# isno0907/ldmae

Measured on AMD Instinct MI355X. Metric: DiT-B train-step images/sec (32×32×16 latents) at 1/2/4/8 MI355X, higher is better.
Workload: dtype bf16; 1 GPU; LightningDiT-B/1 f8d16 bf16 train step (fwd+bwd+AdamW+EMA), 1024 tokens x 768, synthetic ImageNet-256 latents 32x32x16; per_gpu_batch=256, global_batch=256, parallelism=dp1

## Files before the change

### include/ldmae_hip.h

```cpp
#ifndef LDMAE_HIP_H
#define LDMAE_HIP_H
#ifdef __cplusplus
extern "C" {
#endif

#define LDMAE_OK 0
#define LDMAE_ERR_INVALID (-1)
#define LDMAE_ERR_HIP (-2)

#define LDMAE_F32 0
#define LDMAE_BF16 1
#define LDMAE_F16 2

#define LDMAE_EPI_BIAS 0
#define LDMAE_EPI_GATE_RES 1
#define LDMAE_EPI_BIAS_POS 2
#define LDMAE_EPI_BIAS_GELU 3
#define LDMAE_EPI_SWIGLU 4
#define LDMAE_EPI_SWIGLU_BWD 5
#define LDMAE_EPI_GELU_BWD 6
#define LDMAE_EPI_QKV_ROPE 7
#define LDMAE_EPI_TILE_LAUNCH 0x100
#define LDMAE_EPI_HALF_LINES 0x200
#define LDMAE_EPI_F16_INF 0x400

const char* ldmae_last_error(void);
const char* ldmae_version(void);
const char* ldmae_arch(void);

int ldmae_gemm_nt(int dtype, int out_dtype, int epi, const void* A, int lda, const void* B, int ldb, void* C, int ldc,
                  int M, int N, int K, const float* bias, float beta, const float* xin, float* xout,
                  const float* gate, int gate_ld, int rows_per_batch, void* stream);
int ldmae_gemm_nt_qkv_rope_ok(int B, int N, int H, int hd, int K, int lda, int ldb);
int ldmae_gemm_nt_qkv_rope(const void* A, int lda, const void* W, int ldb, const float* bias, void* qkv, void* q2, void* k2, const float* wq,
                           const float* wk, const float* cos, const float* sin, int B, int N, int H, int hd, int K, float eps, int store_raw_qk,
                           int tile_launch, void* stream);
int ldmae_gemm_tn_splits(int dtype, int M, int N, int K);
long ldmae_gemm_tn_workspace_bytes(int dtype, int M, int N, int K);
int ldmae_gemm_tn(int dtype, const void* A, int lda, const void* B, int ldb, float* C, float* dbias, int M, int N, int K, float beta,
                  float* workspace, long workspace_bytes, void* stream);
long ldmae_colsum_workspace_bytes(int M, int N);
int ldmae_colsum(int dtype, const void* X, int ldx, int M, int N, float* out, float beta, float* workspace, void* stream);

int ldmae_cast_weight(int dst_dtype, const float* src, void* dst, void* dstT, int R, int C, void* stream);
int ldmae_cast(int src_dtype, int dst_dtype, const void* src, void* dst, long n, void* stream);
int ldmae_thin_nt(int out_dtype, const float* T, const float* W, const float* bias, const float* pos, void* out, int M, int N, int K,
                  int rows_per_batch, void* stream);
long ldmae_thin_tn_workspace_bytes(int M, int N, int K);
int ldmae_thin_tn(const float* G, const float* T, float* dW, float* dbias, int M, int N, int K, float beta, float* workspace,
                  long workspace_bytes, void* stream);
int ldmae_multi_add(int count, void* const* dst, const void* const* src, const long* n, void* stream);
int ldmae_cast_stack(int dst_dtype, const void* const* srcs, int count, long n_each, void* dst, void* stream);

int ldmae_rmsnorm_modulate_fwd(int out_dtype, const float* x, const float* w, const float* shift, const float* scale,
                               int mod_ld, void* out, float* rstd, int M, int D, int rows_per_batch, float eps, void* stream);
long ldmae_rmsnorm_modulate_bwd_workspace_bytes(int M, int D, int rows_per_batch);
int ldmae_rmsnorm_modulate_bwd(int dtype, const void* dout, const float* x, const float* w, const float* scale, int mod_ld,
                               const float* rstd, float* dx_accum, float beta_x, float* dshift, float* dscale, int dmod_ld, float* dw,
                               float beta_w, int M, int D, int rows_per_batch, float* workspace, void* stream);
long ldmae_rmsnorm_modulate_bwd_gate_workspace_bytes(int M, int D, int rows_per_batch);
int ldmae_rmsnorm_modulate_bwd_gate(int dtype, const void* dout, const float* x, const float* w, const float* scale, int mod_ld,
                                    const float* rstd, float* dx_accum, float beta_x, float* dshift, float* dscale, int dmod_ld, float* dw,
                                    float beta_w, const void* y, const float* gate, int gate_ld, void* dy, float* dgate, int dgate_ld,
                                    float* dbias, int M, int D, int rows_per_batch, float* workspace, void* stream);
int ldmae_layernorm_modulate_fwd(int out_dtype, const float* x, const float* shift, const float* scale, int mod_ld, void* out, float* rstd,
                                 int M, int D, int rows_per_batch, float eps, void* stream);
int ldmae_layernorm_modulate_bwd(int dtype, const void* dout, const float* x, const float* scale, int mod_ld, const float* rstd, float* dx_accum,
                                 float beta_x, float* dshift, float* dscale, int dmod_ld, int M, int D, int rows_per_batch, float* workspace,
                                 void* stream);
int ldmae_layernorm_modulate_bwd_gate(int dtype, const void* dout, const float* x, const float* scale, int mod_ld, const float* rstd,
                                      float* dx_accum, float beta_x, float* dshift, float* dscale, int dmod_ld, const void* y, const float* gate,
                                      int gate_ld, void* dy, float* dgate, int dgate_ld, float* dbias, int M, int D, int rows_per_batch,
                                      float* workspace, void* stream);

int ldmae_qknorm_rope_fwd(int dtype, const void* qkv, const float* wq, const float* wk, const float* cos, const float* sin,
                          void* q, void* k, void* v, int B, int N, int H, int hd, float eps, void* stream);
long ldmae_qknorm_rope_bwd_workspace_bytes(int B, int N, int H, int hd);
int ldmae_qknorm_rope_bwd(int dtype, const void* dq, const void* dk, const void* dv, const void* qkv, const float* wq,
                          const float* wk, const float* cos, const float* sin, void* dqkv, float* dwq, float* dwk, float beta_w,
                          float* dbias_hqd, int B, int N, int H, int hd, float eps, float* workspace, void* stream);

int ldmae_rope(int dtype, const void* t, const float* cos, const float* sin, void* out, long rows, int N, int hd, int transposed,
               void* stream);

int ldmae_attention_fwd(int dtype, const void* q, const void* k, const void* v, void* o, float* lse, int B, int H, int N, int hd,
                        float scale, void* stream);
int ldmae_attention_bwd(int dtype, const void* q, const void* k, const void* v, const void* o, const void* do_, const float* lse,
                        void* dq, void* dk, void* dv, float* delta, int B, int H, int N, int hd, float scale, void* stream);

int ldmae_attention_fwd_qkv(int dtype, const void* qkv, void* o, float* lse, int B, int H, int N, int hd, float scale, void* stream);
int ldmae_attention_fwd_qkv_bounded(int dtype, const void* qkv, void* o, float* lse, const float* qk_max2, int B, int H, int N, int hd,
                                    float scale, void* stream);
int ldmae_k_norm_max(const void* qkv, float* qk_max2, int B, int N, int H, int hd, void* stream);
int ldmae_attention_bwd_qkv(int dtype, const void* qkv, const void* o, const void* do_, const float* lse, void* dqkv, float* delta,
                            int B, int H, int N, int hd, float scale, void* stream);

int ldmae_attention_fwd_pv(int dtype, const void* q, const void* k, const void* qkv, void* o, float* lse, int B, int H, int N, int hd,
                           float scale, void* stream);
int ldmae_attention_fwd_pv_bounded(int dtype, const void* q, const void* k, const void* qkv, void* o, float* lse, const float* score_bound,
                                   int B, int H, int N, int hd, float scale, void* stream);
int ldmae_qk_score_bound(const float* wq, const float* wk, int hd, float scale, float* out, void* stream);
int ldmae_attention_bwd_pv(int dtype, const void* q, const void* k, const void* qkv, const void* o, const void* do_, const float* lse,
                           void* dq, void* dk, void* dqkv, float* delta, int B, int H, int N, int hd, float scale, void* stream);
long ldmae_attention_bwd_pv_qknorm_workspace_bytes(int B, int H, int N, int hd);
int ldmae_attention_bwd_pv_qknorm(int dtype, const void* q, const void* k, const void* qkv, const void* o, const void* do_, const float* lse,
                                  const float* wq, const float* wk, const float* cos, const float* sin, float eps, void* dqkv, float* dwq,
                                  float* dwk, float* dbias, float* workspace, int B, int H, int N, int hd, float scale, void* stream);

int ldmae_swiglu_fwd(int dtype, const void* h12, void* hid, int M, int Hs, void* stream);
int ldmae_swiglu_bwd(int dtype, const void* dhid, const void* h12, void* dh12, int M, int Hs, void* stream);

long ldmae_gate_bwd_workspace_bytes(int M, int D, int rows_per_batch);
int ldmae_gate_bwd(int dtype, const float* dxout, const void* y, const float* gate, int gate_ld, void* dy, float* dgate,
                   int dgate_ld, float* dbias, int M, int D, int rows_per_batch, float* workspace, void* stream);

int ldmae_timestep_embedding(const float* t, float* out, int B, int dim, float max_period, void* stream);
int ldmae_silu_fwd(int out_dtype, const float* x, void* out, long n, void* stream);
int ldmae_silu_bwd(const float* dy, const float* x, float* dx, long n, void* stream);
int ldmae_label_embed_fwd(const float* table, const long long* y, const unsigned char* drop, float* out, int B, int D,
                          int num_classes, void* stream);
int ldmae_label_embed_bwd(const float* dout, const long long* y, const unsigned char* drop, float* dtable, int B, int D,
                          int num_classes, int rows, void* stream);

int ldmae_adamw_ema(float* p, const float* g, float* m, float* v, float* ema, long n, int step, double lr, double beta1,
                    double beta2, double eps, double weight_decay, double ema_decay, double grad_scale, void* stream);
int ldmae_ema_only(float* ema, const float* p, long n, double ema_decay, void* stream);

int ldmae_random_masking(const float* noise, long long* ids_restore, float* mask, long long* ids_keep, int N, int L, int keep,
                         void* stream);
int ldmae_patch_gather(int tok_dtype, const float* img, const long long* ids, const float* pos, void* tok, float* posg, int N, int keep,
                       int C, int S, int p, int D, void* stream);
int ldmae_latent_prologue(const float* moments, const float* noise, const float* lat_mean, const float* lat_std, float multiplier,
                          float* out, int B, int C, int HW, int sample, void* stream);
int ldmae_crop_resize_flip_u8(const unsigned char* blob, long blob_bytes, const long* offset, const int* geom, void* out, int out_bf16, int B,
                              int S, float mean, float std, void* stream);
int ldmae_gather_rows(const float* x, const long long* ids, float* out, int N, int L, int keep, int D, void* stream);
int ldmae_scatter_rows(const float* dout, const long long* ids, float* dx, int N, int L, int keep, int D, void* stream);
int ldmae_restore_tokens(const float* x, const float* mask_token, const float* pos, const long long* ids_restore, float* out, int B, int L,
                         int keep, int D, void* stream);
long ldmae_restore_tokens_bwd_workspace_bytes(int B, int L, int D);
int ldmae_restore_tokens_bwd(const float* dout, const long long* ids_restore, float* dx, float* dmask_token, int B, int L, int keep, int D,
                             float* workspace, void* stream);
long ldmae_vmae_encoder_blob_bytes(int nblocks);
int ldmae_vmae_encoder_fwd(const float* x, float* out, const void* blob, int B, int tokens, int dim, int heads, int hidden, int nblocks,
                           float eps, void* stream);
long ldmae_vmae_encoder_fwd_tiled_workspace_bytes(int B, int tokens);
int ldmae_vmae_encoder_fwd_tiled(const float* x, float* out, const void* blob, void* workspace, int B, int tokens, int dim, int heads,
                                 int hidden, int nblocks, float eps, void* stream);
int ldmae_vmae_encoder_fwd_tiled_f16(const float* x, float* out, const void* blob, void* workspace, int B, int tokens, int dim, int heads,
                                     int hidden, int nblocks, float eps, void* stream);
int ldmae_layernorm_fwd(int out_dtype, const float* x, const float* w, const float* b, void* out, float* mean, float* rstd,
                        int M, int D, float eps, void* stream);
long ldmae_layernorm_bwd_workspace_bytes(int M, int D);
int ldmae_layernorm_bwd(int dtype, const void* dout, const float* x, const float* w, const float* mean, const float* rstd,
                        float* dx_accum, float* dw, float* db, float beta_w, int M, int D, float* workspace, void* stream);
int ldmae_layernorm_bwd_cast(int dtype, const void* dout, const float* x, const float* w, const float* mean, const float* rstd,
                             float* dx_accum, void* dx_cast, float* dw, float* db, float beta_w, int M, int D, float* workspace, void* stream);
int ldmae_gelu_fwd(int dtype, const void* x, void* out, long n, void* stream);
int ldmae_gelu_bwd(int dtype, const void* dout, const void* x, void* dx, long n, void* stream);
int ldmae_gelu_tanh_fwd(int dtype, const void* x, void* out, long n, void* stream);
int ldmae_gelu_tanh_bwd(int dtype, const void* dout, const void* x, void* dx, long n, void* stream);
int ldmae_conv3x3(const float* x, const float* w, const float* b, float* out, int B, int C, int H, int W, void* stream);
long ldmae_conv3x3_bwd_workspace_bytes(int C);
int ldmae_conv3x3_bwd(const float* dout, const float* x, const float* w, float* dx, float* dw, float* db, int B, int C, int H, int W,
                      float* workspace, void* stream);

long ldmae_mae_loss_groups(long elements);
int ldmae_mae_loss_fwd(const float* pred_img, const float* imgs, const float* mask, float* partials, int B, int C, int H, int W, int p, void* stream);
int ldmae_mae_loss_bwd(const float* pred_img, const float* imgs, const float* mask, const float* coef, float* dpred_img, int B, int C, int H, int W,
                       int p, void* stream);

int ldmae_conv2d_nhwc_f32(const float* x, int ldx, int xoff, const float* w, const float* bias, float* out, int ldo, int ooff, int B, int H, int W,
                          int Cin, int Cout, int kh, int kw, int sh, int sw, int ph, int pw, int relu, void* stream);
int ldmae_pool2d_nhwc_f32(int mode, const float* x, int ldx, int xoff, float* out, int ldo, int ooff, int B, int H, int W, int C, int k, int stride,
                          int pad, void* stream);
int ldmae_global_avgpool_nhwc_f32(const float* x, int ldx, int xoff, float* out, int B, int HW, int C, void* stream);
int ldmae_fid_preprocess(const unsigned char* img, float* out, int B, int H, int W, int Ho, int Wo, void* stream);
int ldmae_fid_stats_accumulate(const float* feats, int n, int D, const float* shift, double* sum, double* cross, void* stream);

int ldmae_adm_preprocess(const unsigned char* img, float* out, int B, int H, int W, int Ho, int Wo, void* stream);
int ldmae_adm_spatial_tap(const float* x, int ldx, int xoff, float* out, int B, int HW, int C, void* stream);
int ldmae_row_sqnorms_f32(const float* x, int M, int D, float* out, void* stream);
int ldmae_pairwise_logits(const float* u, int M, int D, const float* w, int N, float* out, void* stream);
long ldmae_knn_partials_bytes(int M, int nsplit);
int ldmae_knn_radii(const float* x, const float* norms, int N, int D, const int* nhood, int nk, int nsplit, float* partials, float* radii,
                    void* stream);
int ldmae_pr_flags(const float* u, const float* nu, const float* ru, int M, const float* v, const float* nv, const float* rv, int N, int D, int nk,
                   int nsplit, int* u_in, int* v_in, void* stream);
long ldmae_adm_is_workspace_bytes(int M, int C, int split);
int ldmae_adm_softmax_is(const float* logits, int M, int C, int split, void* workspace, double* h, double* S, void* stream);

int ldmae_lpips_prep(const float* input, const float* target, float* out, int B, int H, int W, void* stream);
long ldmae_lpips_workspace_bytes(int B, int h, int w);
int ldmae_lpips_layer(const float* f, const float* lin_w, float* out, int B, int h, int w, int C, void* workspace, void* stream);
long ldmae_ssim_workspace_bytes(int B, int C, int H, int W);
int ldmae_ssim(const float* preds, const float* target, float* out, int B, int C, int H, int W, float lo, float hi, float data_range,
               void* workspace, void* stream);
long ldmae_sse_workspace_bytes(int B, long pixels);
int ldmae_recon_quantize_psnr(const float* decoded, const float* ref, unsigned char* dec8, unsigned char* ref8, long long* sse, int B, int H,
                              int W, void* workspace, void* stream);
int ldmae_sse_u8(const unsigned char* a, const unsigned char* b, long long* sse, int B, long n, void* workspace, void* stream);

int ldmae_conv3x3_relu_dgrad_nhwc_f32(const float* dy, const float* y, const float* w_rot, float* dx, int B, int H, int W, int Cy, int Cx,
                                      void* stream);
int ldmae_maxpool2x2_bwd_nhwc_f32(const float* dy, const float* x, float* dx, int B, int H, int W, int C, void* stream);
int ldmae_lpips_layer_bwd(const float* f, const float* lin_w, const float* g, float* d_input, float* d_target, int B, int h, int w, int C,
                          int accumulate, void* stream);
int ldmae_lpips_prep_bwd(const float* g, float* out, int B, int H, int W, void* stream);

int ldmae_lpips_prep_f16(const float* input, const float* target, void* out, int B, int H, int W, void* stream);
int ldmae_conv3x3_relu_nhwc_f16(const void* x, const void* w, const float* bias, void* out, int B, int H, int W, int Cin, int Cout, void* stream);
int ldmae_maxpool2x2_nhwc_f16(const void* x, void* out, int B, int H, int W, int C, void* stream);
int ldmae_lpips_layer_f16(const void* f, const float* lin_w, float* out, int B, int h, int w, int C, void* workspace, void* stream);
int ldmae_conv3x3_relu_dgrad_nhwc_bf16(const float* dy, const void* y, const void* w_rot, float* dx, int B, int H, int W, int Cy, int Cx,
                                       void* stream);
int ldmae_maxpool2x2_bwd_nhwc_xf16(const float* dy, const void* x, float* dx, int B, int H, int W, int C, void* stream);
int ldmae_lpips_layer_bwd_f16(const void* f, const float* lin_w, const float* g, float* d_input, float* d_target, int B, int h, int w, int C,
// ... 75 lines not shown
```

### ldmae_amd/_lib.py

```python
from __future__ import annotations

import ctypes as C
import os

import torch

_HERE = os.path.dirname(os.path.abspath(__file__))
LIB_PATH = os.path.join(_HERE, "libldmae_hip.so")
LIB_PATH = os.environ.get("LDMAE_HIP_LIB", LIB_PATH)

F32, BF16, F16 = 0, 1, 2
EPI_BIAS, EPI_GATE_RES, EPI_BIAS_POS, EPI_BIAS_GELU, EPI_SWIGLU, EPI_SWIGLU_BWD, EPI_GELU_BWD = 0, 1, 2, 3, 4, 5, 6

_vp, _i, _l, _f, _d = C.c_void_p, C.c_int, C.c_long, C.c_float, C.c_double

SIGNATURES = {
    "ldmae_last_error": (C.c_char_p, []),
    "ldmae_version": (C.c_char_p, []),
    "ldmae_arch": (C.c_char_p, []),
    "ldmae_gemm_nt": (_i, [_i, _i, _i, _vp, _i, _vp, _i, _vp, _i, _i, _i, _i, _vp, _f, _vp, _vp, _vp, _i, _i, _vp]),
    "ldmae_gemm_nt_qkv_rope_ok": (_i, [_i, _i, _i, _i, _i, _i, _i]),
    "ldmae_gemm_nt_qkv_rope": (_i, [_vp, _i, _vp, _i, _vp, _vp, _vp, _vp, _vp, _vp, _vp, _vp, _i, _i, _i, _i, _i, _f, _i, _i, _vp]),
    "ldmae_gemm_tn_splits": (_i, [_i, _i, _i, _i]),
    "ldmae_gemm_tn_workspace_bytes": (_l, [_i, _i, _i, _i]),
    "ldmae_gemm_tn": (_i, [_i, _vp, _i, _vp, _i, _vp, _vp, _i, _i, _i, _f, _vp, _l, _vp]),
    "ldmae_colsum_workspace_bytes": (_l, [_i, _i]),
    "ldmae_colsum": (_i, [_i, _vp, _i, _i, _i, _vp, _f, _vp, _vp]),
    "ldmae_cast_weight": (_i, [_i, _vp, _vp, _vp, _i, _i, _vp]),
    "ldmae_cast": (_i, [_i, _i, _vp, _vp, _l, _vp]),
    "ldmae_cast_stack": (_i, [_i, _vp, _i, _l, _vp, _vp]),
    "ldmae_multi_add": (_i, [_i, _vp, _vp, _vp, _vp]),
    "ldmae_thin_nt": (_i, [_i, _vp, _vp, _vp, _vp, _vp, _i, _i, _i, _i, _vp]),
    "ldmae_thin_tn_workspace_bytes": (_l, [_i, _i, _i]),
    "ldmae_thin_tn": (_i, [_vp, _vp, _vp, _vp, _i, _i, _i, _f, _vp, _l, _vp]),
    "ldmae_rmsnorm_modulate_fwd": (_i, [_i, _vp, _vp, _vp, _vp, _i, _vp, _vp, _i, _i, _i, _f, _vp]),
    "ldmae_rmsnorm_modulate_bwd_workspace_bytes": (_l, [_i, _i, _i]),
    "ldmae_rmsnorm_modulate_bwd": (_i, [_i, _vp, _vp, _vp, _vp, _i, _vp, _vp, _f, _vp, _vp, _i, _vp, _f, _i, _i, _i, _vp, _vp]),
    "ldmae_rmsnorm_modulate_bwd_gate_workspace_bytes": (_l, [_i, _i, _i]),
    "ldmae_rmsnorm_modulate_bwd_gate": (_i, [_i, _vp, _vp, _vp, _vp, _i, _vp, _vp, _f, _vp, _vp, _i, _vp, _f, _vp, _vp, _i, _vp, _vp, _i, _vp,
                                             _i, _i, _i, _vp, _vp]),
    "ldmae_qknorm_rope_fwd": (_i, [_i, _vp, _vp, _vp, _vp, _vp, _vp, _vp, _vp, _i, _i, _i, _i, _f, _vp]),
    "ldmae_qknorm_rope_bwd_workspace_bytes": (_l, [_i, _i, _i, _i]),
    "ldmae_qknorm_rope_bwd": (_i, [_i, _vp, _vp, _vp, _vp, _vp, _vp, _vp, _vp, _vp, _vp, _vp, _f, _vp, _i, _i, _i, _i, _f, _vp, _vp]),
    "ldmae_rope": (_i, [_i, _vp, _vp, _vp, _vp, _l, _i, _i, _i, _vp]),
    "ldmae_attention_fwd": (_i, [_i, _vp, _vp, _vp, _vp, _vp, _i, _i, _i, _i, _f, _vp]),
    "ldmae_attention_bwd": (_i, [_i, _vp, _vp, _vp, _vp, _vp, _vp, _vp, _vp, _vp, _vp, _i, _i, _i, _i, _f, _vp]),
    "ldmae_attention_fwd_qkv": (_i, [_i, _vp, _vp, _vp, _i, _i, _i, _i, _f, _vp]),
    "ldmae_attention_bwd_qkv": (_i, [_i, _vp, _vp, _vp, _vp, _vp, _vp, _i, _i, _i, _i, _f, _vp]),
    "ldmae_attention_fwd_pv": (_i, [_i, _vp, _vp, _vp, _vp, _vp, _i, _i, _i, _i, _f, _vp]),
    "ldmae_k_norm_max": (_i, [_vp, _vp, _i, _i, _i, _i, _vp]),
    "ldmae_attention_fwd_qkv_bounded": (_i, [_i, _vp, _vp, _vp, _vp, _i, _i, _i, _i, _f, _vp]),
    "ldmae_attention_fwd_pv_bounded": (_i, [_i, _vp, _vp, _vp, _vp, _vp, _vp, _i, _i, _i, _i, _f, _vp]),
    "ldmae_qk_score_bound": (_i, [_vp, _vp, _i, _f, _vp, _vp]),
    "ldmae_attention_bwd_pv": (_i, [_i, _vp, _vp, _vp, _vp, _vp, _vp, _vp, _vp, _vp, _vp, _i, _i, _i, _i, _f, _vp]),
    "ldmae_attention_bwd_pv_qknorm_workspace_bytes": (_l, [_i, _i, _i, _i]),
    "ldmae_attention_bwd_pv_qknorm": (_i, [_i, _vp, _vp, _vp, _vp, _vp, _vp, _vp, _vp, _vp, _vp, _f, _vp, _vp, _vp, _vp, _vp, _i, _i, _i, _i,
                                           _f, _vp]),
    "ldmae_swiglu_fwd": (_i, [_i, _vp, _vp, _i, _i, _vp]),
    "ldmae_swiglu_bwd": (_i, [_i, _vp, _vp, _vp, _i, _i, _vp]),
    "ldmae_gate_bwd_workspace_bytes": (_l, [_i, _i, _i]),
    "ldmae_gate_bwd": (_i, [_i, _vp, _vp, _vp, _i, _vp, _vp, _i, _vp, _i, _i, _i, _vp, _vp]),
    "ldmae_timestep_embedding": (_i, [_vp, _vp, _i, _i, _f, _vp]),
    "ldmae_silu_fwd": (_i, [_i, _vp, _vp, _l, _vp]),
    "ldmae_silu_bwd": (_i, [_vp, _vp, _vp, _l, _vp]),
    "ldmae_label_embed_fwd": (_i, [_vp, _vp, _vp, _vp, _i, _i, _i, _vp]),
    "ldmae_label_embed_bwd": (_i, [_vp, _vp, _vp, _vp, _i, _i, _i, _i, _vp]),
    "ldmae_adamw_ema": (_i, [_vp, _vp, _vp, _vp, _vp, _l, _i, _d, _d, _d, _d, _d, _d, _d, _vp]),
    "ldmae_ema_only": (_i, [_vp, _vp, _l, _d, _vp]),
    "ldmae_random_masking": (_i, [_vp, _vp, _vp, _vp, _i, _i, _i, _vp]),
    "ldmae_patch_gather": (_i, [_i, _vp, _vp, _vp, _vp, _vp, _i, _i, _i, _i, _i, _i, _vp]),
    "ldmae_latent_prologue": (_i, [_vp, _vp, _vp, _vp, _f, _vp, _i, _i, _i, _i, _vp]),
    "ldmae_crop_resize_flip_u8": (_i, [_vp, _l, _vp, _vp, _vp, _i, _i, _i, _f, _f, _vp]),
    "ldmae_gather_rows": (_i, [_vp, _vp, _vp, _i, _i, _i, _i, _vp]),
    "ldmae_scatter_rows": (_i, [_vp, _vp, _vp, _i, _i, _i, _i, _vp]),
    "ldmae_restore_tokens": (_i, [_vp, _vp, _vp, _vp, _vp, _i, _i, _i, _i, _vp]),
    "ldmae_restore_tokens_bwd_workspace_bytes": (_l, [_i, _i, _i]),
    "ldmae_restore_tokens_bwd": (_i, [_vp, _vp, _vp, _vp, _i, _i, _i, _i, _vp, _vp]),
    "ldmae_vmae_encoder_blob_bytes": (_l, [_i]),
    "ldmae_vmae_encoder_fwd": (_i, [_vp, _vp, _vp, _i, _i, _i, _i, _i, _i, _f, _vp]),
    "ldmae_vmae_encoder_fwd_tiled_workspace_bytes": (_l, [_i, _i]),
    "ldmae_vmae_encoder_fwd_tiled": (_i, [_vp, _vp, _vp, _vp, _i, _i, _i, _i, _i, _i, _f, _vp]),
    "ldmae_vmae_encoder_fwd_tiled_f16": (_i, [_vp, _vp, _vp, _vp, _i, _i, _i, _i, _i, _i, _f, _vp]),
    "ldmae_layernorm_fwd": (_i, [_i, _vp, _vp, _vp, _vp, _vp, _vp, _i, _i, _f, _vp]),
    "ldmae_layernorm_bwd_workspace_bytes": (_l, [_i, _i]),
    "ldmae_layernorm_bwd": (_i, [_i, _vp, _vp, _vp, _vp, _vp, _vp, _vp, _vp, _f, _i, _i, _vp, _vp]),
    "ldmae_mae_loss_groups": (_l, [_l]),
    "ldmae_mae_loss_fwd": (_i, [_vp, _vp, _vp, _vp, _i, _i, _i, _i, _i, _vp]),
    "ldmae_mae_loss_bwd": (_i, [_vp, _vp, _vp, _vp, _vp, _i, _i, _i, _i, _i, _vp]),
    "ldmae_layernorm_bwd_cast": (_i, [_i, _vp, _vp, _vp, _vp, _vp, _vp, _vp, _vp, _vp, _f, _i, _i, _vp, _vp]),
    "ldmae_gelu_fwd": (_i, [_i, _vp, _vp, _l, _vp]),
    "ldmae_gelu_bwd": (_i, [_i, _vp, _vp, _vp, _l, _vp]),
    "ldmae_gelu_tanh_fwd": (_i, [_i, _vp, _vp, _l, _vp]),
    "ldmae_gelu_tanh_bwd": (_i, [_i, _vp, _vp, _vp, _l, _vp]),
    "ldmae_layernorm_modulate_fwd": (_i, [_i, _vp, _vp, _vp, _i, _vp, _vp, _i, _i, _i, _f, _vp]),
    "ldmae_layernorm_modulate_bwd": (_i, [_i, _vp, _vp, _vp, _i, _vp, _vp, _f, _vp, _vp, _i, _i, _i, _i, _vp, _vp]),
    "ldmae_layernorm_modulate_bwd_gate": (_i, [_i, _vp, _vp, _vp, _i, _vp, _vp, _f, _vp, _vp, _i, _vp, _vp, _i, _vp, _vp, _i, _vp, _i, _i, _i, _vp, _vp]),
    "ldmae_conv3x3": (_i, [_vp, _vp, _vp, _vp, _i, _i, _i, _i, _vp]),
    "ldmae_conv3x3_bwd_workspace_bytes": (_l, [_i]),
    "ldmae_conv3x3_bwd": (_i, [_vp, _vp, _vp, _vp, _vp, _vp, _i, _i, _i, _i, _vp, _vp]),
    "ldmae_conv2d_nhwc_f32": (_i, [_vp, _i, _i, _vp, _vp, _vp, _i, _i, _i, _i, _i, _i, _i, _i, _i, _i, _i, _i, _i, _i, _vp]),
    "ldmae_pool2d_nhwc_f32": (_i, [_i, _vp, _i, _i, _vp, _i, _i, _i, _i, _i, _i, _i, _i, _i, _vp]),
    "ldmae_global_avgpool_nhwc_f32": (_i, [_vp, _i, _i, _vp, _i, _i, _i, _vp]),
    "ldmae_fid_preprocess": (_i, [_vp, _vp, _i, _i, _i, _i, _i, _vp]),
    "ldmae_fid_stats_accumulate": (_i, [_vp, _i, _i, _vp, _vp, _vp, _vp]),
    "ldmae_adm_preprocess": (_i, [_vp, _vp, _i, _i, _i, _i, _i, _vp]),
    "ldmae_adm_spatial_tap": (_i, [_vp, _i, _i, _vp, _i, _i, _i, _vp]),
    "ldmae_row_sqnorms_f32": (_i, [_vp, _i, _i, _vp, _vp]),
    "ldmae_pairwise_logits": (_i, [_vp, _i, _i, _vp, _i, _vp, _vp]),
    "ldmae_knn_partials_bytes": (_l, [_i, _i]),
    "ldmae_knn_radii": (_i, [_vp, _vp, _i, _i, _vp, _i, _i, _vp, _vp, _vp]),
    "ldmae_pr_flags": (_i, [_vp, _vp, _vp, _i, _vp, _vp, _vp, _i, _i, _i, _i, _vp, _vp, _vp]),
    "ldmae_adm_is_workspace_bytes": (_l, [_i, _i, _i]),
    "ldmae_adm_softmax_is": (_i, [_vp, _i, _i, _i, _vp, _vp, _vp, _vp]),
    "ldmae_lpips_prep": (_i, [_vp, _vp, _vp, _i, _i, _i, _vp]),
    "ldmae_lpips_workspace_bytes": (_l, [_i, _i, _i]),
    "ldmae_lpips_layer": (_i, [_vp, _vp, _vp, _i, _i, _i, _i, _vp, _vp]),
    "ldmae_ssim_workspace_bytes": (_l, [_i, _i, _i, _i]),
    "ldmae_ssim": (_i, [_vp, _vp, _vp, _i, _i, _i, _i, _f, _f, _f, _vp, _vp]),
    "ldmae_sse_workspace_bytes": (_l, [_i, _l]),
    "ldmae_recon_quantize_psnr": (_i, [_vp, _vp, _vp, _vp, _vp, _i, _i, _i, _vp, _vp]),
    "ldmae_sse_u8": (_i, [_vp, _vp, _vp, _i, _l, _vp, _vp]),
    "ldmae_conv3x3_relu_dgrad_nhwc_f32": (_i, [_vp, _vp, _vp, _vp, _i, _i, _i, _i, _i, _vp]),
    "ldmae_maxpool2x2_bwd_nhwc_f32": (_i, [_vp, _vp, _vp, _i, _i, _i, _i, _vp]),
    "ldmae_lpips_layer_bwd": (_i, [_vp, _vp, _vp, _vp, _vp, _i, _i, _i, _i, _i, _vp]),
    "ldmae_lpips_prep_bwd": (_i, [_vp, _vp, _i, _i, _i, _vp]),
    "ldmae_lpips_prep_f16": (_i, [_vp, _vp, _vp, _i, _i, _i, _vp]),
    "ldmae_conv3x3_relu_nhwc_f16": (_i, [_vp, _vp, _vp, _vp, _i, _i, _i, _i, _i, _vp]),
    "ldmae_maxpool2x2_nhwc_f16": (_i, [_vp, _vp, _i, _i, _i, _i, _vp]),
    "ldmae_lpips_layer_f16": (_i, [_vp, _vp, _vp, _i, _i, _i, _i, _vp, _vp]),
    "ldmae_conv3x3_relu_dgrad_nhwc_bf16": (_i, [_vp, _vp, _vp, _vp, _i, _i, _i, _i, _i, _vp]),
    "ldmae_maxpool2x2_bwd_nhwc_xf16": (_i, [_vp, _vp, _vp, _i, _i, _i, _i, _vp]),
    "ldmae_lpips_layer_bwd_f16": (_i, [_vp, _vp, _vp, _vp, _vp, _i, _i, _i, _i, _i, _vp]),
    "ldmae_lpips_prep_bwd_c8": (_i, [_vp, _vp, _i, _i, _i, _vp]),
    "ldmae_groupnorm_stats_nhwc_f32": (_i, [_vp, _vp, _vp, _i, _i, _i, _i, _f, _vp]),
    "ldmae_groupnorm_apply_nhwc_f32": (_i, [_vp, _vp, _vp, _vp, _vp, _vp, _i, _i, _i, _i, _i, _vp]),
    "ldmae_conv3x3_vae_nhwc_f32": (_i, [_i, _vp, _vp, _vp, _vp, _vp, _vp, _vp, _vp, _i, _i, _vp, _i, _i, _i, _i, _i, _vp]),
    "ldmae_conv1x1_res_nhwc_f32": (_i, [_vp, _vp, _vp, _vp, _vp, _i, _i, _i, _vp]),
    "ldmae_softmax_rows_f32": (_i, [_vp, _i, _i, _i, _f, _vp]),
    "ldmae_conv3x3_vae_nhwc_f16": (_i, [_i, _i, _vp, _vp, _vp, _vp, _vp, _vp, _vp, _vp, _i, _i, _vp, _i, _i, _i, _i, _i, _vp]),
    "ldmae_conv1x1_res_nhwc_f16": (_i, [_vp, _vp, _vp, _vp, _vp, _i, _i, _i, _vp]),
    "ldmae_groupnorm_apply_nhwc_f16out": (_i, [_vp, _vp, _vp, _vp, _vp, _vp, _i, _i, _i, _i, _i, _vp]),
    "ldmae_ode_partials": (_i, [_l]),
    "ldmae_rk_stage_f32": (_i, [_vp, _vp, _l, C.POINTER(_f), _i, _vp, _vp, _l, _vp, _f, _vp, _i, _vp]),
    "ldmae_dopri5_finish_f32": (_i, [_vp, _vp, _l, _vp, _f, _f, _vp, _vp, _vp, _l, _vp]),
    "ldmae_rms_norm_scaled_f32": (_i, [_vp, _vp, _f, _f, _vp, _vp, _l, _vp]),
    "ldmae_dopri5_interp_f32": (_i, [_vp, _vp, _vp, _vp, _l, _vp, _vp, _f, _vp, _l, _vp]),
    "ldmae_dopri5_advance": (_i, [_vp, _vp, _vp, _vp, _vp]),
    "ldmae_dopri5_initial_step": (_i, [_vp, _i, _vp, _vp]),
    "ldmae_rademacher_f32": (_i, [_vp, _l, C.c_ulonglong, C.c_ulonglong, _vp]),
    "ldmae_rowdot_partials": (_l, [_i, _l]),
    "ldmae_rowdot_f32": (_i, [_vp, _vp, _vp, _i, _l, _vp, _vp]),
    "ldmae_likelihood_finish_f32": (_i, [_vp, _vp, _f, _vp, _i, _vp]),
    "ldmae_normal_f32": (_i, [_vp, _l, C.c_ulonglong, C.c_ulonglong, _vp]),
    "ldmae_sde_combine_f32": (_i, [_vp, _vp, _vp, _vp, C.POINTER(_f), _i, _vp, _f, _i, C.c_ulonglong, C.c_ulonglong, _vp, _vp, _l, _f, _vp, _i, _vp]),
    "ldmae_prof_enable": (_i, [_i]),
    "ldmae_prof_collect": (_i, [C.POINTER(_d), C.POINTER(_d), C.POINTER(_l)]),
    "ldmae_launch_counts": (_i, [C.POINTER(_l), _i, _i]),
    "ldmae_mx8_quantize": (_i, [_i, _vp, _i, _vp, _vp, _i, _i, _vp]),
    "ldmae_rmsnorm_modulate_fwd_mx8": (_i, [_vp, _vp, _vp, _vp, _i, _vp, _vp, _vp, _i, _i, _i, _f, _vp]),
    "ldmae_gemm_nt_mx8_ok": (_i, [_i, _i, _i, _i, _i]),
    "ldmae_gemm_nt_mx8": (_i, [_i, _i, _vp, _vp, _i, _vp, _vp, _i, _vp, _i, _i, _i, _i, _vp, _vp, _vp, _vp, _i, _i, _vp]),
    "ldmae_gemm_nt_qkv_rope_mx8_ok": (_i, [_i, _i, _i, _i, _i, _i, _i]),
    "ldmae_gemm_nt_qkv_rope_mx8": (_i, [_vp, _vp, _i, _vp, _vp, _i, _vp, _vp, _vp, _vp, _vp, _vp, _vp, _vp, _i, _i, _i, _i, _i, _f, _i, _i, _vp]),
    "ldmae_mx8_launch_counts": (_i, [C.POINTER(_l), _i, _i]),
}
DIAG_SIGNATURES = {
    "ldmae_tune": (_i, [_i, _i]),
    "ldmae_tune_query": (_i, [_i]),
    "ldmae_debug_nt_stamps": (None, [_vp]),
}
EPI_TILE_LAUNCH = 0x100
EPI_HALF_LINES = 0x200
EPI_F16_INF = 0x400

_lib = None


def load():
    global _lib
    if _lib is not None:
        return _lib
    if not os.path.exists(LIB_PATH):
        raise RuntimeError(
            f"{LIB_PATH} is missing: build it with `python -c 'import __graft_entry__ as g; g.build()'` "
            "(or `make -C ldmae_amd/csrc`).  ldmae_amd has no CPU / PyTorch fallback.")
    lib = C.CDLL(LIB_PATH)
    for name, (res, args) in SIGNATURES.items():
        fn = getattr(lib, name)
        fn.restype = res
        fn.argtypes = args
    if hasattr(lib, "ldmae_tune"):
        for name, (res, args) in DIAG_SIGNATURES.items():
            fn = getattr(lib, name)
# ... 61 lines not shown
```

### ldmae_amd/csrc/common.h

```cpp
#pragma once
#include <hip/hip_runtime.h>
#include <stdint.h>
#include <stdio.h>

#include "../../include/ldmae_hip.h"

typedef __bf16 bf16;
typedef __attribute__((ext_vector_type(8))) __bf16 bf16x8;
typedef __attribute__((ext_vector_type(4))) __bf16 bf16x4;
typedef __attribute__((ext_vector_type(2))) __bf16 bf16x2;
typedef _Float16 f16;
typedef __attribute__((ext_vector_type(8))) _Float16 f16x8;
typedef __attribute__((ext_vector_type(4))) _Float16 f16x4;
typedef __attribute__((ext_vector_type(4))) float f32x4;
typedef __attribute__((ext_vector_type(16))) float f32x16;
typedef __attribute__((ext_vector_type(4))) short s16x4;

#define LDS_PTR(T, p) ((__attribute__((address_space(3))) T*)(p))
#define GLB_PTR(p) ((const __attribute__((address_space(1))) void*)(p))

__device__ __forceinline__ void glds16(const void* g, const void* lds) {
  const unsigned a = __builtin_amdgcn_readfirstlane((unsigned)(uintptr_t)LDS_PTR(void, lds));
  asm volatile("s_mov_b32 m0, %1\n\ts_nop 0\n\tglobal_load_lds_dwordx4 %0, off" ::"v"(g), "s"(a) : "memory", "m0");
}
__device__ __forceinline__ void glds4(const void* g, const void* lds) {
  const unsigned a = __builtin_amdgcn_readfirstlane((unsigned)(uintptr_t)LDS_PTR(void, lds));
  asm volatile("s_mov_b32 m0, %1\n\ts_nop 0\n\tglobal_load_lds_dword %0, off" ::"v"(g), "s"(a) : "memory", "m0");
}

__device__ __forceinline__ void glds16_s(const void* sbase, unsigned voff, unsigned lds_addr) {
  asm volatile("s_mov_b32 m0, %2\n\ts_nop 0\n\tglobal_load_lds_dwordx4 %0, %1" ::"v"(voff), "s"(sbase), "s"(lds_addr) : "memory", "m0");
}
__device__ __forceinline__ void glds4_s(const void* sbase, unsigned voff, unsigned lds_addr) {
  asm volatile("s_mov_b32 m0, %2\n\ts_nop 0\n\tglobal_load_lds_dword %0, %1" ::"v"(voff), "s"(sbase), "s"(lds_addr) : "memory", "m0");
}

void ldmae_set_error(const char* fmt, ...);
#define LDMAE_FAIL(code, ...) do { ldmae_set_error(__VA_ARGS__); return (code); } while (0)
#define LDMAE_REQUIRE(cond, ...) do { if (!(cond)) LDMAE_FAIL(LDMAE_ERR_INVALID, __VA_ARGS__); } while (0)
#define LDMAE_CHECK_LAUNCH(name) do { hipError_t e_ = hipGetLastError(); \
    if (e_ != hipSuccess) LDMAE_FAIL(LDMAE_ERR_HIP, "%s: %s", name, hipGetErrorString(e_)); } while (0)

template <typename T> __device__ __forceinline__ float to_f(T v);
template <> __device__ __forceinline__ float to_f<float>(float v) { return v; }
template <> __device__ __forceinline__ float to_f<bf16>(bf16 v) { return (float)v; }
template <typename T> __device__ __forceinline__ T from_f(float v);
template <> __device__ __forceinline__ float from_f<float>(float v) { return v; }
template <> __device__ __forceinline__ bf16 from_f<bf16>(float v) { return (bf16)v; }
template <> __device__ __forceinline__ float to_f<f16>(f16 v) { return (float)v; }
template <> __device__ __forceinline__ f16 from_f<f16>(float v) { return (f16)v; }
__device__ __forceinline__ float sat_f16(float v, float mx) { return v == v ? __builtin_amdgcn_fmed3f(v, -mx, mx) : v; }
__device__ __forceinline__ float4 sat_f16(float4 v, float mx) { return make_float4(sat_f16(v.x, mx), sat_f16(v.y, mx), sat_f16(v.z, mx), sat_f16(v.w, mx)); }
template <typename T> struct Pack;
template <> struct Pack<bf16> { typedef bf16x8 v8; typedef bf16x4 v4; };
template <> struct Pack<f16> { typedef f16x8 v8; typedef f16x4 v4; };

__device__ __forceinline__ float erf_as(float x) {
  const float ax = fabsf(x);
  const float t = __builtin_amdgcn_rcpf(fmaf(0.3275911f, ax, 1.f));
  const float poly = t * fmaf(t, fmaf(t, fmaf(t, fmaf(t, 1.061405429f, -1.453152027f), 1.421413741f), -0.284496736f), 0.254829592f);
  return copysignf(fmaf(-poly, __builtin_amdgcn_exp2f(-ax * ax * 1.4426950408889634f), 1.f), x);
}
template <typename T> __device__ __forceinline__ float erf_act(float x) { return erff(x); }
template <typename T> __device__ __forceinline__ float gelu_act(float y) { return 0.5f * y * (1.f + erf_act<T>(y * 0.70710678118654752f)); }

template <typename T> struct Vec8;
template <> struct Vec8<float> {
  static __device__ __forceinline__ void load(const float* p, float (&v)[8]) {
    float4 a = *(const float4*)p, b = *(const float4*)(p + 4);
    v[0] = a.x; v[1] = a.y; v[2] = a.z; v[3] = a.w; v[4] = b.x; v[5] = b.y; v[6] = b.z; v[7] = b.w;
  }
  static __device__ __forceinline__ void store(float* p, const float (&v)[8]) {
    *(float4*)p = make_float4(v[0], v[1], v[2], v[3]);
    *(float4*)(p + 4) = make_float4(v[4], v[5], v[6], v[7]);
  }
};
template <> struct Vec8<bf16> {
  static __device__ __forceinline__ void load(const bf16* p, float (&v)[8]) {
    bf16x8 a = *(const bf16x8*)p;
#pragma unroll
    for (int i = 0; i < 8; ++i) v[i] = (float)a[i];
  }
  static __device__ __forceinline__ void store(bf16* p, const float (&v)[8]) {
    bf16x8 a;
#pragma unroll
    for (int i = 0; i < 8; ++i) a[i] = (bf16)v[i];
    *(bf16x8*)p = a;
  }
};

template <> struct Vec8<f16> {
  static __device__ __forceinline__ void load(const f16* p, float (&v)[8]) {
    f16x8 a = *(const f16x8*)p;
#pragma unroll
    for (int i = 0; i < 8; ++i) v[i] = (float)a[i];
  }
  static __device__ __forceinline__ void store(f16* p, const float (&v)[8]) {
    f16x8 a;
#pragma unroll
    for (int i = 0; i < 8; ++i) a[i] = from_f<f16>(v[i]);
    *(f16x8*)p = a;
  }
};

__device__ __forceinline__ float4 load4f(const float* p) { return *(const float4*)p; }
__device__ __forceinline__ float4 load4f(const f16* p) {
  const f16x4 v = *(const f16x4*)p;
  return make_float4((float)v[0], (float)v[1], (float)v[2], (float)v[3]);
}

__device__ __forceinline__ float wave_sum(float v) {
#pragma unroll
  for (int o = 32; o > 0; o >>= 1) v += __shfl_xor(v, o, 64);
  return v;
}
template <int CTRL> __device__ __forceinline__ float dpp_add_f(float v) {
  return v + __builtin_bit_cast(float, __builtin_amdgcn_update_dpp(0, __builtin_bit_cast(int, v), CTRL, 0xF, 0xF, true));
}
__device__ __forceinline__ float wave_sum_dpp(float v) {
  v = dpp_add_f<0xB1>(v);
  v = dpp_add_f<0x4E>(v);
  v = dpp_add_f<0x141>(v);
  v = dpp_add_f<0x140>(v);
  const int i = __builtin_bit_cast(int, v);
  const float r0 = __builtin_bit_cast(float, __builtin_amdgcn_readlane(i, 0)), r1 = __builtin_bit_cast(float, __builtin_amdgcn_readlane(i, 16));
  const float r2 = __builtin_bit_cast(float, __builtin_amdgcn_readlane(i, 32)), r3 = __builtin_bit_cast(float, __builtin_amdgcn_readlane(i, 48));
  return (r0 + r1) + (r2 + r3);
}
__device__ __forceinline__ float wave_max(float v) {
#pragma unroll
  for (int o = 32; o > 0; o >>= 1) v = fmaxf(v, __shfl_xor(v, o, 64));
  return v;
}
template <int W> __device__ __forceinline__ float group_sum(float v) {
#pragma unroll
  for (int o = W / 2; o > 0; o >>= 1) v += __shfl_xor(v, o, 64);
  return v;
}

__device__ __forceinline__ float4 rope_apply(float4 t, float4 c, float4 s) {
  return make_float4(t.x * c.x - t.y * s.x, t.y * c.y + t.x * s.y, t.z * c.z - t.w * s.z, t.w * c.w + t.z * s.w);
}

__device__ __forceinline__ unsigned xcd_remap(unsigned bid, unsigned nwg) {
  const unsigned q = nwg >> 3, r = nwg & 7, x = bid & 7, i = bid >> 3;
  return (x < r ? x * (q + 1) : r * (q + 1) + (x - r) * q) + i;
}

#ifdef LDMAE_DIAG
int ldmae_tune_get(int key);
#else
static inline constexpr int ldmae_tune_get(int) { return 0; }
#endif
void ldmae_count(int family);
bool ldmae_prof_is_on();
long ldmae_prof_begin(hipStream_t st, double flops);
void ldmae_prof_end(long idx, hipStream_t st);

static inline hipStream_t as_stream(void* s) { return (hipStream_t)s; }
static inline unsigned cdiv(long a, long b) { return (unsigned)((a + b - 1) / b); }

__device__ __forceinline__ float fast_sigmoid(float a) { return __builtin_amdgcn_rcpf(1.f + __expf(-a)); }
```

### ldmae_amd/csrc/elementwise.hip

```cpp
#include "common.h"

template <typename T> __device__ __forceinline__ float4 load4(const T* p);
template <> __device__ __forceinline__ float4 load4<float>(const float* p) { const f32x4 v = __builtin_nontemporal_load((const f32x4*)p); return make_float4(v[0], v[1], v[2], v[3]); }
template <> __device__ __forceinline__ float4 load4<bf16>(const bf16* p) {
  bf16x4 v = __builtin_nontemporal_load((const bf16x4*)p);
  return make_float4((float)v[0], (float)v[1], (float)v[2], (float)v[3]);
}
template <> __device__ __forceinline__ float4 load4<f16>(const f16* p) {
  const f16x4 a = *(const f16x4*)p;
  return make_float4((float)a[0], (float)a[1], (float)a[2], (float)a[3]);
}
template <typename T> __device__ __forceinline__ void store4(T* p, float4 v);
template <> __device__ __forceinline__ void store4<float>(float* p, float4 v) { f32x4 o = {v.x, v.y, v.z, v.w}; __builtin_nontemporal_store(o, (f32x4*)p); }
template <> __device__ __forceinline__ void store4<bf16>(bf16* p, float4 v) {
  bf16x4 o; o[0] = (bf16)v.x; o[1] = (bf16)v.y; o[2] = (bf16)v.z; o[3] = (bf16)v.w;
  __builtin_nontemporal_store(o, (bf16x4*)p);
}
__device__ __forceinline__ float4 f4(float a) { return make_float4(a, a, a, a); }
__device__ __forceinline__ float4 operator+(float4 a, float4 b) { return make_float4(a.x + b.x, a.y + b.y, a.z + b.z, a.w + b.w); }
__device__ __forceinline__ float4 operator-(float4 a, float4 b) { return make_float4(a.x - b.x, a.y - b.y, a.z - b.z, a.w - b.w); }
__device__ __forceinline__ float4 operator*(float4 a, float4 b) { return make_float4(a.x * b.x, a.y * b.y, a.z * b.z, a.w * b.w); }
__device__ __forceinline__ float4 operator*(float4 a, float s) { return make_float4(a.x * s, a.y * s, a.z * s, a.w * s); }
__device__ __forceinline__ float hsum(float4 a) { return (a.x + a.y) + (a.z + a.w); }

template <int RL>
__global__ __launch_bounds__(32 * RL) void group_reduce_kernel(const float* __restrict__ P, int p_ld, int nout, int cols, int group,
                                                              float* __restrict__ out, int out_ld, float beta,
                                                              const float* __restrict__ P2 = nullptr, float* __restrict__ out2 = nullptr,
                                                              float beta2 = 0.f) {
  __shared__ float red[RL][33];
  if (blockIdx.z == 1) { P = P2; out = out2; beta = beta2; }
  const int cl = threadIdx.x & 31, rl = threadIdx.x >> 5;
  const int c = blockIdx.x * 32 + cl, o = blockIdx.y;
  float s = 0.f;
  if (c < cols) {
    const float* p = P + (size_t)o * group * p_ld + c;
    for (int r = rl; r < group; r += RL) s += p[(size_t)r * p_ld];
  }
  red[rl][cl] = s;
  __syncthreads();
  if (rl == 0 && c < cols) {
    float t = red[0][cl];
#pragma unroll
    for (int k = 1; k < RL; ++k) t += red[k][cl];
    float* q = out + (size_t)o * out_ld + c;
    *q = (beta != 0.f ? beta * *q : 0.f) + t;
  }
}
static void group_reduce(const float* P, int p_ld, int nout, int cols, int group, float* out, int out_ld, float beta, hipStream_t st,
                         const float* P2 = nullptr, float* out2 = nullptr, float beta2 = 0.f) {
  const unsigned gz = P2 ? 2 : 1;
  if (group >= 256)
    hipLaunchKernelGGL(group_reduce_kernel<32>, dim3(cdiv(cols, 32), nout, gz), dim3(1024), 0, st, P, p_ld, nout, cols, group, out, out_ld, beta, P2, out2, beta2);
  else
    hipLaunchKernelGGL(group_reduce_kernel<8>, dim3(cdiv(cols, 32), nout, gz), dim3(256), 0, st, P, p_ld, nout, cols, group, out, out_ld, beta, P2, out2, beta2);
}

static int pick_rows_per_wg(int rows_per_batch) {
  const int cap = ldmae_tune_get(10) > 0 ? ldmae_tune_get(10) : 64;
  for (int r = cap; r >= 1; r >>= 1) if (rows_per_batch % r == 0) return r;
  return 0;
}

__device__ __forceinline__ float4 mul_rn(float4 a, float4 b) {
#pragma clang fp contract(off)
  return make_float4(a.x * b.x, a.y * b.y, a.z * b.z, a.w * b.w);
}

template <int NCH, typename OutT, bool FULL = false>
__global__ __launch_bounds__(256) void rmsnorm_mod_fwd_kernel(const float* __restrict__ x, const float* __restrict__ w,
                                                              const float* __restrict__ shift, const float* __restrict__ scale,
                                                              int mod_ld, OutT* __restrict__ out, float* __restrict__ rstd, int M, int D,
                                                              int rpb, float eps, int center = 0) {
  const int lane = threadIdx.x & 63, wave = threadIdx.x >> 6, nch = D >> 2;
  float4 wv[NCH];
#pragma unroll
  for (int i = 0; i < NCH; ++i) { const int c = lane + 64 * i; wv[i] = c < nch ? (w ? *(const float4*)(w + 4 * c) : f4(1.f)) : f4(0.f); }
  if constexpr (FULL) {
    const int m0 = (blockIdx.x * 4 + wave) * 4, b = m0 / rpb;
    float4 sc1[NCH], sh[NCH];
#pragma unroll
    for (int i = 0; i < NCH; ++i) {
      sc1[i] = scale ? f4(1.f) + *(const float4*)(scale + (size_t)b * mod_ld + 4 * lane + 256 * i) : f4(1.f);
      sh[i] = shift ? *(const float4*)(shift + (size_t)b * mod_ld + 4 * lane + 256 * i) : f4(0.f);
    }
    for (int r = 0; r < 4; ++r) {
      const int m = m0 + r;
      float4 xv[NCH];
      float ss = 0.f;
#pragma unroll
      for (int i = 0; i < NCH; ++i) xv[i] = *(const float4*)(x + (size_t)m * D + 4 * lane + 256 * i);
#pragma unroll
      for (int i = 0; i < NCH; ++i) ss += hsum(xv[i] * xv[i]);
      ss = wave_sum(ss);
      const float rs = rsqrtf(ss / (float)D + eps);
      if (lane == 0 && rstd) rstd[m] = rs;
#pragma unroll
      for (int i = 0; i < NCH; ++i) {
        float4 y = (xv[i] * rs) * wv[i];
        if (scale) y = y * sc1[i];
        if (shift) y = y + sh[i];
        store4<OutT>(out + (size_t)m * D + 4 * lane + 256 * i, y);
      }
    }
    return;
  }
  for (int r = 0; r < 4; ++r) {
    const int m = (blockIdx.x * 4 + wave) * 4 + r;
    if (m >= M) return;
    const int b = m / rpb;
    float4 xv[NCH];
    float ss = 0.f;
#pragma unroll
    for (int i = 0; i < NCH; ++i) {
      const int c = lane + 64 * i;
      xv[i] = c < nch ? *(const float4*)(x + (size_t)m * D + 4 * c) : f4(0.f);
      ss += hsum(xv[i] * xv[i]);
    }
    if (center) {
      float s1 = 0.f;
#pragma unroll
      for (int i = 0; i < NCH; ++i) s1 += hsum(xv[i]);
      const float mean = wave_sum(s1) / (float)D;
      ss = 0.f;
#pragma unroll
      for (int i = 0; i < NCH; ++i) {
        if (lane + 64 * i < nch) xv[i] = xv[i] - f4(mean);
        ss += hsum(xv[i] * xv[i]);
      }
    }
    ss = wave_sum(ss);
    const float rs = rsqrtf(ss / (float)D + eps);
    if (lane == 0 && rstd) rstd[m] = rs;
#pragma unroll
    for (int i = 0; i < NCH; ++i) {
      const int c = lane + 64 * i;
      if (c < nch) {
        float4 y = (xv[i] * rs) * wv[i];
        if (scale) y = y * (f4(1.f) + *(const float4*)(scale + (size_t)b * mod_ld + 4 * c));
        if (shift) y = y + *(const float4*)(shift + (size_t)b * mod_ld + 4 * c);
        store4<OutT>(out + (size_t)m * D + 4 * c, y);
      }
    }
  }
}

struct GateBwdArgs { const void* y; const float* gate; int gate_ld; void* dy; float* Pg; float* Pb; int dx_overwrite; int center; };
template <int NCH, typename T, bool GATE, bool FULL = false>
__global__ __launch_bounds__(256) void rmsnorm_mod_bwd_kernel(const T* __restrict__ dout, const float* __restrict__ x,
                                                              const float* __restrict__ w, const float* __restrict__ scale, int mod_ld,
                                                              const float* __restrict__ rstd, float* __restrict__ dx, float* __restrict__ P,
                                                              int M, int D, int rpb, int rows_per_wg, GateBwdArgs ga) {
  extern __shared__ float red[];
  const int lane = threadIdx.x & 63, wave = threadIdx.x >> 6, nch = D >> 2;
  const int m_base = blockIdx.x * rows_per_wg, b = m_base / rpb;
  float4 wv[GATE ? 1 : NCH], sc1[GATE ? 1 : NCH], a_sh[NCH], a_sc[NCH], a_w[NCH];
  float4 a_g[GATE ? NCH : 1], a_b[GATE ? NCH : 1];
  const T* gy = (const T*)ga.y;
  T* gdy = (T*)ga.dy;
  float* cw = red;
  float* cs = red + D;
  float* cg = red + 2 * D;
  if constexpr (GATE) {
    for (int c = threadIdx.x; c < nch; c += 256) {
      *(float4*)(cw + 4 * c) = w ? *(const float4*)(w + 4 * c) : f4(1.f);
      *(float4*)(cs + 4 * c) = scale ? f4(1.f) + *(const float4*)(scale + (size_t)b * mod_ld + 4 * c) : f4(1.f);
      *(float4*)(cg + 4 * c) = *(const float4*)(ga.gate + (size_t)b * ga.gate_ld + 4 * c);
    }
    __syncthreads();
  }
#pragma unroll
  for (int i = 0; i < NCH; ++i) {
    const int c = lane + 64 * i;
    if constexpr (!GATE) {
      wv[i] = c < nch ? (w ? *(const float4*)(w + 4 * c) : f4(1.f)) : f4(0.f);
      sc1[i] = (c < nch && scale) ? f4(1.f) + *(const float4*)(scale + (size_t)b * mod_ld + 4 * c) : f4(1.f);
    }
    a_sh[i] = a_sc[i] = a_w[i] = f4(0.f);
    if constexpr (GATE) a_g[i] = a_b[i] = f4(0.f);
  }
  if constexpr (FULL) {
    for (int r = wave; r < rows_per_wg; r += 4) {
      const int m = m_base + r;
      if (m >= M) break;
      const size_t ro = (size_t)m * D + 4 * lane;
      float4 g[NCH], nv[NCH], dold[NCH], yv[GATE ? NCH : 1];
#pragma unroll
      for (int i = 0; i < NCH; ++i) { g[i] = load4<T>(dout + ro + 256 * i); nv[i] = *(const float4*)(x + ro + 256 * i); }
#pragma unroll
      for (int i = 0; i < NCH; ++i) {
        dold[i] = ga.dx_overwrite ? f4(0.f) : *(const float4*)(dx + ro + 256 * i);
        if constexpr (GATE) yv[i] = load4<T>(gy + ro + 256 * i);
      }
      const float rs = rstd[m];
      float4 dn[NCH];
      float dot = 0.f;
#pragma unroll
      for (int i = 0; i < NCH; ++i) {
        const int c = lane + 64 * i;
        const float4 wc = GATE ? *(const float4*)(cw + 4 * c) : wv[i], sc = GATE ? *(const float4*)(cs + 4 * c) : sc1[i];
        nv[i] = nv[i] * rs;
        const float4 dy = g[i] * sc;
        a_sh[i] = a_sh[i] + g[i];
        a_sc[i] = a_sc[i] + g[i] * (nv[i] * wc);
        a_w[i] = a_w[i] + dy * nv[i];
        dn[i] = dy * wc;
        dot += hsum(dn[i] * nv[i]);
      }
      dot = wave_sum_dpp(dot) / (float)D;
#pragma unroll
      for (int i = 0; i < NCH; ++i) {
        const int c = lane + 64 * i;
        const float4 d0 = (dn[i] - nv[i] * dot) * rs;
        const float4 gn = ga.dx_overwrite ? d0 : dold[i] + d0;
        *(float4*)(dx + ro + 256 * i) = gn;
        if constexpr (GATE) {
          a_g[i] = a_g[i] + gn * yv[i];
          const float4 d = mul_rn(gn, *(const float4*)(cg + 4 * c));
          store4<T>(gdy + ro + 256 * i, d);
          a_b[i] = a_b[i] + make_float4(to_f<T>(from_f<T>(d.x)), to_f<T>(from_f<T>(d.y)), to_f<T>(from_f<T>(d.z)), to_f<T>(from_f<T>(d.w)));
        }
      }
    }
  } else
  for (int r = wave; r < rows_per_wg; r += 4) {
    const int m = m_base + r;
    if (m >= M) break;
    const float rs = rstd[m];
    float4 nv[NCH], dn[NCH];
    float dot = 0.f, mean = 0.f;
    if (ga.center) {
      float s1 = 0.f;
#pragma unroll
      for (int i = 0; i < NCH; ++i) { const int c = lane + 64 * i; if (c < nch) s1 += hsum(*(const float4*)(x + (size_t)m * D + 4 * c)); }
      mean = wave_sum(s1) / (float)D;
    }
#pragma unroll
    for (int i = 0; i < NCH; ++i) {
      const int c = lane + 64 * i;
      if (c < nch) {
        const float4 g = load4<T>(dout + (size_t)m * D + 4 * c);
        const float4 wc = GATE ? *(const float4*)(cw + 4 * c) : wv[i], sc = GATE ? *(const float4*)(cs + 4 * c) : sc1[i];
        nv[i] = (*(const float4*)(x + (size_t)m * D + 4 * c) - f4(mean)) * rs;
        const float4 dy = g * sc;
        a_sh[i] = a_sh[i] + g;
        a_sc[i] = a_sc[i] + g * (nv[i] * wc);
        a_w[i] = a_w[i] + dy * nv[i];
        dn[i] = dy * wc;
        dot += hsum(dn[i] * nv[i]);
      } else { nv[i] = dn[i] = f4(0.f); }
    }
    dot = wave_sum(dot) / (float)D;
    float msum = 0.f;
    if (ga.center) {
      float s1 = 0.f;
#pragma unroll
      for (int i = 0; i < NCH; ++i) s1 += hsum(dn[i]);
      msum = wave_sum(s1) / (float)D;
    }
#pragma unroll
    for (int i = 0; i < NCH; ++i) {
      const int c = lane + 64 * i;
      if (c < nch) {
        float* p = dx + (size_t)m * D + 4 * c;
        const float4 d0 = ((dn[i] - nv[i] * dot) - f4(msum)) * rs;
        const float4 g = ga.dx_overwrite ? d0 : *(const float4*)p + d0;
        *(float4*)p = g;
        if constexpr (GATE) {
          a_g[i] = a_g[i] + g * load4<T>(gy + (size_t)m * D + 4 * c);
          const float4 d = mul_rn(g, *(const float4*)(cg + 4 * c));
          store4<T>(gdy + (size_t)m * D + 4 * c, d);
          a_b[i] = a_b[i] + make_float4(to_f<T>(from_f<T>(d.x)), to_f<T>(from_f<T>(d.y)), to_f<T>(from_f<T>(d.z)), to_f<T>(from_f<T>(d.w)));
        }
      }
    }
  }
  if constexpr (GATE) __syncthreads();
#pragma unroll
  for (int i = 0; i < NCH; ++i) {
    const int c = lane + 64 * i;
    if (c < nch) {
      *(float4*)(red + (wave * 3 + 0) * D + 4 * c) = a_sh[i];
      *(float4*)(red + (wave * 3 + 1) * D + 4 * c) = a_sc[i];
      *(float4*)(red + (wave * 3 + 2) * D + 4 * c) = a_w[i];
    }
  }
  __syncthreads();
  for (int i = threadIdx.x; i < 3 * D; i += 256)
    P[(size_t)blockIdx.x * 3 * D + i] = (red[i] + red[3 * D + i]) + (red[6 * D + i] + red[9 * D + i]);
  if constexpr (GATE) {
    __syncthreads();
#pragma unroll
    for (int i = 0; i < NCH; ++i) {
      const int c = lane + 64 * i;
      if (c < nch) { *(float4*)(red + (wave * 2 + 0) * D + 4 * c) = a_g[i]; *(float4*)(red + (wave * 2 + 1) * D + 4 * c) = a_b[i]; }
    }
    __syncthreads();
    for (int i = threadIdx.x; i < D; i += 256) {
      ga.Pg[(size_t)blockIdx.x * D + i] = (red[i] + red[2 * D + i]) + (red[4 * D + i] + red[6 * D + i]);
      ga.Pb[(size_t)blockIdx.x * D + i] = (red[D + i] + red[3 * D + i]) + (red[5 * D + i] + red[7 * D + i]);
    }
  }
}

__global__ void mod_partials_reduce_kernel(const float* __restrict__ P, int D, int gps, float* __restrict__ dshift,
                                           float* __restrict__ dscale, int dmod_ld, float* __restrict__ dwb,
                                           const float* __restrict__ Pg = nullptr, float* __restrict__ dgate = nullptr, int dgate_ld = 0,
                                           const float* __restrict__ Pb = nullptr, float* __restrict__ dbb = nullptr) {
  const int d = blockIdx.x * blockDim.x + threadIdx.x, b = blockIdx.y;
  if (d >= D) return;
  auto sum = [&](const float* p, size_t stride) {
    float s = 0.f;
    int g = 0;
    for (; g + 8 <= gps; g += 8) {
      float v[8];
#pragma unroll
      for (int j = 0; j < 8; ++j) v[j] = p[(size_t)(g + j) * stride];
#pragma unroll
      for (int j = 0; j < 8; ++j) s += v[j];
    }
    for (; g < gps; ++g) s += p[(size_t)g * stride];
    return s;
  };
  if (P) {
    const float* p = P + (size_t)b * gps * 3 * D + d;
    const float s0 = sum(p, (size_t)3 * D), s1 = sum(p + D, (size_t)3 * D), s2 = sum(p + 2 * D, (size_t)3 * D);
    if (dshift) dshift[(size_t)b * dmod_ld + d] = s0;
    if (dscale) dscale[(size_t)b * dmod_ld + d] = s1;
    dwb[(size_t)b * D + d] = s2;
  }
  if (Pg) dgate[(size_t)b * dgate_ld + d] = sum(Pg + (size_t)b * gps * D + d, (size_t)D);
  if (Pb) dbb[(size_t)b * D + d] = sum(Pb + (size_t)b * gps * D + d, (size_t)D);
}

#define DISPATCH_NCH(D, CALL)                                   \
  switch (((D) / 4 + 63) / 64) {                                \
    case 1: { constexpr int NCH = 1; CALL; } break;             \
    case 2: { constexpr int NCH = 2; CALL; } break;             \
    case 3: { constexpr int NCH = 3; CALL; } break;             \
    case 4: { constexpr int NCH = 4; CALL; } break;             \
    case 5: { constexpr int NCH = 5; CALL; } break;             \
    case 6: { constexpr int NCH = 6; CALL; } break;             \
    case 7: { constexpr int NCH = 7; CALL; } break;             \
    case 8: { constexpr int NCH = 8; CALL; } break;             \
    default: LDMAE_FAIL(LDMAE_ERR_INVALID, "row width D=%d > 2048 unsupported", (D)); }

static int norm_modulate_fwd(int out_dtype, const float* x, const float* w, const float* shift, const float* scale,
                             int mod_ld, void* out, float* rstd, int M, int D, int rows_per_batch, float eps, int center, void* stream) {
  LDMAE_REQUIRE(x && (w || center) && out && M > 0 && D > 0, "rmsnorm_modulate_fwd: null pointer or empty");
  LDMAE_REQUIRE(D % 4 == 0 && (mod_ld % 4 == 0 || (!shift && !scale)), "rmsnorm_modulate_fwd: D=%d mod_ld=%d must be multiples of 4", D, mod_ld);
  LDMAE_REQUIRE(rows_per_batch > 0 && M % rows_per_batch == 0, "rmsnorm_modulate_fwd: M=%d %% rows_per_batch=%d != 0", M, rows_per_batch);
  hipStream_t st = as_stream(stream);
  const unsigned grid = cdiv(M, 16);
  if (out_dtype == LDMAE_BF16 && D % 256 == 0 && M % 16 == 0 && rows_per_batch % 16 == 0 && !center) {
    DISPATCH_NCH(D, hipLaunchKernelGGL((rmsnorm_mod_fwd_kernel<NCH, bf16, true>), dim3(grid), dim3(256), 0, st, x, w, shift, scale, mod_ld, (bf16*)out, rstd, M, D, rows_per_batch, eps, 0));
  } else if (out_dtype == LDMAE_BF16) {
    DISPATCH_NCH(D, hipLaunchKernelGGL((rmsnorm_mod_fwd_kernel<NCH, bf16>), dim3(grid), dim3(256), 0, st, x, w, shift, scale, mod_ld, (bf16*)out, rstd, M, D, rows_per_batch, eps, center));
  } else {
    DISPATCH_NCH(D, hipLaunchKernelGGL((rmsnorm_mod_fwd_kernel<NCH, float>), dim3(grid), dim3(256), 0, st, x, w, shift, scale, mod_ld, (float*)out, rstd, M, D, rows_per_batch, eps, center));
  }
  LDMAE_CHECK_LAUNCH("rmsnorm_modulate_fwd");
  return LDMAE_OK;
}
extern "C" int ldmae_rmsnorm_modulate_fwd(int out_dtype, const float* x, const float* w, const float* shift, const float* scale,
                                          int mod_ld, void* out, float* rstd, int M, int D, int rows_per_batch, float eps, void* stream) {
  return norm_modulate_fwd(out_dtype, x, w, shift, scale, mod_ld, out, rstd, M, D, rows_per_batch, eps, 0, stream);
}
extern "C" int ldmae_layernorm_modulate_fwd(int out_dtype, const float* x, const float* shift, const float* scale, int mod_ld, void* out,
                                            float* rstd, int M, int D, int rows_per_batch, float eps, void* stream) {
  return norm_modulate_fwd(out_dtype, x, nullptr, shift, scale, mod_ld, out, rstd, M, D, rows_per_batch, eps, 1, stream);
}

extern "C" long ldmae_rmsnorm_modulate_bwd_workspace_bytes(int M, int D, int rows_per_batch) {
  const int rw = pick_rows_per_wg(rows_per_batch);
  if (rw == 0) return -1;
  return ((long)(M / rw) * 3 * D + (long)(M / rows_per_batch) * D) * 4;
}

extern "C" long ldmae_colsum_workspace_bytes(int M, int N);
extern "C" int ldmae_colsum(int dtype, const void* X, int ldx, int M, int N, float* out, float beta, float* workspace, void* stream);
extern "C" long ldmae_gate_bwd_workspace_bytes(int M, int D, int rows_per_batch);

static int rmsnorm_modulate_bwd_core(int dtype, const void* dout, const float* x, const float* w, const float* scale, int mod_ld,
                                     const float* rstd, float* dx_accum, float beta_x, float* dshift, float* dscale, int dmod_ld, float* dw,
                                     float beta_w, int M, int D, int rows_per_batch, float* workspace, const GateBwdArgs* gate,
                                     float* dgate, int dgate_ld, float* dbias, void* stream, int center = 0) {
  LDMAE_REQUIRE(dout && x && (w || center) && rstd && dx_accum && (dw || center) && workspace, "rmsnorm_modulate_bwd: null pointer");
  LDMAE_REQUIRE(D % 4 == 0 && M > 0 && rows_per_batch > 0 && M % rows_per_batch == 0, "rmsnorm_modulate_bwd: bad shape M=%d D=%d rpb=%d", M, D, rows_per_batch);
  const int rw = pick_rows_per_wg(rows_per_batch);
  LDMAE_REQUIRE(rw > 0, "rmsnorm_modulate_bwd: rows_per_batch=%d must be a multiple of 4", rows_per_batch);
  hipStream_t st = as_stream(stream);
  const int G = M / rw, B = M / rows_per_batch, gps = rows_per_batch / rw;
  float* P = workspace;
  float* dwb = workspace + (size_t)G * 3 * D;
  float* gws = dwb + (size_t)B * D;
  const size_t lds = (size_t)4 * 3 * D * sizeof(float);
  LDMAE_REQUIRE(beta_x == 0.f || beta_x == 1.f, "rmsnorm_modulate_bwd: beta_x must be 0 (write dx) or 1 (accumulate into dx)");
  GateBwdArgs ga{nullptr, nullptr, 0, nullptr, nullptr, nullptr, 0, 0};
  if (gate) { ga = *gate; ga.Pg = gws; ga.Pb = gws + (size_t)G * D; }
  ga.dx_overwrite = beta_x == 0.f;
  ga.center = center;
  if (center && !dw) dw = P;
#define LAUNCH(T, GATE) DISPATCH_NCH(D, hipLaunchKernelGGL((rmsnorm_mod_bwd_kernel<NCH, T, GATE>), dim3(G), dim3(256), lds, st, (const T*)dout, x, w, scale, mod_ld, rstd, dx_accum, P, M, D, rows_per_batch, rw, ga))
#define LAUNCH_FULL(T, GATE) DISPATCH_NCH(D, hipLaunchKernelGGL((rmsnorm_mod_bwd_kernel<NCH, T, GATE, true>), dim3(G), dim3(256), lds, st, (const T*)dout, x, w, scale, mod_ld, rstd, dx_accum, P, M, D, rows_per_batch, rw, ga))
  if (dtype == LDMAE_BF16 && D % 256 == 0 && !center) { if (gate) { LAUNCH_FULL(bf16, true); } else { LAUNCH_FULL(bf16, false); } }
  else if (dtype == LDMAE_BF16) { if (gate) { LAUNCH(bf16, true); } else { LAUNCH(bf16, false); } }
  else { if (gate) { LAUNCH(float, true); } else { LAUNCH(float, false); } }
#undef LAUNCH
#undef LAUNCH_FULL
  LDMAE_CHECK_LAUNCH("rmsnorm_modulate_bwd");
  if (gate) {
    float* dbb = ga.Pb + (size_t)G * D;
    hipLaunchKernelGGL(mod_partials_reduce_kernel, dim3(cdiv(D, 256), B), dim3(256), 0, st, P, D, gps, dshift, dscale, dmod_ld, dwb,
                       (const float*)ga.Pg, dgate, dgate_ld, (const float*)ga.Pb, dbb);
    group_reduce(dwb, D, 1, D, B, dw, D, beta_w, st, dbb, dbias, 0.f);
    LDMAE_CHECK_LAUNCH("rmsnorm_modulate_bwd_gate reduce");
    return LDMAE_OK;
  }
  hipLaunchKernelGGL(mod_partials_reduce_kernel, dim3(cdiv(D, 256), B), dim3(256), 0, st, P, D, gps, dshift, dscale, dmod_ld, dwb);
  group_reduce(dwb, D, 1, D, B, dw, D, beta_w, st);
  LDMAE_CHECK_LAUNCH("rmsnorm_modulate_bwd reduce");
  return LDMAE_OK;
}

extern "C" int ldmae_rmsnorm_modulate_bwd(int dtype, const void* dout, const float* x, const float* w, const float* scale, int mod_ld,
                                          const float* rstd, float* dx_accum, float beta_x, float* dshift, float* dscale, int dmod_ld, float* dw,
                                          float beta_w, int M, int D, int rows_per_batch, float* workspace, void* stream) {
  return rmsnorm_modulate_bwd_core(dtype, dout, x, w, scale, mod_ld, rstd, dx_accum, beta_x, dshift, dscale, dmod_ld, dw, beta_w, M, D, rows_per_batch,
                                   workspace, nullptr, nullptr, 0, nullptr, stream);
}

extern "C" long ldmae_rmsnorm_modulate_bwd_gate_workspace_bytes(int M, int D, int rows_per_batch) {
  const long a = ldmae_rmsnorm_modulate_bwd_workspace_bytes(M, D, rows_per_batch), b = ldmae_gate_bwd_workspace_bytes(M, D, rows_per_batch);
  return a < 0 ? a : a + b;
}
extern "C" int ldmae_rmsnorm_modulate_bwd_gate(int dtype, const void* dout, const float* x, const float* w, const float* scale, int mod_ld,
                                               const float* rstd, float* dx_accum, float beta_x, float* dshift, float* dscale, int dmod_ld, float* dw,
                                               float beta_w, const void* y, const float* gate, int gate_ld, void* dy, float* dgate,
                                               int dgate_ld, float* dbias, int M, int D, int rows_per_batch, float* workspace, void* stream) {
  LDMAE_REQUIRE(y && gate && dy && dgate && dbias, "rmsnorm_modulate_bwd_gate: null pointer");
  LDMAE_REQUIRE(gate_ld % 4 == 0, "rmsnorm_modulate_bwd_gate: gate_ld=%d must be a multiple of 4", gate_ld);
  const GateBwdArgs ga{y, gate, gate_ld, dy, nullptr, nullptr, 0, 0};
  return rmsnorm_modulate_bwd_core(dtype, dout, x, w, scale, mod_ld, rstd, dx_accum, beta_x, dshift, dscale, dmod_ld, dw, beta_w, M, D, rows_per_batch,
                                   workspace, &ga, dgate, dgate_ld, dbias, stream);
}
extern "C" int ldmae_layernorm_modulate_bwd(int dtype, const void* dout, const float* x, const float* scale, int mod_ld, const float* rstd,
                                            float* dx_accum, float beta_x, float* dshift, float* dscale, int dmod_ld, int M, int D, int rows_per_batch,
                                            float* workspace, void* stream) {
  return rmsnorm_modulate_bwd_core(dtype, dout, x, nullptr, scale, mod_ld, rstd, dx_accum, beta_x, dshift, dscale, dmod_ld, nullptr, 0.f, M, D, rows_per_batch,
                                   workspace, nullptr, nullptr, 0, nullptr, stream, 1);
}
extern "C" int ldmae_layernorm_modulate_bwd_gate(int dtype, const void* dout, const float* x, const float* scale, int mod_ld, const float* rstd,
                                                 float* dx_accum, float beta_x, float* dshift, float* dscale, int dmod_ld, const void* y, const float* gate,
                                                 int gate_ld, void* dy, float* dgate, int dgate_ld, float* dbias, int M, int D, int rows_per_batch,
                                                 float* workspace, void* stream) {
  LDMAE_REQUIRE(y && gate && dy && dgate && dbias, "layernorm_modulate_bwd_gate: null pointer");
  LDMAE_REQUIRE(gate_ld % 4 == 0, "layernorm_modulate_bwd_gate: gate_ld=%d must be a multiple of 4", gate_ld);
  const GateBwdArgs ga{y, gate, gate_ld, dy, nullptr, nullptr, 0, 1};
  return rmsnorm_modulate_bwd_core(dtype, dout, x, nullptr, scale, mod_ld, rstd, dx_accum, beta_x, dshift, dscale, dmod_ld, nullptr, 0.f, M, D, rows_per_batch,
                                   workspace, &ga, dgate, dgate_ld, dbias, stream, 1);
}

__device__ __forceinline__ float4 rope_apply_bwd(float4 g, float4 c, float4 s) {
  return make_float4(g.x * c.x + g.y * s.y, g.y * c.y - g.x * s.x, g.z * c.z + g.w * s.w, g.w * c.w - g.z * s.z);
}

template <int LPR, typename T>
__global__ __launch_bounds__(256) void qknorm_rope_fwd_kernel(const T* __restrict__ qkv, const float* __restrict__ wq,
                                                              const float* __restrict__ wk, const float* __restrict__ cosT,
                                                              const float* __restrict__ sinT, T* __restrict__ q, T* __restrict__ k,
                                                              T* __restrict__ v, int B, int N, int H, int hd, float eps) {
  const int sub = threadIdx.x % LPR, c4 = sub * 4;
  const bool act = c4 < hd;
  const long items = (long)B * N * H;
  const long gid = ((long)blockIdx.x * 256 + threadIdx.x) / LPR, gstride = (long)gridDim.x * 256 / LPR;
  const bool plain = cosT == nullptr;
  const bool norm = wq != nullptr;
  const float4 wqv = (act && norm) ? *(const float4*)(wq + c4) : f4(1.f), wkv = (act && norm) ? *(const float4*)(wk + c4) : f4(1.f);
  for (long it = gid; it < items; it += gstride) {
    const int h = it % H, n = (it / H) % N, b = it / ((long)H * N);
    const T* src = qkv + ((size_t)(b * N + n) * 3 * H + h) * hd + c4;
    const size_t dst = ((size_t)(b * H + h) * N + n) * hd + c4;
    float4 qv = f4(0.f), kv = f4(0.f), vv = f4(0.f), cs = f4(0.f), sn = f4(0.f);
    if (act) {
      qv = load4<T>(src); kv = load4<T>(src + (size_t)H * hd);
      if (v) vv = load4<T>(src + (size_t)2 * H * hd);
      if (!plain) { cs = *(const float4*)(cosT + (size_t)n * hd + c4); sn = *(const float4*)(sinT + (size_t)n * hd + c4); }
    }
    if (plain) {
      if (act) { store4<T>(q + dst, qv); store4<T>(k + dst, kv); store4<T>(v + dst, vv); }
      continue;
    }
    const float rq = norm ? rsqrtf(group_sum<LPR>(hsum(qv * qv)) / (float)hd + eps) : 1.f;
    const float rk = norm ? rsqrtf(group_sum<LPR>(hsum(kv * kv)) / (float)hd + eps) : 1.f;
    if (act) {
      store4<T>(q + dst, rope_apply((qv * rq) * wqv, cs, sn));
      store4<T>(k + dst, rope_apply((kv * rk) * wkv, cs, sn));
      if (v) store4<T>(v + dst, vv);
    }
  }
}

template <int LPR>
__global__ __launch_bounds__(256) void qknorm_rope_fwd8_kernel(const bf16* __restrict__ qkv, const float* __restrict__ wq, const float* __restrict__ wk,
                                                               const float* __restrict__ cosT, const float* __restrict__ sinT, bf16* __restrict__ q,
                                                               bf16* __restrict__ k, int B, int N, int H, float eps) {
  constexpr int hd = LPR * 8;
  const int sub = threadIdx.x % LPR, c8 = sub * 8;
  const long items = (long)B * N * H;
  const long gid = ((long)blockIdx.x * 256 + threadIdx.x) / LPR, gstride = (long)gridDim.x * 256 / LPR;
  float wqv[8], wkv[8];
  const bool norm = wq != nullptr;
#pragma unroll
  for (int j = 0; j < 8; ++j) { wqv[j] = norm ? wq[c8 + j] : 1.f; wkv[j] = norm ? wk[c8 + j] : 1.f; }
  auto one = [&](long it, bf16x8 qi, bf16x8 ki) {
    const int h = it % H, n = (it / H) % N, b = it / ((long)H * N);
    const float4 c0 = *(const float4*)(cosT + (size_t)n * hd + c8), c1 = *(const float4*)(cosT + (size_t)n * hd + c8 + 4);
    const float4 s0 = *(const float4*)(sinT + (size_t)n * hd + c8), s1 = *(const float4*)(sinT + (size_t)n * hd + c8 + 4);
    float qv[8], kv[8], sq = 0.f, sk = 0.f;
#pragma unroll
    for (int j = 0; j < 8; ++j) { qv[j] = (float)qi[j]; kv[j] = (float)ki[j]; }
    sq = ((qv[0] * qv[0] + qv[1] * qv[1]) + (qv[2] * qv[2] + qv[3] * qv[3])) + ((qv[4] * qv[4] + qv[5] * qv[5]) + (qv[6] * qv[6] + qv[7] * qv[7]));
    sk = ((kv[0] * kv[0] + kv[1] * kv[1]) + (kv[2] * kv[2] + kv[3] * kv[3])) + ((kv[4] * kv[4] + kv[5] * kv[5]) + (kv[6] * kv[6] + kv[7] * kv[7]));
    const float rq = norm ? rsqrtf(group_sum<LPR>(sq) / (float)hd + eps) : 1.f, rk = norm ? rsqrtf(group_sum<LPR>(sk) / (float)hd + eps) : 1.f;
    const float4 a0 = rope_apply(make_float4(qv[0] * rq * wqv[0], qv[1] * rq * wqv[1], qv[2] * rq * wqv[2], qv[3] * rq * wqv[3]), c0, s0);
    const float4 a1 = rope_apply(make_float4(qv[4] * rq * wqv[4], qv[5] * rq * wqv[5], qv[6] * rq * wqv[6], qv[7] * rq * wqv[7]), c1, s1);
    const float4 b0 = rope_apply(make_float4(kv[0] * rk * wkv[0], kv[1] * rk * wkv[1], kv[2] * rk * wkv[2], kv[3] * rk * wkv[3]), c0, s0);
    const float4 b1 = rope_apply(make_float4(kv[4] * rk * wkv[4], kv[5] * rk * wkv[5], kv[6] * rk * wkv[6], kv[7] * rk * wkv[7]), c1, s1);
    bf16x8 qo, ko;
    qo[0] = (bf16)a0.x; qo[1] = (bf16)a0.y; qo[2] = (bf16)a0.z; qo[3] = (bf16)a0.w; qo[4] = (bf16)a1.x; qo[5] = (bf16)a1.y; qo[6] = (bf16)a1.z; qo[7] = (bf16)a1.w;
    ko[0] = (bf16)b0.x; ko[1] = (bf16)b0.y; ko[2] = (bf16)b0.z; ko[3] = (bf16)b0.w; ko[4] = (bf16)b1.x; ko[5] = (bf16)b1.y; ko[6] = (bf16)b1.z; ko[7] = (bf16)b1.w;
    const size_t dst = ((size_t)(b * H + h) * N + n) * hd + c8;
    __builtin_nontemporal_store(qo, (bf16x8*)(q + dst));
    __builtin_nontemporal_store(ko, (bf16x8*)(k + dst));
  };
  auto src_of = [&](long it) { const int h = it % H; const long bn = it / H; return qkv + ((size_t)bn * 3 * H + h) * hd + c8; };
  long it = gid;
  for (; it + gstride < items; it += 2 * gstride) {
    const bf16* p0 = src_of(it);
    const bf16* p1 = src_of(it + gstride);
    const bf16x8 q0 = __builtin_nontemporal_load((const bf16x8*)p0), k0 = __builtin_nontemporal_load((const bf16x8*)(p0 + (size_t)H * hd));
    const bf16x8 q1 = __builtin_nontemporal_load((const bf16x8*)p1), k1 = __builtin_nontemporal_load((const bf16x8*)(p1 + (size_t)H * hd));
    one(it, q0, k0);
    one(it + gstride, q1, k1);
  }
  if (it < items) {
    const bf16* p0 = src_of(it);
    one(it, *(const bf16x8*)p0, *(const bf16x8*)(p0 + (size_t)H * hd));
  }
}

template <typename T>
__global__ __launch_bounds__(256) void qknorm_rope_fwd_dense_kernel(const T* __restrict__ qkv, const float* __restrict__ wq,
                                                                    const float* __restrict__ wk, const float* __restrict__ cosT,
                                                                    const float* __restrict__ sinT, T* __restrict__ q, T* __restrict__ k,
                                                                    T* __restrict__ v, int B, int N, int H, int hd, float eps) {
  __shared__ float2 red[256];
  const int cpi = hd >> 2, ipw = 256 / cpi, t = threadIdx.x, li = t / cpi, c4 = (t % cpi) * 4;
  const bool lane_ok = li < ipw;
  const long items = (long)B * N * H;
  const float4 wqv = *(const float4*)(wq + c4), wkv = *(const float4*)(wk + c4);
  for (long base = (long)blockIdx.x * ipw; base < items; base += (long)gridDim.x * ipw) {
    const long it = base + li;
    const bool act = lane_ok && it < items;
    const long tile = it / (8 * H);
    const int rr = (int)(it % (8 * H)), h = rr >> 3;
    const long tok = tile * 8 + (rr & 7);
    const int n = (int)(tok % N), b = (int)(tok / N);
    const T* src = qkv + ((size_t)(b * N + n) * 3 * H + h) * hd + c4;
    const size_t dst = ((size_t)(b * H + h) * N + n) * hd + c4;
    float4 qv = f4(0.f), kv = f4(0.f), vv = f4(0.f), cs = f4(0.f), sn = f4(0.f);
    if (act) {
      qv = load4<T>(src); kv = load4<T>(src + (size_t)H * hd);
      if (v) vv = load4<T>(src + (size_t)2 * H * hd);
      cs = *(const float4*)(cosT + (size_t)n * hd + c4); sn = *(const float4*)(sinT + (size_t)n * hd + c4);
    }
    red[t] = make_float2(hsum(qv * qv), hsum(kv * kv));
    __syncthreads();
    float sq = 0.f, sk = 0.f;
    if (lane_ok) {
      for (int j = 0; j < cpi; ++j) { const float2 p = red[li * cpi + j]; sq += p.x; sk += p.y; }
    }
    __syncthreads();
    if (act) {
      const float rq = rsqrtf(sq / (float)hd + eps), rk = rsqrtf(sk / (float)hd + eps);
      store4<T>(q + dst, rope_apply((qv * rq) * wqv, cs, sn));
      store4<T>(k + dst, rope_apply((kv * rk) * wkv, cs, sn));
      if (v) store4<T>(v + dst, vv);
    }
  }
}

__global__ __launch_bounds__(256) void qknorm_rope_fwd_dense8_kernel(const bf16* __restrict__ qkv, const float* __restrict__ wq,
                                                                     const float* __restrict__ wk, const float* __restrict__ cosT,
                                                                     const float* __restrict__ sinT, bf16* __restrict__ q, bf16* __restrict__ k,
// ... 806 lines not shown
```

### ldmae_amd/csrc/gemm_nt_common.h

```cpp
#pragma once
#include "common.h"

struct EpiArgs {
  void* C;
  void* C2;
  const float* bias;
  const float* xin;
  float* xout;
  const float* gate;
  int gate_ld;
  int rows_per_batch;
  int ldc;
  float beta;
  float f16_max;
  void* q2;
  void* k2;
  const float* wq;
  const float* wk;
  const float* cosT;
  const float* sinT;
  int heads;
  int store_raw_qk;
  float eps;
};

int ldmae_launch_nt_lines(int epi, int out_bf16, const void* A, const void* B, int M, int N, int K, int lda, int ldb, const struct EpiArgs& e,
                          int grid, int ntiles, hipStream_t st);
int ldmae_launch_nt_lines_f16(int epi, int out_f16, const void* A, const void* B, int M, int N, int K, int lda, int ldb, const struct EpiArgs& e,
                              int grid, int ntiles, hipStream_t st);

#ifdef LDMAE_DIAG
int ldmae_launch_nt_defer(int epi, const void* A, const void* B, int M, int N, int K, int lda, int ldb, const EpiArgs& e, int grid, int ntiles,
                          hipStream_t st);
int ldmae_launch_nt_wl(int epi, const void* A, const void* B, int M, int N, int K, int lda, int ldb, const EpiArgs& e, int grid, int ntiles,
                       hipStream_t st);
int ldmae_launch_nt_w4(int epi, int out_bf16, const void* A, const void* B, int M, int N, int K, int lda, int ldb, const EpiArgs& e, int grid,
                       int ntiles, hipStream_t st);
int ldmae_launch_nt_p8(int epi, int out_bf16, const void* A, const void* B, int M, int N, int K, int lda, int ldb, const EpiArgs& e, int grid,
                       int ntiles, hipStream_t st);
#endif

template <typename OutT> __device__ __forceinline__ float act_round(float y) { return to_f<OutT>(from_f<OutT>(y)); }
__device__ __forceinline__ float4 gate_res4(float4 x, float4 g, float4 y) {
  return make_float4(fmaf(g.x, y.x, x.x), fmaf(g.y, y.y, x.y), fmaf(g.z, y.z, x.z), fmaf(g.w, y.w, x.w));
}
template <typename OutT> __device__ __forceinline__ float4 act_round4(float4 y) {
  return make_float4(act_round<OutT>(y.x), act_round<OutT>(y.y), act_round<OutT>(y.z), act_round<OutT>(y.w));
}

template <typename OutT> __device__ __forceinline__ float gelu_bwd_val(float acc, float v) {
  const float cdf = 0.5f * (1.f + erf_act<OutT>(v * 0.70710678118654752f)), pdf = 0.3989422804014327f * __expf(-0.5f * v * v);
  return act_round<OutT>(acc) * (cdf + v * pdf);
}

template <typename OutT> __device__ __forceinline__ OutT cvt_out(const EpiArgs& e, float v) {
  if constexpr (__is_same(OutT, f16)) return from_f<OutT>(sat_f16(v, e.f16_max));
  else return from_f<OutT>(v);
}
template <int EPI, typename OutT>
__device__ __forceinline__ void epi_store(const EpiArgs& e, int m, int n, int M, int N, float acc) {
  if (m >= M || n >= N) return;
  float y = acc + (e.bias ? e.bias[n] : 0.f);
  if (EPI == LDMAE_EPI_BIAS) {
    OutT* C = (OutT*)e.C;
    if (e.beta != 0.f) y += e.beta * to_f<OutT>(C[(size_t)m * e.ldc + n]);
    C[(size_t)m * e.ldc + n] = cvt_out<OutT>(e, y);
  } else if (EPI == LDMAE_EPI_BIAS_POS) {
    y += e.xin[(size_t)(m % e.rows_per_batch) * N + n];
    ((OutT*)e.C)[(size_t)m * e.ldc + n] = cvt_out<OutT>(e, y);
  } else if (EPI == LDMAE_EPI_BIAS_GELU) {
    if (e.C2) ((OutT*)e.C2)[(size_t)m * e.ldc + n] = cvt_out<OutT>(e, y);
    ((OutT*)e.C)[(size_t)m * e.ldc + n] = cvt_out<OutT>(e, gelu_act<OutT>(y));
  } else if (EPI == LDMAE_EPI_GELU_BWD) {
    const size_t o = (size_t)m * e.ldc + n;
    ((OutT*)e.C)[o] = cvt_out<OutT>(e, gelu_bwd_val<OutT>(y, to_f<OutT>(((const OutT*)e.xin)[o])));
  } else {
    if (e.C) ((OutT*)e.C)[(size_t)m * e.ldc + n] = cvt_out<OutT>(e, y);
    const size_t o = (size_t)m * N + n;
    const float gt = e.gate ? e.gate[(size_t)(m / e.rows_per_batch) * e.gate_ld + n] : 1.f;
    e.xout[o] = fmaf(gt, act_round<OutT>(y), e.xin[o]);
  }
}

__device__ __forceinline__ int ring_f(int g) { return (0x78 >> (2 * g)) & 3; }

template <int EPI, typename OutT> struct Epi4 {
  const EpiArgs& e;
  int n, N;
  float4 bias, gate;
  __device__ __forceinline__ Epi4(const EpiArgs& e_, int m_first, int n_, int N_) : e(e_), n(n_), N(N_) {
    bias = e.bias ? *(const float4*)(e.bias + n) : make_float4(0.f, 0.f, 0.f, 0.f);
    gate = make_float4(1.f, 1.f, 1.f, 1.f);
    if (EPI == LDMAE_EPI_GATE_RES && e.gate) gate = *(const float4*)(e.gate + (size_t)(m_first / e.rows_per_batch) * e.gate_ld + n);
  }
  __device__ __forceinline__ void put(void* base, size_t off, float4 v) const {
    const float e_f16_max = e.f16_max;
    OutT* p = (OutT*)base + off;
    if constexpr (sizeof(OutT) == 4) *(float4*)p = v;
    else { if constexpr (__is_same(OutT, f16)) v = sat_f16(v, e_f16_max);
      typename Pack<OutT>::v4 o; o[0] = from_f<OutT>(v.x); o[1] = from_f<OutT>(v.y); o[2] = from_f<OutT>(v.z); o[3] = from_f<OutT>(v.w); *(typename Pack<OutT>::v4*)p = o; }
  }
  __device__ __forceinline__ void compute(int m, float4 a, float4& c, float4& c2) const {
    a.x += bias.x; a.y += bias.y; a.z += bias.z; a.w += bias.w;
    c = a; c2 = a;
    if (EPI == LDMAE_EPI_BIAS) {
      if (e.beta != 0.f) {
        const OutT* p = (const OutT*)e.C + (size_t)m * e.ldc + n;
        c.x += e.beta * to_f<OutT>(p[0]); c.y += e.beta * to_f<OutT>(p[1]); c.z += e.beta * to_f<OutT>(p[2]); c.w += e.beta * to_f<OutT>(p[3]);
      }
    } else if (EPI == LDMAE_EPI_BIAS_POS) {
      const float4 q = *(const float4*)(e.xin + (size_t)(m % e.rows_per_batch) * N + n);
      c = make_float4(a.x + q.x, a.y + q.y, a.z + q.z, a.w + q.w);
    } else if (EPI == LDMAE_EPI_BIAS_GELU) {
      auto g = [](float y) { return gelu_act<OutT>(y); };
      c = make_float4(g(a.x), g(a.y), g(a.z), g(a.w));
    } else if (EPI == LDMAE_EPI_GELU_BWD) {
      const OutT* p = (const OutT*)e.xin + (size_t)m * e.ldc + n;
      c = make_float4(gelu_bwd_val<OutT>(a.x, to_f<OutT>(p[0])), gelu_bwd_val<OutT>(a.y, to_f<OutT>(p[1])), gelu_bwd_val<OutT>(a.z, to_f<OutT>(p[2])),
                      gelu_bwd_val<OutT>(a.w, to_f<OutT>(p[3])));
    } else if (EPI == LDMAE_EPI_GATE_RES) {
      const size_t o = (size_t)m * N + n;
      const float4 xi = *(const float4*)(e.xin + o);
      *(float4*)(e.xout + o) = gate_res4(xi, gate, act_round4<OutT>(a));
    }
  }
  __device__ __forceinline__ void apply(int m, float4 a) const {
    a.x += bias.x; a.y += bias.y; a.z += bias.z; a.w += bias.w;
    const size_t oc = (size_t)m * e.ldc + n;
    if (EPI == LDMAE_EPI_BIAS) {
      if (e.beta != 0.f) {
        const OutT* p = (const OutT*)e.C + oc;
        a.x += e.beta * to_f<OutT>(p[0]); a.y += e.beta * to_f<OutT>(p[1]); a.z += e.beta * to_f<OutT>(p[2]); a.w += e.beta * to_f<OutT>(p[3]);
      }
      put(e.C, oc, a);
    } else if (EPI == LDMAE_EPI_BIAS_POS) {
      const float4 q = *(const float4*)(e.xin + (size_t)(m % e.rows_per_batch) * N + n);
      put(e.C, oc, make_float4(a.x + q.x, a.y + q.y, a.z + q.z, a.w + q.w));
    } else if (EPI == LDMAE_EPI_BIAS_GELU) {
      if (e.C2) put(e.C2, oc, a);
      auto g = [](float y) { return gelu_act<OutT>(y); };
      put(e.C, oc, make_float4(g(a.x), g(a.y), g(a.z), g(a.w)));
    } else if (EPI == LDMAE_EPI_GELU_BWD) {
      const OutT* p = (const OutT*)e.xin + oc;
      put(e.C, oc, make_float4(gelu_bwd_val<OutT>(a.x, to_f<OutT>(p[0])), gelu_bwd_val<OutT>(a.y, to_f<OutT>(p[1])),
                               gelu_bwd_val<OutT>(a.z, to_f<OutT>(p[2])), gelu_bwd_val<OutT>(a.w, to_f<OutT>(p[3]))));
    } else {
      if (e.C) put(e.C, oc, a);
      const size_t o = (size_t)m * N + n;
      const float4 xi = *(const float4*)(e.xin + o);
      *(float4*)(e.xout + o) = gate_res4(xi, gate, act_round4<OutT>(a));
    }
  }
};

struct NoHook { __device__ __forceinline__ void operator()(int, int) const {} };
template <int EPI, typename OutT, int TM, int TNn, int MI, int NI, typename Hook = NoHook>
__device__ __forceinline__ void nt_epilogue(f32x4 (&acc)[MI][NI], float* ew, float* ex, const EpiArgs& e, int m0, int n0, int wm, int wn,
                                            int lane, int M, int N, Hook consumed = Hook()) {
  constexpr int ELD = 68;
  auto fill = [&](int i, int cblk) {
#pragma unroll
    for (int j = 0; j < 4; ++j)
#pragma unroll
      for (int r = 0; r < 4; ++r) ew[((lane >> 4) * 4 + r) * ELD + j * 16 + (lane & 15)] = acc[i][cblk * 4 + j][r];
    consumed(i, cblk);
  };
  if constexpr (EPI == LDMAE_EPI_QKV_ROPE) {
    static_assert(TNn == 64 && sizeof(OutT) == 2, "EPI_QKV_ROPE: 64-column wave slices, bf16 outputs");
    const int nb = n0 + wn * TNn, c8 = (lane & 7) * 8, mw = m0 + wm * TM;
    const int which = nb / (e.heads * 64), hh = (nb >> 6) % e.heads;
    const int bsmp = mw / e.rows_per_batch, tok0 = mw - bsmp * e.rows_per_batch;
    const float4 b0 = e.bias ? *(const float4*)(e.bias + nb + c8) : make_float4(0.f, 0.f, 0.f, 0.f);
    const float4 b1 = e.bias ? *(const float4*)(e.bias + nb + c8 + 4) : make_float4(0.f, 0.f, 0.f, 0.f);
    const unsigned coff = ((unsigned)(lane >> 3) * (unsigned)e.ldc + (unsigned)(nb + c8)) * 2u;
    auto raw8 = [&](int i, int it, const bf16x8& o) {
      char* rb = (char*)e.C + (size_t)(mw + i * 16 + it * 8) * (size_t)e.ldc * 2;
      __builtin_nontemporal_store(o, (bf16x8*)(rb + coff));
    };
    auto round8 = [&](const float4& u, const float4& v) {
      bf16x8 o;
      o[0] = (bf16)(u.x + b0.x); o[1] = (bf16)(u.y + b0.y); o[2] = (bf16)(u.z + b0.z); o[3] = (bf16)(u.w + b0.w);
      o[4] = (bf16)(v.x + b1.x); o[5] = (bf16)(v.y + b1.y); o[6] = (bf16)(v.z + b1.z); o[7] = (bf16)(v.w + b1.w);
      return o;
    };
    if (which == 2) {
#pragma unroll
      for (int i = 0; i < MI; ++i) {
        fill(i, 0);
#pragma unroll
        for (int it = 0; it < 2; ++it) {
          const int row = it * 8 + (lane >> 3);
          raw8(i, it, round8(*(const float4*)(ew + row * ELD + c8), *(const float4*)(ew + row * ELD + c8 + 4)));
        }
      }
      return;
    }
    const bool norm = e.wq != nullptr;
    const float* wsel = which == 0 ? e.wq : e.wk;
// ... 293 lines not shown
```

### ldmae_amd/models/lightningdit.py

```python
from __future__ import annotations

import contextlib
import math

import numpy as np
import os

import torch
import torch.nn as nn
from torch.utils.checkpoint import checkpoint

from ldmae_amd import ops
from ldmae_amd.tables import sincos_2d
from .pos_embed import VisionRotaryEmbeddingFast
from .rmsnorm import RMSNorm
from .swiglu_ffn import SwiGLUFFN


def _act_dtype(override=None, allow_f16=False):
    if override is not None:
        return override
    if torch.is_autocast_enabled("cuda"):
        d = torch.get_autocast_dtype("cuda")
        if d == torch.float16 and allow_f16:
# ... 9 lines not shown
        return w, (ops.cast_weight(w, dtype, transposed=True, straight=False)[1] if transposed else None)
    if not transposed:
        return ops.cached_weight_copy(w, dtype), None
    return ops.cast_weight(w, dtype, transposed=True, straight=True)


class _SiluFn(torch.autograd.Function):

    @staticmethod
    def forward(ctx, c):
        c = c.contiguous()
        ctx.save_for_backward(c)
        return ops.silu_fwd(c)

    @staticmethod
    def backward(ctx, g):
        (c,) = ctx.saved_tensors
        return ops.silu_bwd(g.contiguous(), c)


class _LinearF32Fn(torch.autograd.Function):

    @staticmethod
    def forward(ctx, x, w, b):
        x = x.contiguous()
        ctx.save_for_backward(x, w)
        return ops.gemm_nt(x, w, b, out_dtype=torch.float32)

    @staticmethod
    def backward(ctx, g):
        x, w = ctx.saved_tensors
        g = g.contiguous()
        dx = ops.gemm_nt(g, ops.cast_weight(w, torch.float32, True, False)[1]) if ctx.needs_input_grad[0] else None
        return dx, ops.gemm_tn(g, x), ops.colsum(g)


class _TimestepFreqFn(torch.autograd.Function):
    @staticmethod
    def forward(ctx, t, dim):
        return ops.timestep_embedding(t, dim)

    @staticmethod
    def backward(ctx, g):
        return None, None


class _LabelEmbedFn(torch.autograd.Function):
    @staticmethod
    def forward(ctx, table, y, drop, num_classes):
        ctx.save_for_backward(y, drop)
        ctx.num_classes, ctx.rows = num_classes, table.shape[0]
        return ops.label_embed_fwd(table, y, drop, num_classes)

    @staticmethod
    def backward(ctx, g):
        y, drop = ctx.saved_tensors
        return ops.label_embed_bwd(g, y, drop, ctx.num_classes, ctx.rows), None, None, None


class _PatchEmbedFn(torch.autograd.Function):

    @staticmethod
    def forward(ctx, tok, w2d, b, pos, T, dtype=torch.float32, input_only=False):
        tok = tok.contiguous()
        ctx.input_only = bool(input_only)
        lowp = dtype == torch.bfloat16 and tok.shape[1] % 64 == 0 and tok.shape[0] % 64 == 0
        ctx.lowp = lowp
        if lowp:
            tok = ops.cast(tok, torch.bfloat16)
            ctx.save_for_backward(tok, w2d)
            return ops.gemm_nt_pos(tok, ops.cast(w2d.contiguous(), torch.bfloat16), b, pos, T)
        ctx.save_for_backward(tok, w2d)
        if tok.dtype == torch.float32 and ops.thin_ok(w2d.shape[0], tok.shape[1]):
            return ops.thin_nt(tok, w2d.float(), b, pos, T)
        return ops.gemm_nt_pos(tok, w2d, b, pos, T)

    @staticmethod
    def backward(ctx, g):
        tok, w2d = ctx.saved_tensors
        g = g.contiguous()
        if ctx.input_only:
            return ops.gemm_nt(g, ops.cast_weight(w2d, torch.float32, True, False)[1]), None, None, None, None, None, None
        dtok = ops.gemm_nt(g, ops.cast_weight(w2d, torch.float32, True, False)[1]) if ctx.needs_input_grad[0] else None
        if not ctx.lowp and g.dtype == torch.float32 and tok.dtype == torch.float32 and ops.thin_ok(g.shape[1], tok.shape[1]):
            dw, db = ops.thin_tn(g, tok)
            return dtok, dw, db, None, None, None, None
        dw = ops.gemm_tn(ops.cast(g, torch.bfloat16), tok) if ctx.lowp else ops.gemm_tn(g, tok)
        return dtok, dw, ops.colsum(g), None, None, None, None


def _dmod_times_w(dmod, adaw):
    if dmod.shape[0] % 4 == 0:
        return ops.gemm_tn(dmod.t().contiguous(), adaw)
    return ops.gemm_nt(dmod, ops.cast_weight(adaw, torch.float32, True, False)[1])


def _dw_into_grad(sg, dy, x, param, direct):
    g = param.grad if direct else None
    if g is not None and g.dtype == torch.float32 and g.is_contiguous() and g.shape == (dy.shape[1], x.shape[1]):
        sg.tn(dy, x, out=g, beta=1.0)
        ready = getattr(param, "_ldmae_grad_ready", None)
        return None, ready
    return sg.tn(dy, x), None


def _pad_swiglu(w12, b12, w3):
    Hs = w3.shape[1]
    Hp = (Hs + 127) // 128 * 128
    if Hp == Hs:
        return w12, b12, w3, Hs, Hp
    D = w3.shape[0]
    z = w12.new_zeros(Hp - Hs, D)
    w12p = torch.cat([w12[:Hs], z, w12[Hs:], z], 0)
    zb = b12.new_zeros(Hp - Hs)
    b12p = torch.cat([b12[:Hs], zb, b12[Hs:], zb], 0)
    w3p = torch.cat([w3, w3.new_zeros(D, Hp - Hs)], 1)
    return w12p, b12p, w3p, Hs, Hp


def _unpad_swiglu_grads(dW12, db12, dW3, Hs, Hp):
    if Hp == Hs:
        return dW12, db12, dW3
    cut = lambda t_: None if t_ is None else torch.cat([t_[:Hs], t_[Hp:Hp + Hs]], 0)
    return cut(dW12), cut(db12), (None if dW3 is None else dW3[:, :Hs].contiguous())


_FUSED_QKN_BWD = os.environ.get("LDMAE_FUSED_QKN_BWD", "1") != "0"

_QK_LN_EPS = 1e-5


def _qk_layernorm_fwd(qkv, qnw, qnb, knw, knb, cos, sin, B, N, H, hd, dtype):
    qs, ks, v = ops.heads_split(qkv, B, N, H, hd)
    q32, k32 = ops.cast(qs, torch.float32).view(-1, hd), ops.cast(ks, torch.float32).view(-1, hd)
    qn, muq, rsq = ops.layernorm_fwd(q32, qnw, qnb, dtype, _QK_LN_EPS)
    kn, muk, rsk = ops.layernorm_fwd(k32, knw, knb, dtype, _QK_LN_EPS)
    q, k = ops.rope(qn.view(B, H, N, hd), cos, sin), ops.rope(kn.view(B, H, N, hd), cos, sin)
    return q, k, v, (q32, k32, muq, rsq, muk, rsk)


def _qk_layernorm_bwd(dq, dk, dv, saved, qnw, knw, cos, sin, B, N, H, hd, dtype, with_bias=True):
    q32, k32, muq, rsq, muk, rsk = saved
    dxq, dxk = torch.zeros_like(q32), torch.zeros_like(k32)
    dqw, dqb = ops.layernorm_bwd(ops.rope(dq, cos, sin, transposed=True).view(-1, hd), q32, qnw, muq, rsq, dxq)
    dkw, dkb = ops.layernorm_bwd(ops.rope(dk, cos, sin, transposed=True).view(-1, hd), k32, knw, muk, rsk, dxk)
    dqkv = ops.heads_merge(ops.cast(dxq, dtype).view(B, H, N, hd), ops.cast(dxk, dtype).view(B, H, N, hd), dv, B, N, H, hd)
    return dqkv, dqw, dqb, dkw, dkb, (ops.colsum(dqkv) if with_bias else None)


class _GradChain:

    def __init__(self):
        self.up, self.pre = {}, {}
        self.dmod_all, self.mod_cols = None, 0

    def dmod(self, j, mod):
        if self.mod_cols == 0:
            return torch.empty(mod.shape, dtype=mod.dtype, device=mod.device)
        if self.dmod_all is None:
            self.dmod_all = torch.empty(mod.shape[0], self.mod_cols, dtype=torch.float32, device=mod.device)
        w = mod.shape[1]
        return self.dmod_all[:, j * w:(j + 1) * w]

    def norm_bwd(self, j, dout, x, w, scale, rstd, dx, dshift, dscale, N, dtype, accumulate=True):
        D = x.shape[1]
        prev = self.up.pop(j - 1, None)
        if prev is None:
            return ops.rmsnorm_modulate_bwd(dout, x, w, scale, rstd, dx, dshift, dscale, N, accumulate)
        y2p, modp = prev
        dmodp = self.dmod(j - 1, modp)
        gc = modp.shape[1] - D
        dw, dy2p, db3p = ops.rmsnorm_modulate_bwd_gate(dout, x, w, scale, rstd, dx, dshift, dscale, y2p, modp[:, gc:gc + D],
                                                       dmodp[:, gc:gc + D], N, dtype, accumulate)
        self.pre[j - 1] = (dx.data_ptr(), dy2p, db3p, dmodp)
        return dw


class _AdaLNAllFn(torch.autograd.Function):

    @staticmethod
    def forward(ctx, sc, fwd_only, *wb):
        n = len(wb) // 2
        ws, bs = wb[:n], wb[n:]
        scb = ops.cast(sc.contiguous(), torch.bfloat16)
        stack = ops.cached_stack_copy if fwd_only else ops.cast_stack
        W_all = stack(ws, torch.bfloat16)
        b_all = stack(bs, torch.float32)
        mod_all = ops.gemm_nt(scb, W_all, b_all, out_dtype=torch.float32)
        ctx.save_for_backward(scb, W_all)
        ctx.n, ctx.rows = n, ws[0].shape[0]
        return mod_all

    @staticmethod
    def backward(ctx, g):
        scb, W_all = ctx.saved_tensors
        n, rows = ctx.n, ctx.rows
        g = g.contiguous()
        gb = ops.cast(g, torch.bfloat16)
        dW_all = ops.gemm_tn(gb, scb)
        db_all = ops.colsum(g)
        dsc = ops.gemm_tn(gb.t().contiguous(), W_all) if ctx.needs_input_grad[0] else None
        return (dsc, None) + tuple(dW_all[i * rows:(i + 1) * rows] for i in range(n)) + tuple(db_all[i * rows:(i + 1) * rows] for i in range(n))


_MX8_FWD_ONLY = ("ldmae_amd LightningDiT: gemm_precision='mxfp8' is forward-only bf16 (sampling under torch.no_grad() with bfloat16 activations); "
                 "call set_gemm_precision(None) for a grad-enabled or float32 forward")


def _block_fwd_mx8(x2, B, N, D, H, hd, eps, cos, sin, sh1, s1, g1, sh2, s2, g2, n1w, qkvw, qkvb, qnw, knw, pw, pb, n2w, w12, b12, w3, b3):
    M = B * N
    Wqkv, Wp, W12, W3 = (ops.cached_weight_mx8(w) for w in (qkvw, pw, w12, w3))
    a1q, a1s, _ = ops.rmsnorm_modulate_fwd_mx8(x2, n1w, sh1, s1, N, eps)
    if ops.gemm_nt_qkv_rope_mx8_ok(a1q, Wqkv[0], B, N, H, hd):
        qkv, q, k = ops.gemm_nt_qkv_rope_mx8(a1q, a1s, Wqkv[0], Wqkv[1], qkvb, qnw, knw, cos, sin, B, N, H, hd, eps, store_raw_qk=False)
    else:
        qkv = ops.gemm_nt_mx8(a1q, a1s, Wqkv[0], Wqkv[1], qkvb)
        q, k, _ = ops.qknorm_rope_fwd(qkv, qnw, knw, cos, sin, B, N, H, hd, eps, copy_v=False)
    o, _ = ops.attention_fwd_pv(q, k, qkv, hd ** -0.5, bound=ops.qk_score_bound(qnw, knw, hd, hd ** -0.5) if qnw is not None else None)
    oq, osc = ops.mx8_quantize(o.view(M, D))
    xmid, _ = ops.gemm_nt_gate_res_mx8(oq, osc, Wp[0], Wp[1], pb, x2, g1, N)
    a2q, a2s, _ = ops.rmsnorm_modulate_fwd_mx8(xmid, n2w, sh2, s2, N, eps)
    _, hid = ops.gemm_nt_swiglu_mx8(a2q, a2s, W12[0], W12[1], b12)
    hq, hsc = ops.mx8_quantize(hid)
    xout, _ = ops.gemm_nt_gate_res_mx8(hq, hsc, W3[0], W3[1], b3, xmid, g2, N)
    return xout.view(B, N, D)


class _DiTBlockFn(torch.autograd.Function):

    @staticmethod
    def forward(ctx, x, sc, cos, sin, H, eps, dtype, inplace, chain, idx, direct, fwd_only, mod_all, swiglu,
                n1w, qkvw, qkvb, qnw, knw, qnb, knb, pw, pb, n2w, w12, b12, w3, b3, adaw, adab, input_only=False, gemm_precision=None):
        B, N, D = x.shape
        M, hd = B * N, D // H
        x2 = x.contiguous().view(M, D)
        sc = sc.contiguous()
        ctx.batched_ada = mod_all is not None
        nmod = adaw.shape[0] // D
        if mod_all is not None:
            mod = mod_all[:, idx * nmod * D:(idx + 1) * nmod * D]
        else:
            mod = ops.gemm_nt(sc, adaw, adab, out_dtype=torch.float32)
        if nmod == 6:
            sh1, s1, g1, sh2, s2, g2 = (mod[:, i * D:(i + 1) * D] for i in range(6))
        else:
            s1, g1, s2, g2 = (mod[:, i * D:(i + 1) * D] for i in range(4))
            sh1 = sh2 = None
        bwd = not fwd_only and any(ctx.needs_input_grad)
        if gemm_precision == "mxfp8":
            if not fwd_only or dtype != torch.bfloat16:
                raise RuntimeError(_MX8_FWD_ONLY)
            return _block_fwd_mx8(x2, B, N, D, H, hd, eps, cos, sin, sh1, s1, g1, sh2, s2, g2, n1w, qkvw, qkvb, qnw, knw, pw, pb, n2w, w12, b12, w3, b3)
        Wqkv, WqkvT = _wcopies(qkvw, dtype, bwd)
        Wp, WpT = _wcopies(pw, dtype, bwd)
        ctx.hs = None
        if swiglu and w3.shape[1] % 128 != 0:
            w12, b12, w3, Hs_, Hp_ = _pad_swiglu(w12, b12, w3)
            ctx.hs = (Hs_, Hp_)
        W12, W12T = _wcopies(w12, dtype, bwd)
        W3, W3T = _wcopies(w3, dtype, bwd)
        xm1, rstd1 = ops.rmsnorm_modulate_fwd(x2, n1w, sh1, s1, N, dtype, eps)
        qk_saved = None
        fused_qkv = qnb is None and dtype == torch.bfloat16 and ops.gemm_nt_qkv_rope_ok(xm1, Wqkv, B, N, H, hd)
        if not fused_qkv:
            qkv = ops.gemm_nt(xm1, Wqkv, qkvb)
        if qnb is not None:
            q, k, v, qk_saved = _qk_layernorm_fwd(qkv, qnw, qnb, knw, knb, cos, sin, B, N, H, hd, dtype)
            o, lse = ops.attention_fwd(q, k, v, hd ** -0.5)
        elif dtype == torch.bfloat16:
            if fused_qkv:
                qkv, q, k = ops.gemm_nt_qkv_rope(xm1, Wqkv, qkvb, qnw, knw, cos, sin, B, N, H, hd, eps, store_raw_qk=bwd)
                v = None
            else:
                q, k, v = ops.qknorm_rope_fwd(qkv, qnw, knw, cos, sin, B, N, H, hd, eps, copy_v=False)
            o, lse = ops.attention_fwd_pv(q, k, qkv, hd ** -0.5, bound=ops.qk_score_bound(qnw, knw, hd, hd ** -0.5) if qnw is not None else None)
        else:
            q, k, v = ops.qknorm_rope_fwd(qkv, qnw, knw, cos, sin, B, N, H, hd, eps)
            o, lse = ops.attention_fwd(q, k, v, hd ** -0.5)
        xmid, y1 = ops.gemm_nt_gate_res(o.view(M, D), Wp, pb, x2, g1, N, save_y=bwd)
        xm2, rstd2 = ops.rmsnorm_modulate_fwd(xmid, n2w, sh2, s2, N, dtype, eps)
        if swiglu:
            h12, hid = ops.gemm_nt_swiglu(xm2, W12, b12, save_h12=bwd)
        else:
            h12 = ops.gemm_nt(xm2, W12, b12)
            hid = ops.gelu_tanh_fwd(h12)
        xout, y2 = ops.gemm_nt_gate_res(hid, W3, b3, xmid, g2, N, save_y=bwd)
        if not bwd:
            return xout.view(B, N, D)
        ctx.input_only = bool(input_only)
        if input_only:
            ctx.save_for_backward(x2, cos, sin, mod, rstd1, qkv, q, k, v, o, lse, y1, xmid, rstd2, h12, y2, n1w, qnw, knw, n2w,
                                  WqkvT, WpT, W12T, W3T, *(qk_saved or ()))
            ctx.dims = (B, N, D, H, hd, eps, dtype)
            ctx.swiglu, ctx.qk_ln, ctx.nmod, ctx.inplace = bool(swiglu), qk_saved is not None, nmod, bool(inplace)
            ctx.chain, ctx.idx = chain, idx
            if chain is not None:
                chain.up[idx] = (y2, mod)
            return xout.view(B, N, D)
        ctx.save_for_backward(x2, sc, cos, sin, mod, rstd1, xm1, qkv, q, k, v, o, lse, y1, xmid, rstd2, xm2, h12, hid, y2,
                              n1w, qnw, knw, n2w, adaw, WqkvT, WpT, W12T, W3T, *(qk_saved or ()))
        ctx.dims = (B, N, D, H, hd, eps, dtype)
        ctx.swiglu, ctx.qk_ln = bool(swiglu), qk_saved is not None
        ctx.nmod = nmod
        ctx.inplace = bool(inplace)
        ctx.chain, ctx.idx = chain, idx
        ctx.direct, ctx.wparams = bool(direct), (qkvw, pw, w12, w3)
        ctx.sparams = (n1w, qkvb, qnw, knw, pb, n2w, b12, b3, qnb, knb) if direct else None
        if chain is not None:
            chain.up[idx] = (y2, mod)
        return xout.view(B, N, D)

    @staticmethod
    def _backward_input_only(ctx, gout):
        (x2, cos, sin, mod, rstd1, qkv, q, k, v, o, lse, y1, xmid, rstd2, h12, y2, n1w, qnw, knw, n2w, WqkvT, WpT, W12T, W3T) = ctx.saved_tensors[:24]
        qk_saved = ctx.saved_tensors[24:] if ctx.qk_ln else None
        B, N, D, H, hd, eps, dtype = ctx.dims
        M = B * N
        dx = gout.contiguous().view(M, D)
        if not ctx.inplace and dx.data_ptr() == gout.data_ptr():
            dx = dx.clone()
        chain, idx = ctx.chain, ctx.idx
        c_sh1, c_s1, c_g1, c_sh2, c_s2, c_g2 = (0, 1, 2, 3, 4, 5) if ctx.nmod == 6 else (None, 0, 1, None, 2, 3)
        col = lambda t_, c_: None if c_ is None else t_[:, c_ * D:(c_ + 1) * D]
        s1, g1, s2, g2 = col(mod, c_s1), col(mod, c_g1), col(mod, c_s2), col(mod, c_g2)
        pre = chain.pre.pop(idx, None) if chain is not None else None
        if pre is not None and pre[0] == dx.data_ptr():
            _, dy2, _, dmod = pre
        else:
            dmod = chain.dmod(idx, mod) if chain is not None else torch.empty(mod.shape, dtype=mod.dtype, device=mod.device)
            dy2 = ops.gate_bwd(dx, y2, g2, None, N, dtype)
        if ctx.swiglu:
            dh12 = ops.gemm_nt_swiglu_bwd(dy2, W3T, h12)
        else:
            dh12 = ops.gelu_tanh_bwd(ops.gemm_nt(dy2, W3T), h12)
        dxm2 = ops.gemm_nt(dh12, W12T)
        _, dy1, _ = ops.rmsnorm_modulate_bwd_gate(dxm2, xmid, n2w, s2, rstd2, dx, col(dmod, c_sh2), col(dmod, c_s2), y1, g1, col(dmod, c_g1), N, dtype)
        do = ops.gemm_nt(dy1, WpT)
        if qk_saved is not None:
            dq, dk, dv = ops.attention_bwd(q, k, v, o, do, lse, hd ** -0.5)
            dqkv = _qk_layernorm_bwd(dq, dk, dv, qk_saved, qnw, knw, cos, sin, B, N, H, hd, dtype, with_bias=False)[0]
        elif v is None and hd in (64, 128) and N % 64 == 0 and _FUSED_QKN_BWD:
            dqkv = ops.attention_bwd_pv_qknorm(q, k, qkv, o, do, lse, hd ** -0.5, qnw, knw, cos, sin, eps)[0]
        elif v is None:
            dq, dk, dqkv = ops.attention_bwd_pv(q, k, qkv, o, do, lse, hd ** -0.5)
            dqkv = ops.qknorm_rope_bwd(dq, dk, None, qkv, qnw, knw, cos, sin, B, N, H, hd, eps, dqkv=dqkv)[0]
        else:
            dq, dk, dv = ops.attention_bwd(q, k, v, o, do, lse, hd ** -0.5)
            dqkv = ops.qknorm_rope_bwd(dq, dk, dv, qkv, qnw, knw, cos, sin, B, N, H, hd, eps)[0]
        dxm1 = ops.gemm_nt(dqkv.view(M, 3 * D), WqkvT)
        if chain is not None:
            chain.norm_bwd(idx, dxm1, x2, n1w, s1, rstd1, dx, col(dmod, c_sh1), col(dmod, c_s1), N, dtype)
        else:
            ops.rmsnorm_modulate_bwd(dxm1, x2, n1w, s1, rstd1, dx, col(dmod, c_sh1), col(dmod, c_s1), N)
        return (dx.view(B, N, D),) + (None,) * 30

    @staticmethod
    def backward(ctx, gout):
        if ctx.input_only:
            return _DiTBlockFn._backward_input_only(ctx, gout)
        (x2, sc, cos, sin, mod, rstd1, xm1, qkv, q, k, v, o, lse, y1, xmid, rstd2, xm2, h12, hid, y2,
         n1w, qnw, knw, n2w, adaw, WqkvT, WpT, W12T, W3T) = ctx.saved_tensors[:29]
        qk_saved = ctx.saved_tensors[29:] if ctx.qk_ln else None
        B, N, D, H, hd, eps, dtype = ctx.dims
        M = B * N
        dx = gout.contiguous().view(M, D)
        if not ctx.inplace and dx.data_ptr() == gout.data_ptr():
            dx = dx.clone()
        chain, idx = ctx.chain, ctx.idx
        c_sh1, c_s1, c_g1, c_sh2, c_s2, c_g2 = (0, 1, 2, 3, 4, 5) if ctx.nmod == 6 else (None, 0, 1, None, 2, 3)
        col = lambda t_, c_: None if c_ is None else t_[:, c_ * D:(c_ + 1) * D]
        s1, g1, s2, g2 = col(mod, c_s1), col(mod, c_g1), col(mod, c_s2), col(mod, c_g2)
        sg = ops.SideGemms(dx.device, enabled=dtype == torch.bfloat16)
        pre = chain.pre.pop(idx, None) if chain is not None else None
        if pre is not None and pre[0] == dx.data_ptr():
            _, dy2, db3, dmod = pre
        else:
            dmod = chain.dmod(idx, mod) if chain is not None else torch.empty(mod.shape, dtype=mod.dtype, device=mod.device)
            dy2, db3 = ops.gate_bwd(dx, y2, g2, col(dmod, c_g2), N, dtype, with_bias=True)
        qkvw_p, pw_p, w12_p, w3_p = ctx.wparams
        notify = []
        dW3, r = _dw_into_grad(sg, dy2, hid, w3_p, ctx.direct); notify.append((r, w3_p))
        if ctx.swiglu:
            dh12, db12 = ops.gemm_nt_swiglu_bwd(dy2, W3T, h12, with_bias=True)
        else:
            dh12 = ops.gelu_tanh_bwd(ops.gemm_nt(dy2, W3T), h12)
            db12 = ops.colsum(dh12)
        dW12, r = _dw_into_grad(sg, dh12, xm2, w12_p, ctx.direct); notify.append((r, w12_p))
        dxm2 = ops.gemm_nt(dh12, W12T)
        dn2, dy1, dbp = ops.rmsnorm_modulate_bwd_gate(dxm2, xmid, n2w, s2, rstd2, dx, col(dmod, c_sh2), col(dmod, c_s2),
                                                      y1, g1, col(dmod, c_g1), N, dtype)
        dWp, r = _dw_into_grad(sg, dy1, o.view(M, D), pw_p, ctx.direct); notify.append((r, pw_p))
        do = ops.gemm_nt(dy1, WpT)
        dqnb = dknb = None
        if qk_saved is not None:
            dq, dk, dv = ops.attention_bwd(q, k, v, o, do, lse, hd ** -0.5)
            dqkv, dqn, dqnb, dkn, dknb, dbqkv = _qk_layernorm_bwd(dq, dk, dv, qk_saved, qnw, knw, cos, sin, B, N, H, hd, dtype)
        elif v is None and hd in (64, 128) and N % 64 == 0 and _FUSED_QKN_BWD:
            dqkv, dqn, dkn, dbqkv = ops.attention_bwd_pv_qknorm(q, k, qkv, o, do, lse, hd ** -0.5, qnw, knw, cos, sin, eps)
        elif v is None:
            dq, dk, dqkv = ops.attention_bwd_pv(q, k, qkv, o, do, lse, hd ** -0.5)
            dqkv, dqn, dkn, dbqkv = ops.qknorm_rope_bwd(dq, dk, None, qkv, qnw, knw, cos, sin, B, N, H, hd, eps, with_bias=True, dqkv=dqkv)
        else:
            dq, dk, dv = ops.attention_bwd(q, k, v, o, do, lse, hd ** -0.5)
            dqkv, dqn, dkn, dbqkv = ops.qknorm_rope_bwd(dq, dk, dv, qkv, qnw, knw, cos, sin, B, N, H, hd, eps, with_bias=True)
        dqkv = dqkv.view(M, 3 * D)
        dWqkv, r = _dw_into_grad(sg, dqkv, xm1, qkvw_p, ctx.direct); notify.append((r, qkvw_p))
        dxm1 = ops.gemm_nt(dqkv, WqkvT)
        if chain is not None:
            dn1 = chain.norm_bwd(idx, dxm1, x2, n1w, s1, rstd1, dx, col(dmod, c_sh1), col(dmod, c_s1), N, dtype)
        else:
            dn1 = ops.rmsnorm_modulate_bwd(dxm1, x2, n1w, s1, rstd1, dx, col(dmod, c_sh1), col(dmod, c_s1), N)
        dmod_all = None
        if ctx.batched_ada:
            dadaw = dadab = dsc = None
            if idx == 0:
                dmod_all = chain.dmod_all
        else:
            dadaw, dadab = ops.gemm_tn(dmod, sc), ops.colsum(dmod)
            dsc = _dmod_times_w(dmod, adaw)
        if ctx.hs is not None:
            dW12, db12, dW3 = _unpad_swiglu_grads(dW12, db12, dW3, *ctx.hs)
        sg.join()
        small = [dn1, dbqkv, dqn, dkn, dbp, dn2, db12, db3, dqnb, dknb]
        if ctx.sparams is not None:
            pairs = [(p_, g_) for p_, g_ in zip(ctx.sparams, small) if p_ is not None]
            if all(g_ is not None and p_.grad is not None and p_.grad.dtype == torch.float32 and p_.grad.is_contiguous() and p_.grad.shape == g_.shape
                   for p_, g_ in pairs):
                ops.multi_add_([p_.grad for p_, _ in pairs], [g_ for _, g_ in pairs])
                notify.extend((getattr(p_, "_ldmae_grad_ready", None), p_) for p_, _ in pairs)
                dn1 = dbqkv = dqn = dkn = dbp = dn2 = db12 = db3 = dqnb = dknb = None
        for r, p_ in notify:
            if r is not None:
                r(p_)
        return (dx.view(B, N, D), dsc, None, None, None, None, None, None, None, None, None, None, dmod_all, None,
                dn1, dWqkv, dbqkv, dqn, dkn, dqnb, dknb, dWp, dbp, dn2, dW12, db12, dW3, db3, dadaw, dadab, None)


class _AttentionFn(torch.autograd.Function):

    @staticmethod
    def forward(ctx, x, cos, sin, H, eps, dtype, qkvw, qkvb, qnw, knw, qnb, knb, pw, pb):
        B, N, D = x.shape
        M, hd = B * N, D // H
        xa = ops.cast(x.contiguous().view(M, D), dtype)
        Wqkv, WqkvT = _wcopies(qkvw, dtype, True)
        Wp, WpT = _wcopies(pw, dtype, True)
        qkv = ops.gemm_nt(xa, Wqkv, qkvb)
        qk_saved = None
        if qnb is not None:
            q, k, v, qk_saved = _qk_layernorm_fwd(qkv, qnw, qnb, knw, knb, cos, sin, B, N, H, hd, dtype)
            o, lse = ops.attention_fwd(q, k, v, hd ** -0.5)
        elif dtype == torch.bfloat16:
            q, k, v = ops.qknorm_rope_fwd(qkv, qnw, knw, cos, sin, B, N, H, hd, eps, copy_v=False)
            o, lse = ops.attention_fwd_pv(q, k, qkv, hd ** -0.5, bound=ops.qk_score_bound(qnw, knw, hd, hd ** -0.5) if qnw is not None else None)
        else:
            q, k, v = ops.qknorm_rope_fwd(qkv, qnw, knw, cos, sin, B, N, H, hd, eps)
            o, lse = ops.attention_fwd(q, k, v, hd ** -0.5)
        out = ops.gemm_nt(o.view(M, D), Wp, pb)
        ctx.save_for_backward(xa, cos, sin, qkv, q, k, v, o, lse, qnw, knw, WqkvT, WpT, *(qk_saved or ()))
        ctx.dims = (B, N, D, H, hd, eps, x.dtype)
        ctx.qk_ln = qk_saved is not None
        return out.view(B, N, D)

    @staticmethod
    def backward(ctx, g):
        xa, cos, sin, qkv, q, k, v, o, lse, qnw, knw, WqkvT, WpT = ctx.saved_tensors[:13]
        B, N, D, H, hd, eps, xdt = ctx.dims
        M = B * N
        dy = ops.cast(g.contiguous().view(M, D), xa.dtype)
        dWp, dbp = ops.gemm_tn(dy, o.view(M, D), with_bias=True)
        do = ops.gemm_nt(dy, WpT)
        dqnb = dknb = None
        if ctx.qk_ln:
            dq, dk, dv = ops.attention_bwd(q, k, v, o, do, lse, hd ** -0.5)
            dqkv, dqn, dqnb, dkn, dknb, dbqkv = _qk_layernorm_bwd(dq, dk, dv, ctx.saved_tensors[13:], qnw, knw, cos, sin, B, N, H, hd, xa.dtype)
        elif v is None:
            dq, dk, dqkv = ops.attention_bwd_pv(q, k, qkv, o, do, lse, hd ** -0.5)
            dqkv, dqn, dkn, dbqkv = ops.qknorm_rope_bwd(dq, dk, None, qkv, qnw, knw, cos, sin, B, N, H, hd, eps, with_bias=True, dqkv=dqkv)
        else:
            dq, dk, dv = ops.attention_bwd(q, k, v, o, do, lse, hd ** -0.5)
            dqkv, dqn, dkn, dbqkv = ops.qknorm_rope_bwd(dq, dk, dv, qkv, qnw, knw, cos, sin, B, N, H, hd, eps, with_bias=True)
        dqkv = dqkv.view(M, 3 * D)
        dWqkv = ops.gemm_tn(dqkv, xa)
        dx = ops.gemm_nt(dqkv, WqkvT).view(B, N, D).to(xdt) if ctx.needs_input_grad[0] else None
        return dx, None, None, None, None, None, dWqkv, dbqkv, dqn, dkn, dqnb, dknb, dWp, dbp


class _FinalLayerFn(torch.autograd.Function):

    @staticmethod
    def forward(ctx, x, sc, eps, dtype, chain, idx, nw, lw, lb, adaw, adab, input_only=False):
        B, N, D = x.shape
        ctx.input_only = bool(input_only)
        M = B * N
        x2 = x.contiguous().view(M, D)
        sc = sc.contiguous()
        ctx.chain, ctx.idx = chain, idx
        mod = ops.gemm_nt(sc, adaw, adab, out_dtype=torch.float32)
        xf, rstd = ops.rmsnorm_modulate_fwd(x2, nw, mod[:, :D], mod[:, D:], N, dtype, eps)
        out = ops.gemm_nt(xf, ops.cast(lw, dtype), lb, out_dtype=torch.float32)
        ctx.save_for_backward(x2, sc, mod, rstd, xf, nw, lw, adaw)
        ctx.dims = (B, N, D, dtype)
        return out.view(B, N, -1)

    @staticmethod
    def backward(ctx, gout):
        x2, sc, mod, rstd, xf, nw, lw, adaw = ctx.saved_tensors
        B, N, D, dtype = ctx.dims
        M = B * N
        g = gout.contiguous().view(M, -1)
        io = ctx.input_only
        if not io:
            ga = ops.cast(g, dtype)
            dlw, dlb = ops.gemm_tn(ga, xf), ops.colsum(g)
        if g.dtype == torch.float32 and ops.thin_ok(lw.shape[1], lw.shape[0]):
            dxf = ops.thin_nt(g, lw.float().t().contiguous(), out_dtype=dtype)
        else:
            dxf = ops.gemm_nt(g, ops.cast_weight(lw, torch.float32, True, False)[1], out_dtype=dtype)
        dx = torch.empty(M, D, dtype=torch.float32, device=g.device)
        dmod = torch.empty_like(mod)
        if ctx.chain is not None:
            dnw = ctx.chain.norm_bwd(ctx.idx, dxf, x2, nw, mod[:, D:], rstd, dx, dmod[:, :D], dmod[:, D:], N, dtype, accumulate=False)
        else:
            dnw = ops.rmsnorm_modulate_bwd(dxf, x2, nw, mod[:, D:], rstd, dx, dmod[:, :D], dmod[:, D:], N, accumulate=False)
        if io:
            return (dx.view(B, N, D),) + (None,) * 11
        dadaw, dadab = ops.gemm_tn(dmod, sc), ops.colsum(dmod)
        dsc = _dmod_times_w(dmod, adaw)
        return dx.view(B, N, D), dsc, None, None, None, None, dnw, dlw, dlb, dadaw, dadab, None


class PatchEmbed(nn.Module):

    def __init__(self, img_size=224, patch_size=16, in_chans=3, embed_dim=768, bias=True):
        super().__init__()
        self.img_size = (img_size, img_size)
        self.patch_size = (patch_size, patch_size)
        self.grid_size = (img_size // patch_size, img_size // patch_size)
        self.num_patches = self.grid_size[0] * self.grid_size[1]
        self.proj = nn.Conv2d(in_chans, embed_dim, kernel_size=patch_size, stride=patch_size, bias=bias)
        self.norm = nn.Identity()

    def tokens(self, x):
# ... 168 lines not shown
            pad = (-nout) % 16
            lw, lb = torch.nn.functional.pad(lw, (0, 0, 0, pad)), torch.nn.functional.pad(lb, (0, pad))
        out = _FinalLayerFn.apply(x.float(), sc, self.norm_final.eps, _dtype or _act_dtype(self.precision), _chain, _idx,
                                  self.norm_final.weight, lw, lb, self.adaLN_modulation[1].weight, self.adaLN_modulation[1].bias, _input_only)
        return out if out.shape[-1] == nout else out[..., :nout]


class LightningDiT(nn.Module):

    def __init__(self, input_size=32, patch_size=2, in_channels=32, hidden_size=1152, depth=28, num_heads=16, mlp_ratio=4.0,
                 class_dropout_prob=0.1, num_classes=1000, learn_sigma=False, use_qknorm=False, use_swiglu=False,
                 use_rope=False, use_rmsnorm=False, wo_shift=False, use_checkpoint=False):
        super().__init__()
        self.direct_param_grads = False
        env = os.environ.get("LDMAE_BATCHED_ADALN")
        self.batched_adaln = None if env is None else env != "0"
        self.learn_sigma = learn_sigma
        self.in_channels = in_channels
        self.out_channels = in_channels if not learn_sigma else in_channels * 2
        self.patch_size = patch_size
        self.num_heads = num_heads
        self.use_rope = use_rope
        self.use_rmsnorm = use_rmsnorm
        self.depth = depth
        self.hidden_size = hidden_size
        self.use_checkpoint = use_checkpoint
        self.x_embedder = PatchEmbed(input_size, patch_size, in_channels, hidden_size, bias=True)
        self.t_embedder = TimestepEmbedder(hidden_size)
        self.y_embedder = LabelEmbedder(num_classes, hidden_size, class_dropout_prob)
        num_patches = self.x_embedder.num_patches
        self.pos_embed = nn.Parameter(torch.zeros(1, num_patches, hidden_size), requires_grad=False)
        self.feat_rope = VisionRotaryEmbeddingFast(dim=hidden_size // num_heads // 2, pt_seq_len=input_size // patch_size) if use_rope else None
        self.blocks = nn.ModuleList([
            LightningDiTBlock(hidden_size, num_heads, mlp_ratio=mlp_ratio, use_qknorm=use_qknorm, use_swiglu=use_swiglu,
                              use_rmsnorm=use_rmsnorm, wo_shift=wo_shift) for _ in range(depth)])
        self.final_layer = FinalLayer(hidden_size, patch_size, self.out_channels, use_rmsnorm=use_rmsnorm)
        self.precision = None
        self._input_grad_only = False
        self.gemm_precision = None
        self.initialize_weights()

    def set_precision(self, dtype):
        self.precision = dtype
        for b in self.blocks:
            b.precision = dtype
            b.attn.precision = dtype
        self.final_layer.precision = dtype
        return self

    def set_gemm_precision(self, mode):
        if mode is not None:
            if mode != "mxfp8":
                raise ValueError(f"gemm_precision {mode!r}: None or 'mxfp8'")
            blk = self.blocks[0] if len(self.blocks) else None
            why = None
            if blk is not None and blk.attn.norm_args()[3] is not None:
                why = "an nn.LayerNorm QK-norm (use_qknorm without use_rmsnorm)"
            elif not self.use_rmsnorm:
                why = "use_rmsnorm=False (the LayerNorm blocks have no norm + quantise kernel)"
            elif blk is not None and not isinstance(blk.mlp, SwiGLUFFN):
                why = "use_swiglu=False (the timm Mlp blocks have no block-scaled GEMM epilogue)"
            elif self.hidden_size % 128 != 0:
                why = f"hidden size {self.hidden_size} is not a multiple of 128"
            elif blk is not None and blk.mlp.w3.weight.shape[1] % 128 != 0:
                why = (f"SwiGLU width {blk.mlp.w3.weight.shape[1]} is not a multiple of 128 (the padded 2730 / 4778 widths of LightningDiT-L and "
                       "LightningDiT-1p6B are not built in this mode)")
            if why is not None:
                raise NotImplementedError("ldmae_amd LightningDiT: gemm_precision='mxfp8' is not implemented for " + why)
        self.gemm_precision = mode
        for b in self.blocks:
            b.gemm_precision = mode
        return self

    @contextlib.contextmanager
    def input_grad_only(self, on=True):
        if on and self.gemm_precision is not None:
            raise RuntimeError(_MX8_FWD_ONLY)
        was, self._input_grad_only = self._input_grad_only, bool(on)
        try:
            yield self
        finally:
            self._input_grad_only = was

    def initialize_weights(self):
        def _basic_init(module):
            if isinstance(module, nn.Linear):
                torch.nn.init.xavier_uniform_(module.weight)
                if module.bias is not None:
                    nn.init.constant_(module.bias, 0)
        self.apply(_basic_init)
        pos_embed = get_2d_sincos_pos_embed(self.pos_embed.shape[-1], int(self.x_embedder.num_patches ** 0.5))
        self.pos_embed.data.copy_(torch.from_numpy(pos_embed).float().unsqueeze(0))
        w = self.x_embedder.proj.weight.data
        nn.init.xavier_uniform_(w.view([w.shape[0], -1]))
        nn.init.constant_(self.x_embedder.proj.bias, 0)
        nn.init.normal_(self.y_embedder.embedding_table.weight, std=0.02)
        nn.init.normal_(self.t_embedder.mlp[0].weight, std=0.02)
        nn.init.normal_(self.t_embedder.mlp[2].weight, std=0.02)
        for block in self.blocks:
            nn.init.constant_(block.adaLN_modulation[-1].weight, 0)
            nn.init.constant_(block.adaLN_modulation[-1].bias, 0)
        nn.init.constant_(self.final_layer.adaLN_modulation[-1].weight, 0)
        nn.init.constant_(self.final_layer.adaLN_modulation[-1].bias, 0)
        nn.init.constant_(self.final_layer.linear.weight, 0)
        nn.init.constant_(self.final_layer.linear.bias, 0)

    def unpatchify(self, x):
        c = self.out_channels
        p = self.x_embedder.patch_size[0]
        h = w = int(x.shape[1] ** 0.5)
        assert h * w == x.shape[1]
        x = x.reshape(shape=(x.shape[0], h, w, p, p, c))
        x = torch.einsum('nhwpqc->nchpwq', x)
        return x.reshape(shape=(x.shape[0], c, h * p, h * p))

    def forward(self, x, t=None, y=None):
        dtype = _act_dtype(self.precision)
        if dtype != torch.float32 and self.hidden_size % 64 != 0:
            dtype = torch.float32
        if self.gemm_precision is not None and (torch.is_grad_enabled() or dtype != torch.bfloat16):
            raise RuntimeError(_MX8_FWD_ONLY)
        io = self._input_grad_only and torch.is_grad_enabled()
        if io and self.use_checkpoint:
            raise NotImplementedError("ldmae_amd LightningDiT: input_grad_only with use_checkpoint is not implemented (nothing to recompute for: no parameter gradients)")
        with torch.autocast(device_type="cuda", enabled=False):
            if io:
                x = self.x_embedder(x, self.pos_embed[0], input_only=True)
                with torch.no_grad():
                    c = self.t_embedder(t) + self.y_embedder(y, self.training)
                    sc = _SiluFn.apply(c)
            else:
                x = self.x_embedder(x, self.pos_embed[0])
                t = self.t_embedder(t)
                y = self.y_embedder(y, self.training)
                c = t + y
                sc = _SiluFn.apply(c)
            hooked = [bool(m._forward_hooks or m._forward_pre_hooks or m._backward_hooks) for m in self.blocks]
            fl = self.final_layer
            chain = None
            if torch.is_grad_enabled() and not self.use_checkpoint and not any(hooked) and \
                    not (fl._forward_hooks or fl._forward_pre_hooks or fl._backward_hooks):
                chain = _GradChain()
            mod_all = None
            if self._use_batched_adaln() and dtype == torch.bfloat16 and not self.use_checkpoint and len(self.blocks) <= 64 and sc.shape[0] % 8 == 0 and \
                    (chain is not None or not torch.is_grad_enabled()):
                lins = [b.adaLN_modulation[1] for b in self.blocks]
                if io:
                    with torch.no_grad():
                        mod_all = _AdaLNAllFn.apply(sc, True, *[l.weight for l in lins], *[l.bias for l in lins])
                else:
                    mod_all = _AdaLNAllFn.apply(sc, not torch.is_grad_enabled(), *[l.weight for l in lins], *[l.bias for l in lins])
                if chain is not None:
                    chain.mod_cols = mod_all.shape[1]
            for i, block in enumerate(self.blocks):
                if self.use_checkpoint:
                    x = checkpoint(block, x, c, self.feat_rope, sc, dtype, not hooked[i], use_reentrant=True)
                else:
                    x = block(x, c, self.feat_rope, sc, dtype, not hooked[i], chain, i, self.direct_param_grads and chain is not None and not io, mod_all, io)
            x = self.final_layer(x, c, sc, dtype, chain, len(self.blocks), io)
            x = self.unpatchify(x)
            if self.learn_sigma:
                x, _ = x.chunk(2, dim=1)
        return x

    def _use_batched_adaln(self) -> bool:
        if self.batched_adaln is not None:
            return bool(self.batched_adaln)
        import torch.distributed as dist
        return not (dist.is_available() and dist.is_initialized() and dist.get_world_size() > 1 and torch.is_grad_enabled())

    def forward_with_cfg(self, x, t, y, cfg_scale, cfg_interval=None, cfg_interval_start=None):
        half = x[: len(x) // 2]
        combined = torch.cat([half, half], dim=0)
        model_out = self.forward(combined, t, y)
        eps, rest = model_out[:, :3], model_out[:, 3:]
        cond_eps, uncond_eps = torch.split(eps, len(eps) // 2, dim=0)
        half_eps = uncond_eps + cfg_scale * (cond_eps - uncond_eps)
        if cfg_interval is True:
            timestep = t[0]
            if timestep < cfg_interval_start:
                half_eps = cond_eps
        eps = torch.cat([half_eps, half_eps], dim=0)
        return torch.cat([eps, rest], dim=1)


def get_2d_sincos_pos_embed(embed_dim, grid_size, cls_token=False, extra_tokens=0):
    return sincos_2d(embed_dim, grid_size, np.float64, cls_token=bool(cls_token and extra_tokens > 0))


def LightningDiT_XL_1(**kw): return LightningDiT(depth=28, hidden_size=1152, patch_size=1, num_heads=16, **kw)
def LightningDiT_XL_2(**kw): return LightningDiT(depth=28, hidden_size=1152, patch_size=2, num_heads=16, **kw)
def LightningDiT_L_2(**kw): return LightningDiT(depth=24, hidden_size=1024, patch_size=2, num_heads=16, **kw)
def LightningDiT_B_1(**kw): return LightningDiT(depth=12, hidden_size=768, patch_size=1, num_heads=12, **kw)
def LightningDiT_B_2(**kw): return LightningDiT(depth=12, hidden_size=768, patch_size=2, num_heads=12, **kw)
def LightningDiT_1p0B_1(**kw): return LightningDiT(depth=24, hidden_size=1536, patch_size=1, num_heads=24, **kw)
def LightningDiT_1p0B_2(**kw): return LightningDiT(depth=24, hidden_size=1536, patch_size=2, num_heads=24, **kw)
def LightningDiT_1p6B_1(**kw): return LightningDiT(depth=28, hidden_size=1792, patch_size=1, num_heads=28, **kw)
def LightningDiT_1p6B_2(**kw): return LightningDiT(depth=28, hidden_size=1792, patch_size=2, num_heads=28, **kw)


LightningDiT_models = {
    'LightningDiT-B/1': LightningDiT_B_1, 'LightningDiT-B/2': LightningDiT_B_2,
    'LightningDiT-L/2': LightningDiT_L_2,
    'LightningDiT-XL/1': LightningDiT_XL_1, 'LightningDiT-XL/2': LightningDiT_XL_2,
    'LightningDiT-1p0B/1': LightningDiT_1p0B_1, 'LightningDiT-1p0B/2': LightningDiT_1p0B_2,
    'LightningDiT-1p6B/1': LightningDiT_1p6B_1, 'LightningDiT-1p6B/2': LightningDiT_1p6B_2,
}
```

### ldmae_amd/ops.py

```python
from __future__ import annotations

import ctypes
import os
import weakref

import torch

from . import _lib as L
from ._lib import (BF16, EPI_BIAS, EPI_BIAS_GELU, EPI_BIAS_POS, EPI_F16_INF, EPI_GATE_RES, EPI_GELU_BWD, EPI_HALF_LINES, EPI_SWIGLU, EPI_SWIGLU_BWD, EPI_TILE_LAUNCH, F32, call, dt,
                   ptr, stream)

mx8_launch_counts = L.mx8_launch_counts
launch_counts = L.launch_counts

_ws = {}


def workspace(nbytes: int, device, slot: str = "main") -> torch.Tensor:
    key = (device, slot, torch.cuda.current_stream(device).cuda_stream)
    n = max(1, (int(nbytes) + 3) // 4)
    t = _ws.get(key)
    if t is None or t.numel() < n:
        t = torch.empty(int(n * 1.25) + 1024, dtype=torch.float32, device=device)
        _ws[key] = t
# ... 40 lines not shown

def side_stream(device):
    st = _side.get(device)
    if st is None:
        st = torch.cuda.Stream(device=device)
        _side[device] = st
    return st


class SideGemms:

    def __init__(self, device, enabled=True):
        self.enabled = enabled and os.environ.get("LDMAE_TN_STREAM", "0") == "1"
        self.main = torch.cuda.current_stream(device)
        self.side = side_stream(device) if self.enabled else None

    def tn(self, a, b, out=None, beta=0.0):
        if not self.enabled:
            return gemm_tn(a, b, out=out, beta=beta)
        self.side.wait_stream(self.main)
        with torch.cuda.stream(self.side):
            return gemm_tn(a, b, out=out, beta=beta, ws_slot="tn_side")

    def join(self):
        if self.enabled:
            self.main.wait_stream(self.side)


_GEMM_MODE = "auto"
_AUTO_FLAG = None


def set_gemm_launch_mode(mode: str) -> None:
    global _GEMM_MODE
    if mode not in ("persistent", "tile", "auto"):
        raise ValueError(f"gemm launch mode {mode!r}: 'persistent', 'tile' or 'auto'")
    _GEMM_MODE = mode


_HALF_LINES = 0


def set_gemm_half_lines(on: bool) -> None:
    global _HALF_LINES
    _HALF_LINES = EPI_HALF_LINES if on else 0


def _launch_flag() -> int:
    global _AUTO_FLAG
    if _GEMM_MODE != "auto":
        return (EPI_TILE_LAUNCH if _GEMM_MODE == "tile" else 0) | _HALF_LINES
    if _AUTO_FLAG is not None:
        return _AUTO_FLAG | _HALF_LINES
    import torch.distributed as dist
    if not (dist.is_available() and dist.is_initialized()):
        return _HALF_LINES
    _AUTO_FLAG = EPI_TILE_LAUNCH if dist.get_world_size() > 1 else 0
    return _AUTO_FLAG | _HALF_LINES


def gemm_launch_mode() -> str:
    return "tile" if (_launch_flag() & EPI_TILE_LAUNCH) else "persistent"


def _grad_flag(dtype, grad) -> int:
    return EPI_F16_INF if (grad and dtype == torch.float16) else 0


def gemm_nt(a, b, bias=None, out_dtype=None, out=None, beta=0.0, grad=False):
    a, b = _pair(a, b, "gemm_nt")
    M, K = a.shape
    N = b.shape[0]
    bias = _arg(bias, "gemm_nt bias", torch.float32, (N,))
    if out is None:
        out = torch.empty(M, N, dtype=out_dtype or a.dtype, device=a.device)
    else:
        _arg(out, "gemm_nt out", out_dtype, (M, N), rows=True, out=True)
    call("ldmae_gemm_nt", dt(a.dtype), dt(out.dtype), EPI_BIAS | _launch_flag() | _grad_flag(out.dtype, grad), ptr(a), _ld(a), ptr(b), _ld(b), ptr(out), _ld(out),
         M, N, K, ptr(bias), float(beta), None, None, None, 0, 0, stream())
    return out


def gemm_nt_gate_res(a, b, bias, xin, gate, rows_per_batch, save_y=True, xout=None, y_dtype=None):
    a, b = _pair(a, b, "gemm_nt_gate_res")
    M, K = a.shape
    N = b.shape[0]
    if rows_per_batch <= 0 or M % rows_per_batch:
        raise RuntimeError(f"gemm_nt_gate_res: M={M} is not a multiple of rows_per_batch={rows_per_batch}")
    bias = _arg(bias, "gemm_nt_gate_res bias", torch.float32, (N,))
    xin = _arg(xin, "gemm_nt_gate_res xin", torch.float32, numel=M * N)
    gate = _arg(gate, "gemm_nt_gate_res gate", torch.float32, (M // rows_per_batch, N), rows=True)
    y_dtype = y_dtype or a.dtype
    y = torch.empty(M, N, dtype=y_dtype, device=a.device) if save_y else None
    if xout is None:
        xout = torch.empty(M, N, dtype=torch.float32, device=a.device)
    else:
        _arg(xout, "gemm_nt_gate_res xout", torch.float32, out=True, numel=M * N)
    call("ldmae_gemm_nt", dt(a.dtype), dt(y_dtype), EPI_GATE_RES | _launch_flag(), ptr(a), _ld(a), ptr(b), _ld(b), ptr(y), N,
         M, N, K, ptr(bias), 0.0, ptr(xin), ptr(xout), ptr(gate), _ld(gate) if gate is not None else 0, rows_per_batch, stream())
    return xout, y


def gemm_nt_pos(a, b, bias, pos, rows_per_batch):
    a, b = _pair(a, b, "gemm_nt_pos")
    M, K = a.shape
    N = b.shape[0]
    bias = _arg(bias, "gemm_nt_pos bias", torch.float32, (N,))
    pos = _arg(pos, "gemm_nt_pos pos", torch.float32, numel=rows_per_batch * N)
    out = torch.empty(M, N, dtype=torch.float32, device=a.device)
    call("ldmae_gemm_nt", dt(a.dtype), F32, EPI_BIAS_POS | _launch_flag(), ptr(a), _ld(a), ptr(b), _ld(b), ptr(out), N,
         M, N, K, ptr(bias), 0.0, ptr(pos), None, None, 0, rows_per_batch, stream())
    return out


def gemm_nt_gelu(a, b, bias, save_pre=True):
    a, b = _pair(a, b, "gemm_nt_gelu")
    M, K = a.shape
    N = b.shape[0]
    bias = _arg(bias, "gemm_nt_gelu bias", torch.float32, (N,))
    out = torch.empty(M, N, dtype=a.dtype, device=a.device)
    pre = torch.empty_like(out) if save_pre else None
    call("ldmae_gemm_nt", dt(a.dtype), dt(a.dtype), EPI_BIAS_GELU | _launch_flag(), ptr(a), _ld(a), ptr(b), _ld(b), ptr(out), N,
         M, N, K, ptr(bias), 0.0, None, ptr(pre), None, 0, 0, stream())
    return out, pre


def gemm_nt_gelu_bwd(dy, w2t, pre):
    dy, w2t = _pair(dy, w2t, "gemm_nt_gelu_bwd")
    M, K = dy.shape
    N = w2t.shape[0]
    pre = _arg(pre, "gemm_nt_gelu_bwd pre", dy.dtype, numel=M * N)
    out = torch.empty(M, N, dtype=dy.dtype, device=dy.device)
    call("ldmae_gemm_nt", dt(dy.dtype), dt(dy.dtype), EPI_GELU_BWD | _launch_flag() | _grad_flag(dy.dtype, True), ptr(dy), _ld(dy), ptr(w2t), _ld(w2t), ptr(out), N,
         M, N, K, None, 0.0, ptr(pre), None, None, 0, 0, stream())
    return out


def gemm_nt_swiglu(a, w12, b12, save_h12=True):
    a, w12 = _pair(a, w12, "gemm_nt_swiglu")
    M, K = a.shape
    N = w12.shape[0]
    b12 = _arg(b12, "gemm_nt_swiglu bias", torch.float32, (N,))
    if a.dtype == torch.bfloat16 and N % 256 == 0 and K % 64 == 0:
        h12 = torch.empty(M, N, dtype=a.dtype, device=a.device) if save_h12 else None
        hid = torch.empty(M, N // 2, dtype=a.dtype, device=a.device)
        call("ldmae_gemm_nt", BF16, BF16, EPI_SWIGLU | _launch_flag(), ptr(a), _ld(a), ptr(w12), _ld(w12), ptr(h12), N, M, N, K, ptr(b12), 0.0,
             None, ptr(hid), None, 0, 0, stream())
        return h12, hid
    h12 = gemm_nt(a, w12, b12)
    return h12, swiglu_fwd(h12)


FUSED_QKV = os.environ.get("LDMAE_FUSED_QKV", "1") != "0"


def gemm_nt_qkv_rope_ok(a, w, B, N, H, hd):
    if a.dtype != torch.bfloat16 or not FUSED_QKV or _HALF_LINES:
        return False
    if a.data_ptr() % 128 or w.data_ptr() % 128 or w.shape[0] != 3 * H * hd or a.stride(1) != 1 or w.stride(1) != 1:
        return False
    return bool(L.load().ldmae_gemm_nt_qkv_rope_ok(B, N, H, hd, a.shape[1], a.stride(0), w.stride(0)))


def gemm_nt_qkv_rope(a, w, bias, wq, wk, cos, sin, B, N, H, hd, eps=1e-6, store_raw_qk=True):
    a, w = _pair(a, w, "gemm_nt_qkv_rope")
    M, K = a.shape
    bias = _arg(bias, "gemm_nt_qkv_rope bias", torch.float32, (3 * H * hd,))
    qkv = torch.empty(M, 3 * H * hd, dtype=a.dtype, device=a.device)
    q2 = torch.empty(B, H, N, hd, dtype=a.dtype, device=a.device)
    k2 = torch.empty_like(q2)
    call("ldmae_gemm_nt_qkv_rope", ptr(a), _ld(a), ptr(w), _ld(w), ptr(bias), ptr(qkv), ptr(q2), ptr(k2), ptr(wq), ptr(wk), ptr(cos), ptr(sin),
         B, N, H, hd, K, eps, 1 if store_raw_qk else 0, 1 if (_launch_flag() & EPI_TILE_LAUNCH) else 0, stream())
    return qkv, q2, k2


def mx8_quantize(x):
    if x.dtype not in (torch.float32, torch.bfloat16) or x.dim() != 2:
        raise RuntimeError(f"mx8_quantize: a 2-D float32 or bfloat16 tensor, got {tuple(x.shape)} {x.dtype}")
    x = _arg(x, "mx8_quantize x", rows=True)
    M, K = x.shape
    if K % 128:
        raise RuntimeError(f"mx8_quantize: K={K} is not a multiple of 128")
    q = torch.empty(M, K, dtype=torch.uint8, device=x.device)
    sc = torch.empty(M, K // 32, dtype=torch.uint8, device=x.device)
    call("ldmae_mx8_quantize", dt(x.dtype), ptr(x), _ld(x), ptr(q), ptr(sc), M, K, stream())
    return q, sc


def rmsnorm_modulate_fwd_mx8(x, w, shift, scale, rows_per_batch, eps=1e-6):
    M, D = x.shape
    if w is None:
        raise RuntimeError("rmsnorm_modulate_fwd_mx8: needs the RMSNorm weight (the LayerNorm form is not built in this mode)")
    if D % 128:
        raise RuntimeError(f"rmsnorm_modulate_fwd_mx8: D={D} is not a multiple of 128")
    q = torch.empty(M, D, dtype=torch.uint8, device=x.device)
    sc = torch.empty(M, D // 32, dtype=torch.uint8, device=x.device)
    rstd = torch.empty(M, dtype=torch.float32, device=x.device)
    ld = shift.stride(0) if shift is not None else (scale.stride(0) if scale is not None else 0)
    call("ldmae_rmsnorm_modulate_fwd_mx8", ptr(x), ptr(w), ptr(shift), ptr(scale), ld, ptr(q), ptr(sc), ptr(rstd), M, D, rows_per_batch, eps, stream())
    return q, sc, rstd


def _mx8_pair(aq, asc, wq, wsc, what):
    for t, name in ((aq, "aq"), (asc, "a scales"), (wq, "wq"), (wsc, "w scales")):
        if t.dtype != torch.uint8 or t.dim() != 2:
            raise RuntimeError(f"{what} {name}: a 2-D uint8 tensor, got {tuple(t.shape)} {t.dtype}")
    if wq.shape[1] != aq.shape[1] or aq.shape[1] % 128:
        raise RuntimeError(f"{what}: operands {tuple(aq.shape)} and {tuple(wq.shape)} must be [M,K] and [N,K] with K % 128 == 0")
    K = aq.shape[1]
    aq, wq = _arg(aq, what + " aq", rows=True), _arg(wq, what + " wq", rows=True)
    asc = _arg(asc, what + " a scales", torch.uint8, (aq.shape[0], K // 32))
    wsc = _arg(wsc, what + " w scales", torch.uint8, (wq.shape[0], K // 32))
    return aq, asc, wq, wsc


def gemm_nt_mx8(aq, asc, wq, wsc, bias=None, out_dtype=torch.bfloat16, out=None):
    aq, asc, wq, wsc = _mx8_pair(aq, asc, wq, wsc, "gemm_nt_mx8")
    M, K = aq.shape
    N = wq.shape[0]
    bias = _arg(bias, "gemm_nt_mx8 bias", torch.float32, (N,))
    if out is None:
        out = torch.empty(M, N, dtype=out_dtype, device=aq.device)
    else:
        _arg(out, "gemm_nt_mx8 out", out_dtype, (M, N), rows=True, out=True)
    call("ldmae_gemm_nt_mx8", dt(out.dtype), EPI_BIAS | (_launch_flag() & EPI_TILE_LAUNCH), ptr(aq), ptr(asc), _ld(aq), ptr(wq), ptr(wsc), _ld(wq), ptr(out), _ld(out),
         M, N, K, ptr(bias), None, None, None, 0, 0, stream())
    return out


def gemm_nt_gate_res_mx8(aq, asc, wq, wsc, bias, xin, gate, rows_per_batch, save_y=False, xout=None, y_dtype=torch.bfloat16):
    aq, asc, wq, wsc = _mx8_pair(aq, asc, wq, wsc, "gemm_nt_gate_res_mx8")
    M, K = aq.shape
    N = wq.shape[0]
    if rows_per_batch <= 0 or M % rows_per_batch:
        raise RuntimeError(f"gemm_nt_gate_res_mx8: M={M} is not a multiple of rows_per_batch={rows_per_batch}")
    bias = _arg(bias, "gemm_nt_gate_res_mx8 bias", torch.float32, (N,))
    xin = _arg(xin, "gemm_nt_gate_res_mx8 xin", torch.float32, numel=M * N)
    gate = _arg(gate, "gemm_nt_gate_res_mx8 gate", torch.float32, (M // rows_per_batch, N), rows=True)
    y = torch.empty(M, N, dtype=y_dtype, device=aq.device) if save_y else None
    if xout is None:
        xout = torch.empty(M, N, dtype=torch.float32, device=aq.device)
    else:
        _arg(xout, "gemm_nt_gate_res_mx8 xout", torch.float32, out=True, numel=M * N)
    call("ldmae_gemm_nt_mx8", dt(y_dtype), EPI_GATE_RES | (_launch_flag() & EPI_TILE_LAUNCH), ptr(aq), ptr(asc), _ld(aq), ptr(wq), ptr(wsc), _ld(wq), ptr(y), N,
         M, N, K, ptr(bias), ptr(xin), ptr(xout), ptr(gate), _ld(gate) if gate is not None else 0, rows_per_batch, stream())
    return xout, y


def gemm_nt_swiglu_mx8(aq, asc, w12q, w12sc, b12, save_h12=False):
    aq, asc, w12q, w12sc = _mx8_pair(aq, asc, w12q, w12sc, "gemm_nt_swiglu_mx8")
    M, K = aq.shape
    N = w12q.shape[0]
    if N % 256:
        raise RuntimeError(f"gemm_nt_swiglu_mx8: N={N} (2 * hidden) is not a multiple of 256")
    b12 = _arg(b12, "gemm_nt_swiglu_mx8 bias", torch.float32, (N,))
    h12 = torch.empty(M, N, dtype=torch.bfloat16, device=aq.device) if save_h12 else None
    hid = torch.empty(M, N // 2, dtype=torch.bfloat16, device=aq.device)
    call("ldmae_gemm_nt_mx8", BF16, EPI_SWIGLU | (_launch_flag() & EPI_TILE_LAUNCH), ptr(aq), ptr(asc), _ld(aq), ptr(w12q), ptr(w12sc), _ld(w12q), ptr(h12), N,
         M, N, K, ptr(b12), None, ptr(hid), None, 0, 0, stream())
    return h12, hid


def gemm_nt_qkv_rope_mx8_ok(aq, wq, B, N, H, hd):
    if aq.dtype != torch.uint8 or wq.dtype != torch.uint8 or aq.dim() != 2 or wq.dim() != 2:
        return False
    if aq.data_ptr() % 128 or wq.data_ptr() % 128 or wq.shape[0] != 3 * H * hd or aq.stride(1) != 1 or wq.stride(1) != 1:
        return False
    return bool(L.load().ldmae_gemm_nt_qkv_rope_mx8_ok(B, N, H, hd, aq.shape[1], aq.stride(0), wq.stride(0)))


def gemm_nt_qkv_rope_mx8(aq, asc, wq, wsc, bias, nwq, nwk, cos, sin, B, N, H, hd, eps=1e-6, store_raw_qk=False):
    aq, asc, wq, wsc = _mx8_pair(aq, asc, wq, wsc, "gemm_nt_qkv_rope_mx8")
    M, K = aq.shape
    bias = _arg(bias, "gemm_nt_qkv_rope_mx8 bias", torch.float32, (3 * H * hd,))
    qkv = torch.empty(M, 3 * H * hd, dtype=torch.bfloat16, device=aq.device)
    q2 = torch.empty(B, H, N, hd, dtype=torch.bfloat16, device=aq.device)
    k2 = torch.empty_like(q2)
    call("ldmae_gemm_nt_qkv_rope_mx8", ptr(aq), ptr(asc), _ld(aq), ptr(wq), ptr(wsc), _ld(wq), ptr(bias), ptr(qkv), ptr(q2), ptr(k2), ptr(nwq), ptr(nwk),
         ptr(cos), ptr(sin), B, N, H, hd, K, eps, 1 if store_raw_qk else 0, 1 if (_launch_flag() & EPI_TILE_LAUNCH) else 0, stream())
    return qkv, q2, k2


def gemm_nt_swiglu_bwd(dy, w3t, h12, with_bias=False):
    dy, w3t = _pair(dy, w3t, "gemm_nt_swiglu_bwd")
    M, K = dy.shape
    Hs = w3t.shape[0]
    h12 = _arg(h12, "gemm_nt_swiglu_bwd h12", dy.dtype, numel=M * 2 * Hs)
    if dy.dtype == torch.bfloat16 and Hs % 8 == 0 and K % 64 == 0:
        dh12 = torch.empty(h12.shape, dtype=dy.dtype, device=dy.device)
        whole = M % 128 == 0 and Hs % 64 == 0
        part = (torch.empty if whole else torch.zeros)((M + 127) // 128, 2 * Hs, dtype=torch.float32, device=dy.device) if with_bias else None
        call("ldmae_gemm_nt", BF16, BF16, EPI_SWIGLU_BWD | _launch_flag(), ptr(dy), _ld(dy), ptr(w3t), _ld(w3t), ptr(dh12), 2 * Hs, M, Hs, K, None, 0.0,
             ptr(h12), ptr(part), None, 0, 0, stream())
        return (dh12, colsum(part)) if with_bias else dh12
    dh12 = swiglu_bwd(gemm_nt(dy, w3t), h12)
    return (dh12, colsum(dh12)) if with_bias else dh12


def gemm_tn(a, b, out=None, beta=0.0, with_bias=False, ws_slot="tn", dbias_out=None):
    if b.dtype != a.dtype or a.dim() != 2 or b.dim() != 2 or b.shape[0] != a.shape[0]:
        raise RuntimeError(f"gemm_tn: operands {tuple(a.shape)} {a.dtype} and {tuple(b.shape)} {b.dtype} must be [M,N] and [M,K] of one dtype")
    a, b = _arg(a, "gemm_tn a", rows=True), _arg(b, "gemm_tn b", rows=True)
    M, N = a.shape
    K = b.shape[1]
    if out is None:
        out = torch.empty(N, K, dtype=torch.float32, device=a.device)
        beta = 0.0
    else:
        _arg(out, "gemm_tn out", torch.float32, (N, K), out=True)
    if dbias_out is not None:
        if not with_bias:
            raise RuntimeError("gemm_tn: dbias_out must be a contiguous f32 [N] buffer and needs with_bias=True")
        dbias = _arg(dbias_out, "gemm_tn dbias_out", torch.float32, (N,), out=True)
    else:
        dbias = (torch.zeros if beta != 0.0 else torch.empty)(N, dtype=torch.float32, device=a.device) if with_bias else None
    d = dt(a.dtype)
    nb = max(L.load().ldmae_gemm_tn_workspace_bytes(d, M, N, K), L.load().ldmae_colsum_workspace_bytes(M, N) if with_bias else 0)
    ws = workspace(nb, a.device, ws_slot)
    call("ldmae_gemm_tn", d, ptr(a), _ld(a), ptr(b), _ld(b), ptr(out), ptr(dbias), M, N, K, float(beta), ptr(ws), ws.numel() * 4,
         stream())
    return (out, dbias) if with_bias else out


def colsum(x, out=None, beta=0.0):
    x = _arg(x, "colsum x", rows=True)
    M, N = x.shape
    if out is None:
        out = torch.empty(N, dtype=torch.float32, device=x.device)
        beta = 0.0
    else:
        _arg(out, "colsum out", torch.float32, (N,), out=True)
    ws = workspace(L.load().ldmae_colsum_workspace_bytes(M, N), x.device, "colsum")
    call("ldmae_colsum", dt(x.dtype), ptr(x), _ld(x), M, N, ptr(out), float(beta), ptr(ws), stream())
    return out


def cast_weight(w, dtype, transposed=True, straight=True):
    w = _arg(w, "cast_weight w", torch.float32)
    R, C = w.shape
    dst = torch.empty(R, C, dtype=dtype, device=w.device) if straight else None
    dstT = torch.empty(C, R, dtype=dtype, device=w.device) if transposed else None
    call("ldmae_cast_weight", dt(dtype), ptr(w), ptr(dst), ptr(dstT), R, C, stream())
    return dst, dstT


def cast(x, dtype):
    if x.dtype == dtype:
        return x
    out = torch.empty(x.shape, dtype=dtype, device=x.device)
    call("ldmae_cast", dt(x.dtype), dt(dtype), ptr(_c(x)), ptr(out), x.numel(), stream())
    return out


_THIN = os.environ.get("LDMAE_THIN_GEMM", "1") != "0"


def thin_ok(N, K):
    return _THIN and K in (16, 32) and N % 4 == 0


def thin_nt(t, w, bias=None, pos=None, rows_per_batch=0, out_dtype=torch.float32):
    M, K = t.shape
    N = w.shape[0]
    t, w = _arg(t, "thin_nt t", torch.float32), _arg(w, "thin_nt w", torch.float32, (N, K))
    bias = _arg(bias, "thin_nt bias", torch.float32, (N,))
    pos = _arg(pos, "thin_nt pos", torch.float32, numel=rows_per_batch * N)
    out = torch.empty(M, N, dtype=out_dtype, device=t.device)
    call("ldmae_thin_nt", dt(out_dtype), ptr(t), ptr(w), ptr(bias), ptr(pos), ptr(out), M, N, K,
         int(rows_per_batch), stream())
    return out


def thin_tn(g, t, with_bias=True):
    M, N = g.shape
    K = t.shape[1]
    g, t = _arg(g, "thin_tn g", torch.float32), _arg(t, "thin_tn t", torch.float32, (M, K))
    dW = torch.empty(N, K, dtype=torch.float32, device=g.device)
    db = torch.empty(N, dtype=torch.float32, device=g.device) if with_bias else None
    ws = workspace(L.load().ldmae_thin_tn_workspace_bytes(M, N, K), g.device)
    call("ldmae_thin_tn", ptr(g), ptr(t), ptr(dW), ptr(db), M, N, K, 0.0, ptr(ws), ws.numel() * 4, stream())
    return dW, db


def multi_add_(dsts, srcs):
    import ctypes
    k = len(dsts)
    srcs = [_c(s_) for s_ in srcs]
    for d_, s_ in zip(dsts, srcs):
        if d_.dtype != torch.float32 or s_.dtype != torch.float32 or d_.numel() != s_.numel() or not d_.is_contiguous():
            raise RuntimeError("multi_add_: contiguous f32 pairs of equal size expected")
    da = (ctypes.c_void_p * k)(*[d_.data_ptr() for d_ in dsts])
    sa = (ctypes.c_void_p * k)(*[s_.data_ptr() for s_ in srcs])
    na = (ctypes.c_long * k)(*[d_.numel() for d_ in dsts])
    call("ldmae_multi_add", k, da, sa, na, stream())


def cast_stack(tensors, dtype):
    import ctypes
    t0 = tensors[0]
    n_each = t0.numel()
    out = torch.empty((len(tensors) * t0.shape[0],) + tuple(t0.shape[1:]), dtype=dtype, device=t0.device)
    srcs = [_c(t) for t in tensors]
    if any(t.dtype != torch.float32 or t.numel() != n_each for t in srcs):
        raise RuntimeError("cast_stack: f32 tensors of one size expected")
    arr = (ctypes.c_void_p * len(srcs))(*[t.data_ptr() for t in srcs])
    call("ldmae_cast_stack", dt(dtype), arr, len(srcs), n_each, ptr(out), stream())
    return out


def rmsnorm_modulate_fwd(x, w, shift, scale, rows_per_batch, out_dtype, eps=1e-6):
    M, D = x.shape
    out = torch.empty(M, D, dtype=out_dtype, device=x.device)
    rstd = torch.empty(M, dtype=torch.float32, device=x.device)
    ld = shift.stride(0) if shift is not None else (scale.stride(0) if scale is not None else 0)
    if w is None:
        call("ldmae_layernorm_modulate_fwd", dt(out_dtype), ptr(x), ptr(shift), ptr(scale), ld, ptr(out), ptr(rstd), M, D, rows_per_batch, eps, stream())
        return out, rstd
    call("ldmae_rmsnorm_modulate_fwd", dt(out_dtype), ptr(x), ptr(w), ptr(shift), ptr(scale), ld, ptr(out), ptr(rstd), M, D,
         rows_per_batch, eps, stream())
    return out, rstd


def rmsnorm_modulate_bwd(dout, x, w, scale, rstd, dx_accum, dshift, dscale, rows_per_batch, accumulate=True):
    M, D = x.shape
    ws = workspace(L.load().ldmae_rmsnorm_modulate_bwd_workspace_bytes(M, D, rows_per_batch), x.device)
    dld = (dshift if dshift is not None else dscale).stride(0) if (dshift is not None or dscale is not None) else 0
    if w is None:
        call("ldmae_layernorm_modulate_bwd", dt(dout.dtype), ptr(dout), ptr(x), ptr(scale), scale.stride(0) if scale is not None else 0, ptr(rstd), ptr(dx_accum),
             1.0 if accumulate else 0.0, ptr(dshift), ptr(dscale), dld, M, D, rows_per_batch, ptr(ws), stream())
        return None
    dw = torch.empty(D, dtype=torch.float32, device=x.device)
    call("ldmae_rmsnorm_modulate_bwd", dt(dout.dtype), ptr(dout), ptr(x), ptr(w), ptr(scale), scale.stride(0) if scale is not None else 0,
         ptr(rstd), ptr(dx_accum), 1.0 if accumulate else 0.0, ptr(dshift), ptr(dscale), (dshift if dshift is not None else dscale).stride(0) if (dshift is not None or dscale is not None) else 0,
         ptr(dw), 0.0, M, D, rows_per_batch, ptr(ws), stream())
    return dw


def rmsnorm_modulate_bwd_gate(dout, x, w, scale, rstd, dx_accum, dshift, dscale, y, gate, dgate, rows_per_batch, act_dtype, accumulate=True):
    M, D = x.shape
    dy = torch.empty(M, D, dtype=act_dtype, device=x.device)
    dbias = torch.empty(D, dtype=torch.float32, device=x.device)
    ws = workspace(L.load().ldmae_rmsnorm_modulate_bwd_gate_workspace_bytes(M, D, rows_per_batch), x.device)
    if w is None:
        dld = (dshift if dshift is not None else dscale).stride(0) if (dshift is not None or dscale is not None) else 0
        call("ldmae_layernorm_modulate_bwd_gate", dt(dout.dtype), ptr(dout), ptr(x), ptr(scale), scale.stride(0) if scale is not None else 0, ptr(rstd),
             ptr(dx_accum), 1.0 if accumulate else 0.0, ptr(dshift), ptr(dscale), dld, ptr(y), ptr(gate), gate.stride(0), ptr(dy), ptr(dgate), dgate.stride(0),
             ptr(dbias), M, D, rows_per_batch, ptr(ws), stream())
        return None, dy, dbias
    dw = torch.empty(D, dtype=torch.float32, device=x.device)
    call("ldmae_rmsnorm_modulate_bwd_gate", dt(dout.dtype), ptr(dout), ptr(x), ptr(w), ptr(scale), scale.stride(0) if scale is not None else 0,
         ptr(rstd), ptr(dx_accum), 1.0 if accumulate else 0.0, ptr(dshift), ptr(dscale), (dshift if dshift is not None else dscale).stride(0) if (dshift is not None or dscale is not None) else 0, ptr(dw), 0.0,
         ptr(y), ptr(gate), gate.stride(0), ptr(dy), ptr(dgate), dgate.stride(0), ptr(dbias), M, D, rows_per_batch, ptr(ws), stream())
    return dw, dy, dbias


def qknorm_rope_fwd(qkv, wq, wk, cos, sin, B, N, H, hd, eps=1e-6, copy_v=True):
    q = torch.empty(B, H, N, hd, dtype=qkv.dtype, device=qkv.device)
    k = torch.empty_like(q)
    v = torch.empty_like(q) if copy_v else None
    call("ldmae_qknorm_rope_fwd", dt(qkv.dtype), ptr(qkv), ptr(wq), ptr(wk), ptr(cos), ptr(sin), ptr(q), ptr(k), ptr(v), B, N, H, hd, eps, stream())
    return q, k, v


def qknorm_rope_bwd(dq, dk, dv, qkv, wq, wk, cos, sin, B, N, H, hd, eps=1e-6, with_bias=False, dqkv=None):
    dqkv = torch.empty_like(qkv) if dqkv is None else dqkv
    dwq = torch.empty(hd, dtype=torch.float32, device=qkv.device) if wq is not None else None
    dwk = torch.empty_like(dwq) if wq is not None else None
    db = torch.empty(H, 3, hd, dtype=torch.float32, device=qkv.device) if with_bias else None
    ws = workspace(L.load().ldmae_qknorm_rope_bwd_workspace_bytes(B, N, H, hd), qkv.device)
    call("ldmae_qknorm_rope_bwd", dt(qkv.dtype), ptr(dq), ptr(dk), ptr(dv), ptr(qkv), ptr(wq), ptr(wk), ptr(cos), ptr(sin), ptr(dqkv),
         ptr(dwq), ptr(dwk), 0.0, ptr(db), B, N, H, hd, eps, ptr(ws), stream())
    if with_bias:
        return dqkv, dwq, dwk, db.permute(1, 0, 2).reshape(-1)
    return dqkv, dwq, dwk


def rope(t, cos, sin, transposed=False):
    N, hd = cos.shape
    if t.shape[-2:] != (N, hd):
        raise RuntimeError(f"rope: the last two dims of t {tuple(t.shape)} must be (N, head_dim) = {(N, hd)}")
    t = _c(t)
    out = torch.empty_like(t)
    call("ldmae_rope", dt(t.dtype), ptr(t), ptr(cos), ptr(sin), ptr(out), t.numel() // hd, N, hd, 1 if transposed else 0, stream())
    return out


_ATTN_HDS = (16, 32, 64, 72, 128)
_ATTN_HDS_F32 = (16, 32, 64, 72, 80, 96, 128)


def _attn_hds(dtype):
    return _ATTN_HDS_F32 if dtype == torch.float32 else _ATTN_HDS


def _attn_pad(hd: int, dtype=None) -> int:
    for h in _attn_hds(dtype):
        if h >= hd:
            return h
    raise RuntimeError(f"ldmae_amd attention: head_dim {hd} is above the largest instantiated kernel (128)")


def attention_fwd(q, k, v, scale):
    B, H, N, hd = q.shape
    if hd not in _attn_hds(q.dtype):
        P = _attn_pad(hd, q.dtype)
        pad = lambda t: torch.nn.functional.pad(t, (0, P - hd))
        o, lse = attention_fwd(pad(q), pad(k), pad(v), scale)
        return o.view(B, N, H, P)[..., :hd].reshape(B, N, H * hd), lse
    o = torch.empty(B, N, H * hd, dtype=q.dtype, device=q.device)
    lse = torch.empty(B, H, N, dtype=torch.float32, device=q.device)
    call("ldmae_attention_fwd", dt(q.dtype), ptr(q), ptr(k), ptr(v), ptr(o), ptr(lse), B, H, N, hd, float(scale), stream())
    return o, lse


def attention_bwd(q, k, v, o, do, lse, scale):
    B, H, N, hd = q.shape
    if hd not in _attn_hds(q.dtype):
        P = _attn_pad(hd, q.dtype)
        pad, padt = (lambda t: torch.nn.functional.pad(t, (0, P - hd))), (lambda t: torch.nn.functional.pad(t.reshape(B, N, H, hd), (0, P - hd)).reshape(B, N, H * P))
        dq, dk, dv = attention_bwd(pad(q), pad(k), pad(v), padt(o), padt(_c(do)), lse, scale)
        return dq[..., :hd].contiguous(), dk[..., :hd].contiguous(), dv[..., :hd].contiguous()
    dq, dk, dv = torch.empty_like(q), torch.empty_like(q), torch.empty_like(q)
    delta = torch.empty(2, B, H, (N + 63) // 64 * 64, dtype=torch.float32, device=q.device)
    call("ldmae_attention_bwd", dt(q.dtype), ptr(q), ptr(k), ptr(v), ptr(o), ptr(_c(do)), ptr(lse), ptr(dq), ptr(dk), ptr(dv), ptr(delta),
         B, H, N, hd, float(scale), stream())
    return dq, dk, dv


def qk_score_bound(wq, wk, hd, scale):
    out = torch.empty(1, dtype=torch.float32, device=wq.device)
    call("ldmae_qk_score_bound", ptr(wq), ptr(wk), hd, float(scale), ptr(out), stream())
    return out


def attention_fwd_pv(q, k, qkv, scale, bound=None):
    B, H, N, hd = q.shape
    o = torch.empty(B, N, H * hd, dtype=q.dtype, device=q.device)
    lse = torch.empty(B, H, N, dtype=torch.float32, device=q.device)
    if bound is not None:
        call("ldmae_attention_fwd_pv_bounded", dt(q.dtype), ptr(q), ptr(k), ptr(qkv), ptr(o), ptr(lse), ptr(bound), B, H, N, hd, float(scale), stream())
    else:
        call("ldmae_attention_fwd_pv", dt(q.dtype), ptr(q), ptr(k), ptr(qkv), ptr(o), ptr(lse), B, H, N, hd, float(scale), stream())
    return o, lse


def attention_bwd_pv(q, k, qkv, o, do, lse, scale):
    B, H, N, hd = q.shape
    dq, dk = torch.empty_like(q), torch.empty_like(q)
    dqkv = torch.empty_like(qkv)
    delta = torch.empty(2, B, H, (N + 63) // 64 * 64, dtype=torch.float32, device=q.device)
    call("ldmae_attention_bwd_pv", dt(q.dtype), ptr(q), ptr(k), ptr(qkv), ptr(o), ptr(_c(do)), ptr(lse), ptr(dq), ptr(dk), ptr(dqkv), ptr(delta),
         B, H, N, hd, float(scale), stream())
    return dq, dk, dqkv


def attention_bwd_pv_qknorm(q, k, qkv, o, do, lse, scale, wq, wk, cos, sin, eps=1e-6):
    B, H, N, hd = q.shape
    dqkv = torch.empty_like(qkv)
    if wq is not None:
        dw2 = torch.empty(2 * hd, dtype=torch.float32, device=q.device)
        dwq, dwk = dw2[:hd], dw2[hd:]
    else:
        dwq = dwk = None
    db = torch.empty(3 * H * hd, dtype=torch.float32, device=q.device)
    ws = workspace(L.load().ldmae_attention_bwd_pv_qknorm_workspace_bytes(B, H, N, hd), q.device)
    call("ldmae_attention_bwd_pv_qknorm", dt(q.dtype), ptr(q), ptr(k), ptr(qkv), ptr(o), ptr(_c(do)), ptr(lse), ptr(wq), ptr(wk), ptr(cos),
         ptr(sin), float(eps), ptr(dqkv), ptr(dwq), ptr(dwk), ptr(db), ptr(ws), B, H, N, hd, float(scale), stream())
    return dqkv, dwq, dwk, db


BOUNDED_ATTENTION_MIN_SCORES = int(os.environ.get("LDMAE_BOUNDED_ATTN_MIN", 1 << 31))


def attention_fwd_qkv(qkv, B, N, H, hd, scale):
    if hd not in _attn_hds(qkv.dtype):
        return attention_fwd(*heads_split(qkv, B, N, H, hd), scale)
    o = torch.empty(B, N, H * hd, dtype=qkv.dtype, device=qkv.device)
    lse = torch.empty(B, H, N, dtype=torch.float32, device=qkv.device)
    if qkv.dtype == torch.bfloat16 and hd <= 32 and N >= 512 and B * H * N * N >= BOUNDED_ATTENTION_MIN_SCORES:
        kmax = torch.empty(B * H, 2, dtype=torch.float32, device=qkv.device)
        call("ldmae_k_norm_max", ptr(qkv), ptr(kmax), B, N, H, hd, stream())
        call("ldmae_attention_fwd_qkv_bounded", dt(qkv.dtype), ptr(qkv), ptr(o), ptr(lse), ptr(kmax), B, H, N, hd, float(scale), stream())
    else:
        call("ldmae_attention_fwd_qkv", dt(qkv.dtype), ptr(qkv), ptr(o), ptr(lse), B, H, N, hd, float(scale), stream())
    return o, lse


def attention_bwd_qkv(qkv, o, do, lse, B, N, H, hd, scale):
    if hd not in _attn_hds(qkv.dtype):
        q, k, v = heads_split(qkv, B, N, H, hd)
        return heads_merge(*attention_bwd(q, k, v, o, do, lse, scale), B, N, H, hd)
    dqkv = torch.empty_like(qkv)
    delta = torch.empty(2, B, H, (N + 63) // 64 * 64, dtype=torch.float32, device=qkv.device)
    call("ldmae_attention_bwd_qkv", dt(qkv.dtype), ptr(qkv), ptr(o), ptr(_c(do)), ptr(lse), ptr(dqkv), ptr(delta), B, H, N, hd, float(scale), stream())
    return dqkv


def swiglu_fwd(h12):
    M, H2 = h12.shape
    hid = torch.empty(M, H2 // 2, dtype=h12.dtype, device=h12.device)
    call("ldmae_swiglu_fwd", dt(h12.dtype), ptr(h12), ptr(hid), M, H2 // 2, stream())
    return hid

# ... 1071 lines not shown
```

Measured before the change: 1308 images/s.

## Fuse gated residual adds into next RMSNorm-modulate and recompute xmid in backward

Replaces the per-block GEMM-with-gated-residual epilogues with plain GEMMs, followed by a fused kernel that applies both gated residual updates and computes the next block's RMSNorm-modulate output. The fp32 mid-block residual (xmid) is no longer stored. The backward gate kernel rebuilds it from x, y1 and the gate, which saves fp32 activation writes and separate norm passes. The cost is extra reads of the branch outputs, and a forward norm result handed between blocks through a pointer-keyed chain dict, which adds bookkeeping and some fragility.

```diff
diff --git a/include/ldmae_hip.h b/include/ldmae_hip.h
--- a/include/ldmae_hip.h
+++ b/include/ldmae_hip.h
@@ -63,6 +63,13 @@
                                     const float* rstd, float* dx_accum, float beta_x, float* dshift, float* dscale, int dmod_ld, float* dw,
                                     float beta_w, const void* y, const float* gate, int gate_ld, void* dy, float* dgate, int dgate_ld,
                                     float* dbias, int M, int D, int rows_per_batch, float* workspace, void* stream);
+int ldmae_rmsnorm_modulate_bwd_gate_recompute(int dtype, const void* dout, const float* x, const float* w, const float* scale, int mod_ld,
+                                              const float* rstd, float* dx_accum, float beta_x, float* dshift, float* dscale, int dmod_ld,
+                                              float* dw, float beta_w, const void* y, const float* gate, int gate_ld, void* dy, float* dgate,
+                                              int dgate_ld, float* dbias, int M, int D, int rows_per_batch, float* workspace, void* stream);
+int ldmae_res_rmsnorm_modulate_fwd(int dtype, const float* x, const void* ya, const float* gate_a, int gate_a_ld, const void* yb,
+                                   const float* gate_b, int gate_b_ld, float* xout, const float* w, const float* shift, const float* scale,
+                                   int mod_ld, void* out, float* rstd, int M, int D, int rows_per_batch, float eps, void* stream);
 int ldmae_layernorm_modulate_fwd(int out_dtype, const float* x, const float* shift, const float* scale, int mod_ld, void* out, float* rstd,
                                  int M, int D, int rows_per_batch, float eps, void* stream);
 int ldmae_layernorm_modulate_bwd(int dtype, const void* dout, const float* x, const float* scale, int mod_ld, const float* rstd, float* dx_accum,
diff --git a/ldmae_amd/_lib.py b/ldmae_amd/_lib.py
--- a/ldmae_amd/_lib.py
+++ b/ldmae_amd/_lib.py
@@ -39,6 +39,9 @@
     "ldmae_rmsnorm_modulate_bwd_gate_workspace_bytes": (_l, [_i, _i, _i]),
     "ldmae_rmsnorm_modulate_bwd_gate": (_i, [_i, _vp, _vp, _vp, _vp, _i, _vp, _vp, _f, _vp, _vp, _i, _vp, _f, _vp, _vp, _i, _vp, _vp, _i, _vp,
                                              _i, _i, _i, _vp, _vp]),
+    "ldmae_rmsnorm_modulate_bwd_gate_recompute": (_i, [_i, _vp, _vp, _vp, _vp, _i, _vp, _vp, _f, _vp, _vp, _i, _vp, _f, _vp, _vp, _i, _vp, _vp, _i,
+                                                       _vp, _i, _i, _i, _vp, _vp]),
+    "ldmae_res_rmsnorm_modulate_fwd": (_i, [_i, _vp, _vp, _vp, _i, _vp, _vp, _i, _vp, _vp, _vp, _vp, _i, _vp, _vp, _i, _i, _i, _f, _vp]),
     "ldmae_qknorm_rope_fwd": (_i, [_i, _vp, _vp, _vp, _vp, _vp, _vp, _vp, _vp, _i, _i, _i, _i, _f, _vp]),
     "ldmae_qknorm_rope_bwd_workspace_bytes": (_l, [_i, _i, _i, _i]),
     "ldmae_qknorm_rope_bwd": (_i, [_i, _vp, _vp, _vp, _vp, _vp, _vp, _vp, _vp, _vp, _vp, _vp, _f, _vp, _i, _i, _i, _i, _f, _vp, _vp]),
diff --git a/ldmae_amd/csrc/common.h b/ldmae_amd/csrc/common.h
--- a/ldmae_amd/csrc/common.h
+++ b/ldmae_amd/csrc/common.h
@@ -142,6 +142,10 @@
   return make_float4(t.x * c.x - t.y * s.x, t.y * c.y + t.x * s.y, t.z * c.z - t.w * s.z, t.w * c.w + t.z * s.w);
 }
 
+__device__ __forceinline__ float4 gate_res4(float4 x, float4 g, float4 y) {
+  return make_float4(fmaf(g.x, y.x, x.x), fmaf(g.y, y.y, x.y), fmaf(g.z, y.z, x.z), fmaf(g.w, y.w, x.w));
+}
+
 __device__ __forceinline__ unsigned xcd_remap(unsigned bid, unsigned nwg) {
   const unsigned q = nwg >> 3, r = nwg & 7, x = bid & 7, i = bid >> 3;
   return (x < r ? x * (q + 1) : r * (q + 1) + (x - r) * q) + i;
diff --git a/ldmae_amd/csrc/elementwise.hip b/ldmae_amd/csrc/elementwise.hip
--- a/ldmae_amd/csrc/elementwise.hip
+++ b/ldmae_amd/csrc/elementwise.hip
@@ -15,6 +15,10 @@
 template <> __device__ __forceinline__ void store4<bf16>(bf16* p, float4 v) {
   bf16x4 o; o[0] = (bf16)v.x; o[1] = (bf16)v.y; o[2] = (bf16)v.z; o[3] = (bf16)v.w;
   __builtin_nontemporal_store(o, (bf16x4*)p);
+}
+template <> __device__ __forceinline__ void store4<f16>(f16* p, float4 v) {
+  f16x4 o; o[0] = from_f<f16>(v.x); o[1] = from_f<f16>(v.y); o[2] = from_f<f16>(v.z); o[3] = from_f<f16>(v.w);
+  *(f16x4*)p = o;
 }
 __device__ __forceinline__ float4 f4(float a) { return make_float4(a, a, a, a); }
 __device__ __forceinline__ float4 operator+(float4 a, float4 b) { return make_float4(a.x + b.x, a.y + b.y, a.z + b.z, a.w + b.w); }
@@ -145,8 +149,106 @@
   }
 }
 
-struct GateBwdArgs { const void* y; const float* gate; int gate_ld; void* dy; float* Pg; float* Pb; int dx_overwrite; int center; };
-template <int NCH, typename T, bool GATE, bool FULL = false>
+template <bool FMA> __device__ __forceinline__ float sumsq4_guarded(float4 a) {
+#pragma clang fp contract(off)
+  if constexpr (FMA) return fmaf(a.x, a.x, a.y * a.y) + fmaf(a.z, a.z, a.w * a.w);
+  else return (a.x * a.x + a.y * a.y) + (a.z * a.z + a.w * a.w);
+}
+
+template <int NCH, typename T, bool FULL = false>
+__global__ __launch_bounds__(256) void res_rmsnorm_mod_fwd_kernel(const float* __restrict__ x, const T* __restrict__ ya,
+                                                                  const float* __restrict__ ga, int ga_ld, const T* __restrict__ yb,
+                                                                  const float* __restrict__ gb, int gb_ld, float* __restrict__ xout,
+                                                                  const float* __restrict__ w, const float* __restrict__ shift,
+                                                                  const float* __restrict__ scale, int mod_ld, T* __restrict__ out,
+                                                                  float* __restrict__ rstd, int M, int D, int rpb, float eps) {
+  const int lane = threadIdx.x & 63, wave = threadIdx.x >> 6, nch = D >> 2;
+  float4 wv[NCH];
+#pragma unroll
+  for (int i = 0; i < NCH; ++i) { const int c = lane + 64 * i; wv[i] = (c < nch && out) ? *(const float4*)(w + 4 * c) : f4(0.f); }
+  if constexpr (FULL) {
+    const int m0 = (blockIdx.x * 4 + wave) * 4, b = m0 / rpb;
+    float4 sc1[NCH], sh[NCH], gav[NCH], gbv[NCH];
+#pragma unroll
+    for (int i = 0; i < NCH; ++i) {
+      sc1[i] = scale ? f4(1.f) + *(const float4*)(scale + (size_t)b * mod_ld + 4 * lane + 256 * i) : f4(1.f);
+      sh[i] = shift ? *(const float4*)(shift + (size_t)b * mod_ld + 4 * lane + 256 * i) : f4(0.f);
+      gav[i] = *(const float4*)(ga + (size_t)b * ga_ld + 4 * lane + 256 * i);
+      gbv[i] = yb ? *(const float4*)(gb + (size_t)b * gb_ld + 4 * lane + 256 * i) : f4(0.f);
+    }
+    for (int r = 0; r < 4; ++r) {
+      const int m = m0 + r;
+      const size_t ro = (size_t)m * D + 4 * lane;
+      float4 xv[NCH], yav[NCH], ybv[NCH];
+      float ss = 0.f;
+#pragma unroll
+      for (int i = 0; i < NCH; ++i) xv[i] = *(const float4*)(x + ro + 256 * i);
+#pragma unroll
+      for (int i = 0; i < NCH; ++i) { yav[i] = load4<T>(ya + ro + 256 * i); ybv[i] = yb ? load4<T>(yb + ro + 256 * i) : f4(0.f); }
+#pragma unroll
+      for (int i = 0; i < NCH; ++i) {
+        xv[i] = gate_res4(xv[i], gav[i], yav[i]);
+        if (yb) xv[i] = gate_res4(xv[i], gbv[i], ybv[i]);
+        if (xout) *(float4*)(xout + ro + 256 * i) = xv[i];
+      }
+      if (!out) continue;
+#pragma unroll
+      for (int i = 0; i < NCH; ++i) ss += hsum(xv[i] * xv[i]);
+      ss = wave_sum(ss);
+      const float rs = rsqrtf(ss / (float)D + eps);
+      if (lane == 0 && rstd) rstd[m] = rs;
+#pragma unroll
+      for (int i = 0; i < NCH; ++i) {
+        float4 y = (xv[i] * rs) * wv[i];
+        if (scale) y = y * sc1[i];
+        if (shift) y = y + sh[i];
+        store4<T>(out + ro + 256 * i, y);
+      }
+    }
+    return;
+  }
+  for (int r = 0; r < 4; ++r) {
+    const int m = (blockIdx.x * 4 + wave) * 4 + r;
+    if (m >= M) return;
+    const int b = m / rpb;
+    float4 xv[NCH], yav[NCH], ybv[NCH];
+    float ss = 0.f;
+#pragma unroll
+    for (int i = 0; i < NCH; ++i) {
+      const int c = lane + 64 * i;
+      xv[i] = c < nch ? *(const float4*)(x + (size_t)m * D + 4 * c) : f4(0.f);
+      yav[i] = c < nch ? load4<T>(ya + (size_t)m * D + 4 * c) : f4(0.f);
+      ybv[i] = (c < nch && yb) ? load4<T>(yb + (size_t)m * D + 4 * c) : f4(0.f);
+    }
+#pragma unroll
+    for (int i = 0; i < NCH; ++i) {
+      const int c = lane + 64 * i;
+      if (c < nch) {
+        xv[i] = gate_res4(xv[i], *(const float4*)(ga + (size_t)b * ga_ld + 4 * c), yav[i]);
+        if (yb) xv[i] = gate_res4(xv[i], *(const float4*)(gb + (size_t)b * gb_ld + 4 * c), ybv[i]);
+        if (xout) *(float4*)(xout + (size_t)m * D + 4 * c) = xv[i];
+      }
+      ss += sumsq4_guarded<(NCH > 1)>(xv[i]);
+    }
+    if (!out) continue;
+    ss = wave_sum(ss);
+    const float rs = rsqrtf(ss / (float)D + eps);
+    if (lane == 0 && rstd) rstd[m] = rs;
+#pragma unroll
+    for (int i = 0; i < NCH; ++i) {
+      const int c = lane + 64 * i;
+      if (c < nch) {
+        float4 y = (xv[i] * rs) * wv[i];
+        if (scale) y = y * (f4(1.f) + *(const float4*)(scale + (size_t)b * mod_ld + 4 * c));
+        if (shift) y = y + *(const float4*)(shift + (size_t)b * mod_ld + 4 * c);
+        store4<T>(out + (size_t)m * D + 4 * c, y);
+      }
+    }
+  }
+}
+
+struct GateBwdArgs { const void* y; const float* gate; int gate_ld; void* dy; float* Pg; float* Pb; int dx_overwrite; int center; int recompute; };
+template <int NCH, typename T, bool GATE, bool FULL = false, bool RECOMP = false>
 __global__ __launch_bounds__(256) void rmsnorm_mod_bwd_kernel(const T* __restrict__ dout, const float* __restrict__ x,
                                                               const float* __restrict__ w, const float* __restrict__ scale, int mod_ld,
                                                               const float* __restrict__ rstd, float* __restrict__ dx, float* __restrict__ P,
@@ -186,11 +288,14 @@
       const size_t ro = (size_t)m * D + 4 * lane;
       float4 g[NCH], nv[NCH], dold[NCH], yv[GATE ? NCH : 1];
 #pragma unroll
-      for (int i = 0; i < NCH; ++i) { g[i] = load4<T>(dout + ro + 256 * i); nv[i] = *(const float4*)(x + ro + 256 * i); }
+      for (int i = 0; i < NCH; ++i) {
+        g[i] = load4<T>(dout + ro + 256 * i); nv[i] = *(const float4*)(x + ro + 256 * i);
+        if constexpr (RECOMP) yv[i] = load4<T>(gy + ro + 256 * i);
+      }
 #pragma unroll
       for (int i = 0; i < NCH; ++i) {
         dold[i] = ga.dx_overwrite ? f4(0.f) : *(const float4*)(dx + ro + 256 * i);
-        if constexpr (GATE) yv[i] = load4<T>(gy + ro + 256 * i);
+        if constexpr (GATE && !RECOMP) yv[i] = load4<T>(gy + ro + 256 * i);
       }
       const float rs = rstd[m];
       float4 dn[NCH];
@@ -199,6 +304,7 @@
       for (int i = 0; i < NCH; ++i) {
         const int c = lane + 64 * i;
         const float4 wc = GATE ? *(const float4*)(cw + 4 * c) : wv[i], sc = GATE ? *(const float4*)(cs + 4 * c) : sc1[i];
+        if constexpr (RECOMP) nv[i] = gate_res4(nv[i], *(const float4*)(cg + 4 * c), yv[i]);
         nv[i] = nv[i] * rs;
         const float4 dy = g[i] * sc;
         a_sh[i] = a_sh[i] + g[i];
@@ -241,7 +347,9 @@
       if (c < nch) {
         const float4 g = load4<T>(dout + (size_t)m * D + 4 * c);
         const float4 wc = GATE ? *(const float4*)(cw + 4 * c) : wv[i], sc = GATE ? *(const float4*)(cs + 4 * c) : sc1[i];
-        nv[i] = (*(const float4*)(x + (size_t)m * D + 4 * c) - f4(mean)) * rs;
+        float4 xr = *(const float4*)(x + (size_t)m * D + 4 * c);
+        if constexpr (RECOMP) xr = gate_res4(xr, *(const float4*)(cg + 4 * c), load4<T>(gy + (size_t)m * D + 4 * c));
+        nv[i] = (xr - f4(mean)) * rs;
         const float4 dy = g * sc;
         a_sh[i] = a_sh[i] + g;
         a_sc[i] = a_sc[i] + g * (nv[i] * wc);
@@ -365,6 +473,32 @@
 extern "C" int ldmae_rmsnorm_modulate_fwd(int out_dtype, const float* x, const float* w, const float* shift, const float* scale,
                                           int mod_ld, void* out, float* rstd, int M, int D, int rows_per_batch, float eps, void* stream) {
   return norm_modulate_fwd(out_dtype, x, w, shift, scale, mod_ld, out, rstd, M, D, rows_per_batch, eps, 0, stream);
+}
+extern "C" int ldmae_res_rmsnorm_modulate_fwd(int dtype, const float* x, const void* ya, const float* gate_a, int gate_a_ld, const void* yb,
+                                              const float* gate_b, int gate_b_ld, float* xout, const float* w, const float* shift,
+                                              const float* scale, int mod_ld, void* out, float* rstd, int M, int D, int rows_per_batch, float eps,
+                                              void* stream) {
+  LDMAE_REQUIRE(dtype == LDMAE_BF16 || dtype == LDMAE_F16, "res_rmsnorm_modulate_fwd: dtype %d (bf16 or fp16 activations only)", dtype);
+  LDMAE_REQUIRE(x && ya && gate_a && (xout || out) && M > 0 && D > 0, "res_rmsnorm_modulate_fwd: null pointer or empty");
+  LDMAE_REQUIRE((yb != nullptr) == (gate_b != nullptr), "res_rmsnorm_modulate_fwd: yb and gate_b go together");
+  LDMAE_REQUIRE(!out || w, "res_rmsnorm_modulate_fwd: the norm needs its weight");
+  LDMAE_REQUIRE(out || (!rstd && !shift && !scale), "res_rmsnorm_modulate_fwd: rstd / shift / scale without a norm output");
+  LDMAE_REQUIRE(xout != x, "res_rmsnorm_modulate_fwd: xout must not alias x");
+  LDMAE_REQUIRE(D % 4 == 0 && gate_a_ld % 4 == 0 && (!yb || gate_b_ld % 4 == 0) && (mod_ld % 4 == 0 || (!shift && !scale)),
+                "res_rmsnorm_modulate_fwd: D=%d gate_ld=%d/%d mod_ld=%d must be multiples of 4", D, gate_a_ld, gate_b_ld, mod_ld);
+  LDMAE_REQUIRE(rows_per_batch > 0 && M % rows_per_batch == 0, "res_rmsnorm_modulate_fwd: M=%d %% rows_per_batch=%d != 0", M, rows_per_batch);
+  const uintptr_t al = (uintptr_t)x | (uintptr_t)ya | (uintptr_t)gate_a | (uintptr_t)yb | (uintptr_t)gate_b | (uintptr_t)xout | (uintptr_t)w |
+                       (uintptr_t)shift | (uintptr_t)scale | (uintptr_t)out;
+  LDMAE_REQUIRE(al % 16 == 0, "res_rmsnorm_modulate_fwd: every tensor must be 16-byte aligned");
+  hipStream_t st = as_stream(stream);
+  const unsigned grid = cdiv(M, 16);
+  const bool full = dtype == LDMAE_BF16 && D % 256 == 0 && M % 16 == 0 && rows_per_batch % 16 == 0;
+#define RES_LAUNCH(T, FULLV) DISPATCH_NCH(D, hipLaunchKernelGGL((res_rmsnorm_mod_fwd_kernel<NCH, T, FULLV>), dim3(grid), dim3(256), 0, st, x, (const T*)ya, gate_a, gate_a_ld, (const T*)yb, gate_b, gate_b_ld, xout, w, shift, scale, mod_ld, (T*)out, rstd, M, D, rows_per_batch, eps))
+  if (dtype == LDMAE_BF16) { if (full) { RES_LAUNCH(bf16, true); } else { RES_LAUNCH(bf16, false); } }
+  else { RES_LAUNCH(f16, false); }
+#undef RES_LAUNCH
+  LDMAE_CHECK_LAUNCH("res_rmsnorm_modulate_fwd");
+  return LDMAE_OK;
 }
 extern "C" int ldmae_layernorm_modulate_fwd(int out_dtype, const float* x, const float* shift, const float* scale, int mod_ld, void* out,
                                             float* rstd, int M, int D, int rows_per_batch, float eps, void* stream) {
@@ -403,7 +537,15 @@
   if (center && !dw) dw = P;
 #define LAUNCH(T, GATE) DISPATCH_NCH(D, hipLaunchKernelGGL((rmsnorm_mod_bwd_kernel<NCH, T, GATE>), dim3(G), dim3(256), lds, st, (const T*)dout, x, w, scale, mod_ld, rstd, dx_accum, P, M, D, rows_per_batch, rw, ga))
 #define LAUNCH_FULL(T, GATE) DISPATCH_NCH(D, hipLaunchKernelGGL((rmsnorm_mod_bwd_kernel<NCH, T, GATE, true>), dim3(G), dim3(256), lds, st, (const T*)dout, x, w, scale, mod_ld, rstd, dx_accum, P, M, D, rows_per_batch, rw, ga))
-  if (dtype == LDMAE_BF16 && D % 256 == 0 && !center) { if (gate) { LAUNCH_FULL(bf16, true); } else { LAUNCH_FULL(bf16, false); } }
+  if (gate && gate->recompute) {
+    LDMAE_REQUIRE(dtype == LDMAE_BF16 && !center, "rmsnorm_modulate_bwd_gate_recompute: bf16 activations and the RMSNorm form only");
+    if (D % 256 == 0) {
+      DISPATCH_NCH(D, hipLaunchKernelGGL((rmsnorm_mod_bwd_kernel<NCH, bf16, true, true, true>), dim3(G), dim3(256), lds, st, (const bf16*)dout, x, w, scale, mod_ld, rstd, dx_accum, P, M, D, rows_per_batch, rw, ga));
+    } else {
+      DISPATCH_NCH(D, hipLaunchKernelGGL((rmsnorm_mod_bwd_kernel<NCH, bf16, true, false, true>), dim3(G), dim3(256), lds, st, (const bf16*)dout, x, w, scale, mod_ld, rstd, dx_accum, P, M, D, rows_per_batch, rw, ga));
+    }
+  }
+  else if (dtype == LDMAE_BF16 && D % 256 == 0 && !center) { if (gate) { LAUNCH_FULL(bf16, true); } else { LAUNCH_FULL(bf16, false); } }
   else if (dtype == LDMAE_BF16) { if (gate) { LAUNCH(bf16, true); } else { LAUNCH(bf16, false); } }
   else { if (gate) { LAUNCH(float, true); } else { LAUNCH(float, false); } }
 #undef LAUNCH
@@ -441,6 +583,16 @@
   LDMAE_REQUIRE(y && gate && dy && dgate && dbias, "rmsnorm_modulate_bwd_gate: null pointer");
   LDMAE_REQUIRE(gate_ld % 4 == 0, "rmsnorm_modulate_bwd_gate: gate_ld=%d must be a multiple of 4", gate_ld);
   const GateBwdArgs ga{y, gate, gate_ld, dy, nullptr, nullptr, 0, 0};
+  return rmsnorm_modulate_bwd_core(dtype, dout, x, w, scale, mod_ld, rstd, dx_accum, beta_x, dshift, dscale, dmod_ld, dw, beta_w, M, D, rows_per_batch,
+                                   workspace, &ga, dgate, dgate_ld, dbias, stream);
+}
+extern "C" int ldmae_rmsnorm_modulate_bwd_gate_recompute(int dtype, const void* dout, const float* x, const float* w, const float* scale, int mod_ld,
+                                                         const float* rstd, float* dx_accum, float beta_x, float* dshift, float* dscale, int dmod_ld,
+                                                         float* dw, float beta_w, const void* y, const float* gate, int gate_ld, void* dy, float* dgate,
+                                                         int dgate_ld, float* dbias, int M, int D, int rows_per_batch, float* workspace, void* stream) {
+  LDMAE_REQUIRE(y && gate && dy && dgate && dbias, "rmsnorm_modulate_bwd_gate_recompute: null pointer");
+  LDMAE_REQUIRE(gate_ld % 4 == 0, "rmsnorm_modulate_bwd_gate_recompute: gate_ld=%d must be a multiple of 4", gate_ld);
+  const GateBwdArgs ga{y, gate, gate_ld, dy, nullptr, nullptr, 0, 0, 1};
   return rmsnorm_modulate_bwd_core(dtype, dout, x, w, scale, mod_ld, rstd, dx_accum, beta_x, dshift, dscale, dmod_ld, dw, beta_w, M, D, rows_per_batch,
                                    workspace, &ga, dgate, dgate_ld, dbias, stream);
 }
diff --git a/ldmae_amd/csrc/gemm_nt_common.h b/ldmae_amd/csrc/gemm_nt_common.h
--- a/ldmae_amd/csrc/gemm_nt_common.h
+++ b/ldmae_amd/csrc/gemm_nt_common.h
@@ -41,9 +41,6 @@
 #endif
 
 template <typename OutT> __device__ __forceinline__ float act_round(float y) { return to_f<OutT>(from_f<OutT>(y)); }
-__device__ __forceinline__ float4 gate_res4(float4 x, float4 g, float4 y) {
-  return make_float4(fmaf(g.x, y.x, x.x), fmaf(g.y, y.y, x.y), fmaf(g.z, y.z, x.z), fmaf(g.w, y.w, x.w));
-}
 template <typename OutT> __device__ __forceinline__ float4 act_round4(float4 y) {
   return make_float4(act_round<OutT>(y.x), act_round<OutT>(y.y), act_round<OutT>(y.z), act_round<OutT>(y.w));
 }
diff --git a/ldmae_amd/models/lightningdit.py b/ldmae_amd/models/lightningdit.py
--- a/ldmae_amd/models/lightningdit.py
+++ b/ldmae_amd/models/lightningdit.py
@@ -185,6 +185,7 @@
 
     def __init__(self):
         self.up, self.pre = {}, {}
+        self.nxt, self.fwd = {}, {}
         self.dmod_all, self.mod_cols = None, 0
 
     def dmod(self, j, mod):
@@ -292,7 +293,14 @@
             ctx.hs = (Hs_, Hp_)
         W12, W12T = _wcopies(w12, dtype, bwd)
         W3, W3T = _wcopies(w3, dtype, bwd)
-        xm1, rstd1 = ops.rmsnorm_modulate_fwd(x2, n1w, sh1, s1, N, dtype, eps)
+        resnorm = (ops.FUSED_RESNORM and dtype == torch.bfloat16 and n1w is not None and n2w is not None and mod_all is not None and
+                   chain is not None and bwd and not input_only)
+        ctx.resnorm = resnorm
+        handed = chain.fwd.pop(idx, None) if chain is not None else None
+        if handed is not None and handed[0] == x2.data_ptr():
+            xm1, rstd1 = handed[1], handed[2]
+        else:
+            xm1, rstd1 = ops.rmsnorm_modulate_fwd(x2, n1w, sh1, s1, N, dtype, eps)
         qk_saved = None
         fused_qkv = qnb is None and dtype == torch.bfloat16 and ops.gemm_nt_qkv_rope_ok(xm1, Wqkv, B, N, H, hd)
         if not fused_qkv:
@@ -310,14 +318,30 @@
         else:
             q, k, v = ops.qknorm_rope_fwd(qkv, qnw, knw, cos, sin, B, N, H, hd, eps)
             o, lse = ops.attention_fwd(q, k, v, hd ** -0.5)
-        xmid, y1 = ops.gemm_nt_gate_res(o.view(M, D), Wp, pb, x2, g1, N, save_y=bwd)
-        xm2, rstd2 = ops.rmsnorm_modulate_fwd(xmid, n2w, sh2, s2, N, dtype, eps)
+        if resnorm:
+            y1 = ops.gemm_nt(o.view(M, D), Wp, pb)
+            _, xm2, rstd2 = ops.res_rmsnorm_modulate_fwd(x2, y1, g1, None, None, n2w, sh2, s2, N, eps)
+            xmid = x2
+        else:
+            xmid, y1 = ops.gemm_nt_gate_res(o.view(M, D), Wp, pb, x2, g1, N, save_y=bwd)
+            xm2, rstd2 = ops.rmsnorm_modulate_fwd(xmid, n2w, sh2, s2, N, dtype, eps)
         if swiglu:
             h12, hid = ops.gemm_nt_swiglu(xm2, W12, b12, save_h12=bwd)
         else:
             h12 = ops.gemm_nt(xm2, W12, b12)
             hid = ops.gelu_tanh_fwd(h12)
-        xout, y2 = ops.gemm_nt_gate_res(hid, W3, b3, xmid, g2, N, save_y=bwd)
+        if resnorm:
+            y2 = ops.gemm_nt(hid, W3, b3)
+            n1w_next = chain.nxt.get(idx)
+            if n1w_next is not None:
+                modn = mod_all[:, (idx + 1) * nmod * D:(idx + 2) * nmod * D]
+                shn, sn = (modn[:, :D], modn[:, D:2 * D]) if nmod == 6 else (None, modn[:, :D])
+                xout, xm1n, rstd1n = ops.res_rmsnorm_modulate_fwd(x2, y1, g1, y2, g2, n1w_next, shn, sn, N, eps, want_xout=True)
+                chain.fwd[idx + 1] = (xout.data_ptr(), xm1n, rstd1n)
+            else:
+                xout, _, _ = ops.res_rmsnorm_modulate_fwd(x2, y1, g1, y2, g2, rows_per_batch=N, want_xout=True, want_norm=False)
+        else:
+            xout, y2 = ops.gemm_nt_gate_res(hid, W3, b3, xmid, g2, N, save_y=bwd)
         if not bwd:
             return xout.view(B, N, D)
         ctx.input_only = bool(input_only)
@@ -421,7 +445,7 @@
         dW12, r = _dw_into_grad(sg, dh12, xm2, w12_p, ctx.direct); notify.append((r, w12_p))
         dxm2 = ops.gemm_nt(dh12, W12T)
         dn2, dy1, dbp = ops.rmsnorm_modulate_bwd_gate(dxm2, xmid, n2w, s2, rstd2, dx, col(dmod, c_sh2), col(dmod, c_s2),
-                                                      y1, g1, col(dmod, c_g1), N, dtype)
+                                                      y1, g1, col(dmod, c_g1), N, dtype, recompute=ctx.resnorm)
         dWp, r = _dw_into_grad(sg, dy1, o.view(M, D), pw_p, ctx.direct); notify.append((r, pw_p))
         do = ops.gemm_nt(dy1, WpT)
         dqnb = dknb = None
@@ -896,6 +920,9 @@
                     mod_all = _AdaLNAllFn.apply(sc, not torch.is_grad_enabled(), *[l.weight for l in lins], *[l.bias for l in lins])
                 if chain is not None:
                     chain.mod_cols = mod_all.shape[1]
+            if chain is not None and mod_all is not None and self.use_rmsnorm:
+                for i in range(len(self.blocks) - 1):
+                    chain.nxt[i] = self.blocks[i + 1].norm1.weight
             for i, block in enumerate(self.blocks):
                 if self.use_checkpoint:
                     x = checkpoint(block, x, c, self.feat_rope, sc, dtype, not hooked[i], use_reentrant=True)
diff --git a/ldmae_amd/ops.py b/ldmae_amd/ops.py
--- a/ldmae_amd/ops.py
+++ b/ldmae_amd/ops.py
@@ -216,6 +216,7 @@
 
 
 FUSED_QKV = os.environ.get("LDMAE_FUSED_QKV", "1") != "0"
+FUSED_RESNORM = os.environ.get("LDMAE_FUSED_RESNORM", "1") != "0"
 
 
 def gemm_nt_qkv_rope_ok(a, w, B, N, H, hd):
@@ -485,6 +486,34 @@
     return out, rstd
 
 
+def res_rmsnorm_modulate_fwd(x, ya, gate_a, yb=None, gate_b=None, w=None, shift=None, scale=None, rows_per_batch=0, eps=1e-6,
+                             want_xout=False, want_norm=True):
+    M, D = x.shape
+    if ya.dtype not in (torch.bfloat16, torch.float16) or (yb is not None and yb.dtype != ya.dtype):
+        raise RuntimeError("res_rmsnorm_modulate_fwd: bfloat16 or float16 branch outputs of one type expected")
+    if not (want_xout or want_norm):
+        raise RuntimeError("res_rmsnorm_modulate_fwd: nothing requested (want_xout / want_norm)")
+    if rows_per_batch <= 0 or M % rows_per_batch:
+        raise RuntimeError(f"res_rmsnorm_modulate_fwd: M={M} is not a multiple of rows_per_batch={rows_per_batch}")
+    B = M // rows_per_batch
+    x = _arg(x, "res_rmsnorm_modulate_fwd x", torch.float32, (M, D))
+    ya = _arg(ya, "res_rmsnorm_modulate_fwd ya", None, (M, D))
+    yb = _arg(yb, "res_rmsnorm_modulate_fwd yb", None, (M, D))
+    gate_a = _arg(gate_a, "res_rmsnorm_modulate_fwd gate_a", torch.float32, (B, D), rows=True)
+    gate_b = _arg(gate_b, "res_rmsnorm_modulate_fwd gate_b", torch.float32, (B, D), rows=True)
+    xout = torch.empty(M, D, dtype=torch.float32, device=x.device) if want_xout else None
+    out = rstd = None
+    ld = 0
+    if want_norm:
+        out = torch.empty(M, D, dtype=ya.dtype, device=x.device)
+        rstd = torch.empty(M, dtype=torch.float32, device=x.device)
+        ld = shift.stride(0) if shift is not None else (scale.stride(0) if scale is not None else 0)
+    call("ldmae_res_rmsnorm_modulate_fwd", dt(ya.dtype), ptr(x), ptr(ya), ptr(gate_a), _ld(gate_a), ptr(yb), ptr(gate_b),
+         _ld(gate_b) if gate_b is not None else 0, ptr(xout), ptr(w) if want_norm else None, ptr(shift) if want_norm else None,
+         ptr(scale) if want_norm else None, ld, ptr(out), ptr(rstd), M, D, rows_per_batch, eps, stream())
+    return xout, out, rstd
+
+
 def rmsnorm_modulate_bwd(dout, x, w, scale, rstd, dx_accum, dshift, dscale, rows_per_batch, accumulate=True):
     M, D = x.shape
     ws = workspace(L.load().ldmae_rmsnorm_modulate_bwd_workspace_bytes(M, D, rows_per_batch), x.device)
@@ -500,8 +529,11 @@
     return dw
 
 
-def rmsnorm_modulate_bwd_gate(dout, x, w, scale, rstd, dx_accum, dshift, dscale, y, gate, dgate, rows_per_batch, act_dtype, accumulate=True):
+def rmsnorm_modulate_bwd_gate(dout, x, w, scale, rstd, dx_accum, dshift, dscale, y, gate, dgate, rows_per_batch, act_dtype, accumulate=True,
+                              recompute=False):
     M, D = x.shape
+    if recompute and (w is None or dout.dtype != torch.bfloat16):
+        raise RuntimeError("rmsnorm_modulate_bwd_gate(recompute=True): the RMSNorm form with bfloat16 activations only")
     dy = torch.empty(M, D, dtype=act_dtype, device=x.device)
     dbias = torch.empty(D, dtype=torch.float32, device=x.device)
     ws = workspace(L.load().ldmae_rmsnorm_modulate_bwd_gate_workspace_bytes(M, D, rows_per_batch), x.device)
@@ -512,7 +544,8 @@
              ptr(dbias), M, D, rows_per_batch, ptr(ws), stream())
         return None, dy, dbias
     dw = torch.empty(D, dtype=torch.float32, device=x.device)
-    call("ldmae_rmsnorm_modulate_bwd_gate", dt(dout.dtype), ptr(dout), ptr(x), ptr(w), ptr(scale), scale.stride(0) if scale is not None else 0,
+    call("ldmae_rmsnorm_modulate_bwd_gate_recompute" if recompute else "ldmae_rmsnorm_modulate_bwd_gate", dt(dout.dtype), ptr(dout), ptr(x), ptr(w), ptr(scale),
+         scale.stride(0) if scale is not None else 0,
          ptr(rstd), ptr(dx_accum), 1.0 if accumulate else 0.0, ptr(dshift), ptr(dscale), (dshift if dshift is not None else dscale).stride(0) if (dshift is not None or dscale is not None) else 0, ptr(dw), 0.0,
          ptr(y), ptr(gate), gate.stride(0), ptr(dy), ptr(dgate), dgate.stride(0), ptr(dbias), M, D, rows_per_batch, ptr(ws), stream())
     return dw, dy, dbias
```

Result: faster. 1322 images/s, median of 6 (+1.0%).
